# SimonsRoad/gf-pl-slam

Hardware: AMD Instinct MI355X
Metric: stereo frames/sec (2k ORB + 500 LBD, 10 GN iters) (higher is better)
Workload: dtype f64

## Files before the change

gf-pl-slam_amd/csrc/gfpl_abi.hip:

```cpp
#include <hip/hip_runtime.h>

#include <algorithm>
#include <atomic>
#include <cmath>
#include <mutex>
#include <cstdio>
#include <cstdlib>
#include <cstring>
#include <vector>

#include "../../include/gfpl.h"
#include "gfpl_kernels.hpp"

using namespace gfpl;

#define GFPL_NEV 10

struct gfpl_ctx {
    int device = 0;
    hipStream_t stream = nullptr;
    bool own_stream = false;
    gfpl_camera cam{};
    gfpl_config cfg{};
    bool has_cam = false, has_cfg = false;
    bool timing = false;
    hipEvent_t ev[GFPL_NEV]{};
    float stage_ms[7]{};
    std::vector<gfpl_seqbatch*> sbs;
    std::atomic<int> n_detectors{0};
    std::mutex host_mu;
    char* fuse_ws = nullptr;
    size_t fuse_ws_bytes = 0;
    int* fuse_host = nullptr;
    hipEvent_t fuse_ev[2][4]{};
    bool fuse_timed[2] = {false, false};
};

struct gfpl_seqbatch {
    gfpl_ctx* ctx = nullptr;
    int B = 0, kp_cap = 0, kl_cap = 0, mpt_cap = 0, mls_cap = 0;
    void* base = nullptr;
    int64_t bytes = 0;
    DevFrame slot[2];
    int prev_slot = 0;
    bool initialized = false;
    bool has_curr = false;
    DevTrack tr{};
    DevScratch scr{};
    void* stage[2] = {nullptr, nullptr};
    size_t stage_bytes[2] = {0, 0};
    gfpl_frames stage_view[2]{};
    hipStream_t copy = nullptr;
    hipEvent_t ev_ready[2]{}, ev_free[2]{};
    bool ready_pending[2] = {false, false}, free_recorded[2] = {false, false};
    hipEvent_t ev_ticket[16]{};
    int64_t n_tickets = 0;
    int32_t* last_n_pt = nullptr;
    int32_t* last_n_ls = nullptr;
    PyrBuild* pyrb = nullptr;
    int last_cut_mode = -1;
};

struct gfpl_event {
    int device = 0;
    hipEvent_t ev = nullptr;
    int64_t records = 0;
};

int gfpl_ctx_device(const gfpl_ctx* c) { return c->device; }
void* gfpl_ctx_stream(const gfpl_ctx* c) { return (void*)c->stream; }
const gfpl_camera* gfpl_ctx_camera(const gfpl_ctx* c) { return c->has_cam ? &c->cam : nullptr; }
const gfpl_config* gfpl_ctx_config(const gfpl_ctx* c) { return &c->cfg; }
int64_t gfpl_event_records(const gfpl_event* e) { return e->records; }
void gfpl_ctx_attach(gfpl_ctx* c) { c->n_detectors.fetch_add(1); }
void gfpl_ctx_detach(gfpl_ctx* c) { c->n_detectors.fetch_sub(1); }


namespace {

#define HIPCHK(x)                                                  \
    do {                                                            \
        hipError_t e_ = (x);                                        \
        if (e_ != hipSuccess) {                                     \
            std::fprintf(stderr, "gfpl: %s failed: %s\n", #x, hipGetErrorString(e_)); \
            return GFPL_E_HIP;                                      \
        }                                                           \
    } while (0)

int debug_fill_byte() { return env_int("GFPL_DEBUG_FILL", 0) & 0xFF; }

template <typename F, typename H, typename V>
void frame_fields(F& f, H& o, V& v) {
    v.pt(f.pt.pl, o.pt_pl, 2); v.pt(f.pt.pl_obs, o.pt_pl_obs, 2);
    v.pt(f.pt.disp, o.pt_disp, 1); v.pt(f.pt.P, o.pt_P, 3); v.pt(f.pt.sigma2, o.pt_sigma2, 1);
    v.pt(f.pt.idx, o.pt_idx, 1); v.pt(f.pt.level, o.pt_level, 1); v.pt(f.pt.inlier, o.pt_inlier, 1);
    v.pt(f.pt.desc, o.pdesc, 32); v.count(f.pt.n);
    v.ls(f.ls.spl, o.ls_spl, 2); v.ls(f.ls.epl, o.ls_epl, 2);
    v.ls(f.ls.spl_obs, o.ls_spl_obs, 2); v.ls(f.ls.epl_obs, o.ls_epl_obs, 2);
    v.ls(f.ls.sdisp, o.ls_sdisp, 1); v.ls(f.ls.edisp, o.ls_edisp, 1);
    v.ls(f.ls.sdisp_obs, o.ls_sdisp_obs, 1); v.ls(f.ls.edisp_obs, o.ls_edisp_obs, 1);
    v.ls(f.ls.angle, o.ls_angle, 1); v.ls(f.ls.sigma2, o.ls_sigma2, 1);
    v.ls(f.ls.sP, o.ls_sP, 3); v.ls(f.ls.eP, o.ls_eP, 3);
    v.ls(f.ls.le, o.ls_le, 3); v.ls(f.ls.le_obs, o.ls_le_obs, 3);
    v.ls(f.ls.covS, o.ls_covS, 9); v.ls(f.ls.covE, o.ls_covE, 9);
    v.ls(f.ls.cut, o.ls_cut, 2); v.ls(f.ls.invcov, o.ls_invcov, 36);
    v.ls(f.ls.idx, o.ls_idx, 1); v.ls(f.ls.level, o.ls_level, 1); v.ls(f.ls.inlier, o.ls_inlier, 1);
    v.ls(f.ls.desc, o.ldesc, 32); v.count(f.ls.n);
    v.seq(f.pose.Tfw, o.Tfw, 16); v.seq(f.pose.DT, o.DT, 16);
    v.seq(f.pose.DT_cov, o.DT_cov, 36); v.seq(f.pose.Tfw_cov, o.Tfw_cov, 36);
    v.seq(f.pose.DT_cov_eig, o.DT_cov_eig, 6);
    v.seq(f.pose.err_norm, &o.err_norm, 1); v.seq(f.pose.time_stamp, &o.time_stamp, 1);
}

struct SlotCarve {
    Carver& c;
    size_t B, P, L;
    template <typename T, typename U> void pt(T*& d, U, int w) { d = c.take<T>(P * w); }
    template <typename T, typename U> void ls(T*& d, U, int w) { d = c.take<T>(L * w); }
    template <typename T, typename U> void seq(T*& d, U, int w) { d = c.take<T>(B * w); }
    void count(int32_t*& d) { d = c.take<int32_t>(B); }
};

void carve(Carver& c, gfpl_seqbatch* sb) {
    const size_t B = sb->B, P = (size_t)B * sb->kp_cap, L = (size_t)B * sb->kl_cap;
    const gfpl_frame_host none{};
    SlotCarve v{c, B, P, L};
    for (int s = 0; s < 2; ++s) frame_fields(sb->slot[s], none, v);
    sb->tr.matched_pt = c.take<int32_t>(B * sb->mpt_cap);
    sb->tr.n_matched_pt = c.take<int32_t>(B);
    sb->tr.matched_ls = c.take<int32_t>(B * sb->mls_cap);
    sb->tr.n_matched_ls = c.take<int32_t>(B);
    sb->tr.n_inliers = c.take<int32_t>(B);
    sb->tr.n_inliers_pt = c.take<int32_t>(B);
    sb->tr.n_inliers_ls = c.take<int32_t>(B);
    sb->tr.num_frame_loss = c.take<int32_t>(B);
    sb->tr.kf_T = c.take<double>(B * 16);
    sb->tr.kf_cov = c.take<double>(B * 36);
    sb->tr.kf_entropy0 = c.take<double>(B);
    sb->tr.kf_ratio = c.take<double>(B);
    sb->tr.kf_prev_iskf = c.take<int32_t>(B);
    sb->tr.kf_nsince = c.take<int32_t>(B);
    sb->tr.kf_flag = c.take<int32_t>(B);
    sb->scr.cut_rec = c.take<double>(B * sb->mls_cap * CUT_REC);
    sb->scr.knn = c.take<int32_t>(B * 2 * (size_t)sb->kp_cap * 3);
    sb->scr.proj = reinterpret_cast<double*>(sb->scr.knn);
    sb->scr.bytes = c.take<int64_t>(B * STEP_REC);
    sb->scr.n_subpix = c.take<int32_t>(B);
    sb->scr.cut_sum = c.take<double>(B * CUT_SUM_REC);
    sb->scr.cut_dtinv = c.take<double>(B * 16);
    sb->scr.cut_vtab = c.take<double>(B * sb->mls_cap * 2 * CUT_KS);
    sb->scr.pose_DT = c.take<double>(B * 16);
    sb->scr.pose_H = c.take<double>(B * 36);
    sb->scr.pose_err = c.take<double>(B);
    sb->scr.pose_ok = c.take<int32_t>(B);
    sb->scr.pose_in = c.take<double>(B * (6 * (size_t)sb->mpt_cap + 10 * (size_t)sb->mls_cap));
    sb->scr.pose_act = c.take<double>(B * (6 * (size_t)sb->mpt_cap + 10 * (size_t)sb->mls_cap));
    sb->scr.pose_dtini = c.take<double>(B * 16);
    sb->scr.cross_tinv = c.take<double>(B * 16);
    sb->scr.dbg = c.take<int64_t>(B * DBG_REC);
    sb->scr.cut_prog = c.take<int32_t>((size_t)1 << 17);
    sb->scr.cut_path = c.take<uint8_t>(B * sb->mls_cap * CUT_PATH);
    sb->scr.cut_flag = c.take<int32_t>(B);
    sb->scr.cut_vmax = c.take<double>(B * sb->mls_cap * CUT_VMAX);
    sb->scr.cut_offl = c.take<int32_t>(1 + B * sb->mls_cap);
    sb->scr.cut_dtln = c.take<int32_t>(1 + CUT_DTL * B);
    sb->scr.cut_dtl = c.take<double>(CUT_DTL * B * CUT_DTL_REC);
    sb->scr.kf_mask = c.take<int32_t>(B);
    sb->last_n_pt = c.take<int32_t>(B);
    sb->last_n_ls = c.take<int32_t>(B);
}

DevCam devcam(const gfpl_camera& c) {
    DevCam d;
    d.fx = c.fx; d.fy = c.fy; d.cx = c.cx; d.cy = c.cy; d.b = c.b;
    d.width = c.width; d.height = c.height; d.n_levels = c.n_levels;
    for (int i = 0; i < GFPL_MAX_LEVELS; ++i) {
        d.scale[i] = c.scale[i]; d.inv_scale[i] = c.inv_scale[i];
        d.lvl_cols[i] = c.lvl_cols[i]; d.lvl_rows[i] = c.lvl_rows[i];
        d.lvl_offset[i] = c.lvl_offset[i];
        d.sigma2_pt[i] = c.sigma2_pt[i]; d.sigma2_ln[i] = c.sigma2_ln[i];
    }
    d.pyr_bytes = c.pyr_bytes;
    return d;
}

KParams params(gfpl_seqbatch* sb, const gfpl_frames* in) {
    KParams p;
    std::memset(&p, 0, sizeof p);
    p.cam = devcam(sb->ctx->cam);
    p.cfg = sb->ctx->cfg;
    p.prev = sb->slot[sb->prev_slot];
    p.curr = sb->slot[1 - sb->prev_slot];
    p.tr = sb->tr;
    p.scr = sb->scr;
    if (in) p.in = *in;
    p.B = sb->B; p.kp_cap = sb->kp_cap; p.kl_cap = sb->kl_cap;
    p.mpt_cap = sb->mpt_cap; p.mls_cap = sb->mls_cap;
    p.cfg.max_point_match_num = std::min(p.cfg.max_point_match_num, sb->mpt_cap);
    p.cfg.max_line_match_num = std::min(p.cfg.max_line_match_num, sb->mls_cap);
    p.sp_maxD = (float)p.cam.fx;
    p.sp_mbf = (float)(p.cam.fx * p.cam.b);
    p.cut_tq = 0.25 * p.cfg.cut_certify - 4.0 * 0x1p-53;
    {
        const double s = p.cfg.cut_step, lo = p.cfg.cut_rng[0], hi = p.cfg.cut_rng[1];
        auto same = [](double x, double y) { return std::memcmp(&x, &y, sizeof x) == 0; };
        int n = 0;
        for (double t = 0.0; n < CUT_KS && t <= hi && s > 0.0; t = t + s) p.cut_keys[n++] = t;
        const int ns = n;
        for (int i = 1; i < ns && n < CUT_KS; ++i) {
            const double e = p.cut_keys[i] - s;
            bool have = false;
            for (int k = 0; k < n; ++k) have = have || same(p.cut_keys[k], e);
            if (!have && e >= lo) p.cut_keys[n++] = e;
        }
        for (int i = 0; i < n; ++i) {
            int up = -1, dn = -1;
            for (int k = 0; k < n; ++k) {
                if (same(p.cut_keys[k], p.cut_keys[i] + s)) up = k;
                if (same(p.cut_keys[k], p.cut_keys[i] - s)) dn = k;
            }
            p.cut_knxt[i] = (int8_t)up;
            p.cut_kprv[i] = (int8_t)dn;
        }
        p.cut_nkeys = n;
    }
    return p;
}

int check_in(gfpl_seqbatch* sb, const gfpl_frames* in) {
    if (!in) return GFPL_E_INVALID;
    if (in->batch != sb->B || in->kp_cap != sb->kp_cap || in->kl_cap != sb->kl_cap) return GFPL_E_INVALID;
    if (!in->n_kp_l || !in->n_kp_r || !in->kp_l || !in->kp_r || !in->pdesc_l || !in->pdesc_r || !in->n_kl_l ||
        !in->n_kl_r || !in->kl_l || !in->kl_r || !in->ldesc_l || !in->ldesc_r || !in->pyr_r || !in->time_stamp)
        return GFPL_E_INVALID;
    if (((uintptr_t)in->pyr_r & 3) != 0) return GFPL_E_INVALID;
    if ((in->ready && in->ready->device != sb->ctx->device) || (in->consumed && in->consumed->device != sb->ctx->device))
        return GFPL_E_INVALID;
    return GFPL_OK;
}

int in_acquire(gfpl_seqbatch* sb, const gfpl_frames* in) {
    if (in->ready && hipStreamWaitEvent(sb->ctx->stream, in->ready->ev, 0) != hipSuccess) return -2;
    for (int s = 0; s < 2; ++s)
        if (sb->stage[s] && in->n_kp_l == sb->stage_view[s].n_kp_l) {
            if (sb->ready_pending[s] && hipStreamWaitEvent(sb->ctx->stream, sb->ev_ready[s], 0) != hipSuccess) return -2;
            return s;
        }
    return -1;
}
int in_release(gfpl_seqbatch* sb, const gfpl_frames* in, int slot) {
    if (in->consumed) {
        if (hipEventRecord(in->consumed->ev, sb->ctx->stream) != hipSuccess) return GFPL_E_HIP;
        ++in->consumed->records;
    }
    if (slot < 0) return GFPL_OK;
    if (hipEventRecord(sb->ev_free[slot], sb->ctx->stream) != hipSuccess) return GFPL_E_HIP;
    sb->free_recorded[slot] = true;
    return GFPL_OK;
}

static int cut_mode(const gfpl_config& c) { return c.cut_with_max_vol ? c.cut_proof : 0; }

int cfg_supported(const gfpl_config& c) {
    if (!c.best_lr_matches || !c.lr_in_parallel) return GFPL_E_UNSUPPORTED;
    if (c.max_point_match_num < 1 || c.max_point_match_num > GFPL_MAX_MATCHED_PT) return GFPL_E_INVALID;
    if (c.max_line_match_num < 1 || c.max_line_match_num > GFPL_MAX_MATCHED_LS) return GFPL_E_INVALID;
    if (!(c.cut_certify == 0.0 || (c.cut_certify >= 1e-10 && c.cut_certify < 1.0))) return GFPL_E_INVALID;
    if (c.cut_proof < 0 || c.cut_proof > 3) return GFPL_E_INVALID;
    if (!(std::isfinite(c.cut_step) && c.cut_step > 0.0)) return GFPL_E_INVALID;
    if (!(std::isfinite(c.cut_rng[0]) && std::isfinite(c.cut_rng[1]) && c.cut_rng[0] <= c.cut_rng[1]))
        return GFPL_E_INVALID;
    return GFPL_OK;
}

void tmark(gfpl_ctx* c, int i) {
    if (c->timing) (void)hipEventRecord(c->ev[i], c->stream);
}

}

extern "C" {

int gfpl_create(int device, void* stream, gfpl_ctx** out) {
    if (!out) return GFPL_E_INVALID;
    int n = 0;
    if (hipGetDeviceCount(&n) != hipSuccess || n == 0) return GFPL_E_NO_DEVICE;
    if (device < 0 || device >= n) return GFPL_E_INVALID;
    HIPCHK(hipSetDevice(device));
    gfpl_ctx* c = new gfpl_ctx();
    c->device = device;
    c->stream = (hipStream_t)stream;
    gfpl_config_default(&c->cfg);
    c->has_cfg = true;
    for (int i = 0; i < GFPL_NEV; ++i)
        if (hipEventCreate(&c->ev[i]) != hipSuccess) { delete c; return GFPL_E_HIP; }
    *out = c;
// ... 1017 lines not shown
}
}

extern "C" {

int gfpl_read_frame(gfpl_seqbatch* sb, int which, int seq, gfpl_frame_host* o) {
    if (!sb || !o || seq < 0 || seq >= sb->B || (which != GFPL_PREV && which != GFPL_CURR)) return GFPL_E_INVALID;
    hipStream_t s = sb->ctx->stream;
    const DevFrame& f = sb->slot[which == GFPL_PREV ? sb->prev_slot : 1 - sb->prev_slot];
    HIPCHK(hipStreamSynchronize(s));
    int np = 0, nl = 0;
    HIPCHK(hipMemcpy(&np, f.pt.n + seq, 4, hipMemcpyDeviceToHost));
    HIPCHK(hipMemcpy(&nl, f.ls.n + seq, 4, hipMemcpyDeviceToHost));
    o->n_pt = np; o->n_ls = nl;
    SlotCopy<true> v{s, (size_t)seq, (size_t)seq * sb->kp_cap, (size_t)seq * sb->kl_cap, (size_t)np, (size_t)nl};
    frame_fields(f, *o, v);
    HIPCHK(v.e);
    HIPCHK(hipStreamSynchronize(s));
    return GFPL_OK;
}

int gfpl_write_frame(gfpl_seqbatch* sb, int which, int seq, const gfpl_frame_host* o) {
    if (!sb || !o || seq < 0 || seq >= sb->B || (which != GFPL_PREV && which != GFPL_CURR)) return GFPL_E_INVALID;
    if (o->n_pt < 0 || o->n_pt > sb->kp_cap || o->n_ls < 0 || o->n_ls > sb->kl_cap) return GFPL_E_CAPACITY;
    hipStream_t s = sb->ctx->stream;
    const DevFrame& f = sb->slot[which == GFPL_PREV ? sb->prev_slot : 1 - sb->prev_slot];
    XFER(h2d, f.pt.n + seq, &o->n_pt, 1);
    XFER(h2d, f.ls.n + seq, &o->n_ls, 1);
    SlotCopy<false> v{s, (size_t)seq, (size_t)seq * sb->kp_cap, (size_t)seq * sb->kl_cap, (size_t)o->n_pt, (size_t)o->n_ls};
    frame_fields(f, *o, v);
    HIPCHK(v.e);
    HIPCHK(hipStreamSynchronize(s));
    sb->initialized = true;
    if (which == GFPL_CURR) sb->has_curr = true;
    return GFPL_OK;
}

int gfpl_read_track(gfpl_seqbatch* sb, int seq, gfpl_track_host* o) {
    return read_track(sb, seq, o, sb ? sb->tr.n_matched_pt : nullptr, sb ? sb->tr.n_matched_ls : nullptr);
}

int gfpl_read_last_track(gfpl_seqbatch* sb, int seq, gfpl_track_host* o) {
    return read_track(sb, seq, o, sb ? sb->last_n_pt : nullptr, sb ? sb->last_n_ls : nullptr);
}

int gfpl_write_track(gfpl_seqbatch* sb, int seq, const gfpl_track_host* o) {
    if (!sb || !o || seq < 0 || seq >= sb->B) return GFPL_E_INVALID;
    if (o->n_matched_pt < 0 || o->n_matched_pt > sb->mpt_cap || o->n_matched_ls < 0 || o->n_matched_ls > sb->mls_cap)
        return GFPL_E_CAPACITY;
    for (int i = 0; i < o->n_matched_pt; ++i)
        if (o->matched_pt[i] < 0 || o->matched_pt[i] >= sb->kp_cap) return GFPL_E_INVALID;
    for (int i = 0; i < o->n_matched_ls; ++i)
        if (o->matched_ls[i] < 0 || o->matched_ls[i] >= sb->kl_cap) return GFPL_E_INVALID;
    hipStream_t s = sb->ctx->stream;
    XFER(h2d, sb->tr.n_matched_pt + seq, &o->n_matched_pt, 1);
    XFER(h2d, sb->tr.n_matched_ls + seq, &o->n_matched_ls, 1);
    XFER(h2d, sb->tr.n_inliers + seq, &o->n_inliers, 1);
    XFER(h2d, sb->tr.n_inliers_pt + seq, &o->n_inliers_pt, 1);
    XFER(h2d, sb->tr.n_inliers_ls + seq, &o->n_inliers_ls, 1);
    XFER(h2d, sb->tr.num_frame_loss + seq, &o->num_frame_loss, 1);
    XFER(h2d, sb->tr.matched_pt + (size_t)seq * sb->mpt_cap, o->matched_pt, (size_t)o->n_matched_pt);
    XFER(h2d, sb->tr.matched_ls + (size_t)seq * sb->mls_cap, o->matched_ls, (size_t)o->n_matched_ls);
    HIPCHK(hipStreamSynchronize(s));
    return GFPL_OK;
}

int gfpl_set_timing(gfpl_ctx* c, int enable) {
    if (!c) return GFPL_E_INVALID;
    c->timing = enable != 0;
    return GFPL_OK;
}

int gfpl_get_stage_times(gfpl_ctx* c, float* ms7) {
    if (!c || !ms7) return GFPL_E_INVALID;
    if (!c->timing) return GFPL_E_STATE;
    HIPCHK(hipEventSynchronize(c->ev[6]));
    for (int i = 0; i < 6; ++i) HIPCHK(hipEventElapsedTime(&ms7[i], c->ev[i], c->ev[i + 1]));
    HIPCHK(hipEventElapsedTime(&ms7[6], c->ev[0], c->ev[6]));
    return GFPL_OK;
}

int gfpl_get_kernel_times(gfpl_ctx* c, float* ms4) {
    if (!c || !ms4) return GFPL_E_INVALID;
    if (!c->timing) return GFPL_E_STATE;
    if (!c->cfg.use_line_conf_cut) return GFPL_E_STATE;
    HIPCHK(hipEventSynchronize(c->ev[6]));
    HIPCHK(hipEventElapsedTime(&ms4[0], c->ev[4], c->ev[7]));
    HIPCHK(hipEventElapsedTime(&ms4[1], c->ev[7], c->ev[8]));
    HIPCHK(hipEventElapsedTime(&ms4[2], c->ev[8], c->ev[5]));
    HIPCHK(hipEventElapsedTime(&ms4[3], c->ev[5], c->ev[9]));
    return GFPL_OK;
}

}

namespace {
int step_rec_sums(gfpl_seqbatch* sb, int64_t* sums) {
    std::vector<int64_t> v((size_t)sb->B * STEP_REC);
    HIPCHK(hipStreamSynchronize(sb->ctx->stream));
    HIPCHK(hipMemcpy(v.data(), sb->scr.bytes, sizeof(int64_t) * v.size(), hipMemcpyDeviceToHost));
    for (int s = 0; s < STEP_REC; ++s) {
        int64_t t = 0;
        for (int b = 0; b < sb->B; ++b) t += v[(size_t)b * STEP_REC + s];
        sums[s] = t;
    }
    return GFPL_OK;
}
int step_rec_sums(gfpl_seqbatch* sb, int first, int n, int64_t* out, bool on = true) {
    if (!sb || !out) return GFPL_E_INVALID;
    int64_t v[STEP_REC];
    const int e = step_rec_sums(sb, v);
    if (e) return e;
    for (int s = 0; s < n; ++s) out[s] = on ? v[first + s] : 0;
    return GFPL_OK;
}
}

extern "C" {

int gfpl_last_step_kernel_bytes(gfpl_seqbatch* sb, int64_t* bytes4) {
    if (!sb || !bytes4) return GFPL_E_INVALID;
    int64_t v[STEP_REC];
    int e = step_rec_sums(sb, v);
    if (e) return e;
    const bool cut = sb->last_cut_mode >= 0;
    bytes4[0] = cut ? 212 * v[GFPL_STEP_M_L] + 44 * v[GFPL_STEP_M_P] + 552 * (int64_t)sb->B : 0;
    bytes4[1] = v[GFPL_STEP_B_CUT_SEARCH];
    bytes4[2] = cut ? 612 * v[GFPL_STEP_M_L] : 0;
    bytes4[3] = v[GFPL_STEP_B_POSE];
    return GFPL_OK;
}

int gfpl_last_step_stage_bytes(gfpl_seqbatch* sb, int64_t* bytes7) {
    return step_rec_sums(sb, GFPL_STEP_B_STEREO_POINTS, 7, bytes7);
}

int gfpl_last_step_counts(gfpl_seqbatch* sb, int64_t* counts8) {
    return step_rec_sums(sb, GFPL_STEP_N_O, 8, counts8);
}

int gfpl_last_step_track_counts(gfpl_seqbatch* sb, int64_t* counts4) {
    return step_rec_sums(sb, GFPL_STEP_CUT_STEPS, 4, counts4);
}

int gfpl_last_step_cut_proof(gfpl_seqbatch* sb, int64_t* counts4) {
    return step_rec_sums(sb, GFPL_STEP_PROOF_REDONE, 4, counts4,
                         sb && (sb->last_cut_mode == 1 || sb->last_cut_mode == 3));
}

int gfpl_debug_cut_records(gfpl_seqbatch* sb, int b, double* out, int n_lines) {
    if (!sb || !out || b < 0 || b >= sb->B || n_lines < 0 || n_lines > sb->mls_cap) return GFPL_E_INVALID;
    if (hipSetDevice(sb->ctx->device) != hipSuccess) return GFPL_E_HIP;
    if (hipStreamSynchronize(sb->ctx->stream) != hipSuccess) return GFPL_E_HIP;
    const size_t n = (size_t)n_lines * CUT_REC;
    return hipMemcpy(out, sb->scr.cut_rec + (size_t)b * sb->mls_cap * CUT_REC, n * sizeof(double),
                     hipMemcpyDeviceToHost) == hipSuccess ? GFPL_OK : GFPL_E_HIP;
}

int gfpl_debug_step_records(gfpl_seqbatch* sb, int64_t* out) {
    if (!sb || !out) return GFPL_E_INVALID;
    if (hipSetDevice(sb->ctx->device) != hipSuccess) return GFPL_E_HIP;
    if (hipStreamSynchronize(sb->ctx->stream) != hipSuccess) return GFPL_E_HIP;
    return hipMemcpy(out, sb->scr.bytes, (size_t)sb->B * STEP_REC * sizeof(int64_t), hipMemcpyDeviceToHost) == hipSuccess
               ? GFPL_OK : GFPL_E_HIP;
}

int gfpl_debug_clocks(gfpl_seqbatch* sb, int64_t* out) {
    if (!sb || !out) return GFPL_E_INVALID;
    if (hipSetDevice(sb->ctx->device) != hipSuccess) return GFPL_E_HIP;
    if (hipStreamSynchronize(sb->ctx->stream) != hipSuccess) return GFPL_E_HIP;
    return hipMemcpy(out, sb->scr.dbg, (size_t)sb->B * DBG_REC * sizeof(int64_t), hipMemcpyDeviceToHost) == hipSuccess
               ? GFPL_OK : GFPL_E_HIP;
}

int gfpl_last_step_bytes(gfpl_seqbatch* sb, int64_t* bytes) {
    if (!bytes) return GFPL_E_INVALID;
    return step_rec_sums(sb, GFPL_STEP_B_TOTAL, 1, bytes);
}

}
```

gf-pl-slam_amd/csrc/gfpl_kernels.hpp:

```cpp
#pragma once
#include "gfpl_layout.hpp"
#include "gfpl_state.hpp"

#include <atomic>
#include <cstdlib>

namespace gfpl {

inline int env_int(const char* name, int dflt) {
    const char* e = getenv(name);
    if (!e) return dflt;
    return (int)strtol(e, nullptr, (e[0] == '0' && (e[1] == 'x' || e[1] == 'X')) ? 16 : 10);
}

inline hipError_t ensure_dyn_lds(const void* fn, int bytes, std::atomic<unsigned long long>* done) {
    int dev = 0;
    hipError_t e = hipGetDevice(&dev);
    if (e != hipSuccess) return e;
    const unsigned long long bit = dev < 64 ? 1ull << dev : 0ull;
    if (bit && (done->load(std::memory_order_acquire) & bit)) return hipSuccess;
    e = hipFuncSetAttribute(fn, hipFuncAttributeMaxDynamicSharedMemorySize, bytes);
    if (e == hipSuccess && bit) done->fetch_or(bit, std::memory_order_acq_rel);
    return e;
}

constexpr int DYN_LDS_CEILING = 160 * 1024 - 1024;

int sp_wide_max_b();
hipError_t launch_stereo_points(const KParams& p, hipStream_t s);
hipError_t launch_stereo_lines(const KParams& p, hipStream_t s);
hipError_t launch_line_uncertainty(const KParams& p, hipStream_t s);
hipError_t launch_init(const KParams& p, hipStream_t s);
hipError_t launch_knn2(const uint8_t* q, int nq, const uint8_t* t, int nt, int cell, int32_t* idx, float* dist,
                       hipStream_t s);
hipError_t launch_knn2_batched(const uint8_t* q, const int* nq, const uint8_t* t, const int* nt, int cap, int B,
                               int cell, int32_t* packed, hipStream_t s);
hipError_t launch_knn2_counts(const uint8_t* q, const int* nq, const uint8_t* t, const int* nt, int cap, int cell,
                              int32_t* idx, float* dist, hipStream_t s);
hipError_t launch_radius_count(const uint8_t* q, int nq, const uint8_t* t, int nt, int cell, float radius,
                               int32_t* cnt, hipStream_t s);
hipError_t launch_radius_rows(const uint8_t* q, int nq, const uint8_t* t, int nt, int cell, float radius,
                              const int32_t* row_off, int32_t* idx, float* dist, hipStream_t s);
hipError_t launch_match_stats(int kind, const float* d0, const float* d1, int n, int max_num, double* out,
                              hipStream_t s);
hipError_t launch_cross_points(const KParams& p, hipStream_t s);
hipError_t launch_cross_lines(const KParams& p, hipStream_t s);
hipError_t launch_line_cut(const KParams& p, hipStream_t s, const hipEvent_t* marks );
hipError_t launch_pose(const KParams& p, hipStream_t s, hipEvent_t mark );
hipError_t launch_step_bytes(const KParams& p, hipStream_t s);
hipError_t launch_need_kf(const KParams& p, hipStream_t s);
hipError_t launch_curr_frame_is_kf(const KParams& p, const int32_t* mask , hipStream_t s);

struct KfGate {
    DevCam cam;
    double T0[16], T1[16];
    double max_ratio_12_p, desc_th_l;
    int lines, n0;
    int map;
    const int32_t* loc;
    int p_stride;
    double epip_p, epip_l;
    const double* le1;
    const int32_t* i12;
    const float* d12;
    const int32_t* i21;
    const double* P0;
    const double* eP0;
    const double* le0;
    const double* sigma2_0;
    const double* pl1;
    int32_t* pairs;
    int* count;
};
hipError_t launch_kf_gate(const KfGate& g, hipStream_t s);
hipError_t launch_kf_map_filter(const DevCam& cam, const double* T1, const double* P, int n, int lines,
                                int32_t* loc, uint8_t* desc_out, const uint8_t* desc_in, int* count, hipStream_t s);

struct FuseSelect {
    DevCam cam;
    int lines, n, n_kf;
    const double* X;
    const int32_t* kf;
    const double* T_kf;
    const uint8_t* desc_in;
    int32_t* loc;
    uint8_t* desc_out;
    int* count;
    int* bad_kf;
};
struct FuseGate {
    int lines, cap;
    const int* n_sel;
    const int32_t* loc;
    const int32_t* idx;
    const double* X;
    double max_pp, max_pl, max_dl;
    int32_t* pairs;
    int* count;
};
hipError_t launch_fuse_select(const FuseSelect& a, hipStream_t s);
hipError_t launch_fuse_gate(const FuseGate& g, hipStream_t s);

struct LoopPair {
    int n0_pt, n0_ls;
    const int32_t *pi12, *pi21;
    const int32_t *li12, *li21;
    const double* P0;
    const double* pl1;
    const double *sP0, *eP0;
    const double* le1;
};
struct LoopArgs {
    DevCam cam;
    double homog_th;
    int max_iters;
    gfpl_loop_params prm;
    const LoopPair* pairs;
    int pt_cap, ls_cap;
    int32_t* pt_pairs;
    uint8_t* pt_inlier;
    int32_t* ls_pairs;
    uint8_t* ls_inlier;
    gfpl_loop_result* out;
};
hipError_t launch_loop_closure(const LoopArgs& a, int n, hipStream_t s);

struct BowVocabDev {
    const uint8_t* desc;
    const BowNode* node;
    const int32_t* rank_word;
    const double* rank_weight;
    int weighting;
};
struct BowSet {
    const uint8_t* desc;
    int count, pad;
};
struct BowPair {
    const int32_t* ia; const double* va;
    const int32_t* ib; const double* vb;
    int na, nb;
};
hipError_t launch_bow_transform(const BowVocabDev& v, const BowSet* sets, int n, int max_count, int cap, int32_t* keys,
                                int32_t* word_ids, double* values, int32_t* n_words, hipStream_t s);
hipError_t launch_bow_score(const BowPair* pairs, int n, double* scores, hipStream_t s);

struct LbaProb {
    gfpl_lba_counts n;
    const double* x_kf;
    double* T_kf;
    const double* T_fix;
    double *pt, *ls;
    const double *pt_obs, *pt_sigma, *ls_obs, *ls_sigma;
    double* x_out;
    const int32_t *lm_start, *obs_lm, *obs_kf;
    LbaPtrs m;
};
struct LbaArgs {
    DevCam cam;
    double homog_th;
    gfpl_lba_params prm;
    const LbaProb* probs;
    gfpl_lba_result* out;
    int lds_kfs;
};
hipError_t launch_lba(const LbaArgs& a, int n, hipStream_t s);

struct GbaRules {
    int divisor_zero;
    int line_th_homog;
    int prepass_transposed;
    int any_sign_pivot;
};
constexpr GbaRules GBA_RULES_REFERENCE{1, 1, 1, 1};
struct GbaProb {
    gfpl_gba_counts n;
    const double* x_kf;
    double* T_kf;
    const double* T_fix;
    double *pt, *ls;
    const double *pt_obs, *pt_sigma, *ls_obs, *ls_sigma;
    double* x_out;
    const int32_t *lm_start, *obs_lm, *obs_kf, *obs_pair, *pair_start, *pair_kf, *kf_start, *kf_obs, *blk_start, *terms;
    GbaPtrs m;
};
struct GbaArgs {
    DevCam cam;
    double homog_th;
    gfpl_lba_params prm;
    GbaRules rules;
    GbaProb pr;
    gfpl_lba_result* out;
};
struct GbaGrid {
    int block = GBA_BLOCK;
    int ldlt_kfs = GBA_LDLT_KFS;
};
hipError_t enqueue_gba(const GbaArgs& a, const GbaGrid& grid, hipStream_t s);
int gba_max_lds_bytes(int n_kf);

// ... 161 lines not shown
```

gf-pl-slam_amd/csrc/gfpl_records.hpp:

```cpp
#pragma once
#include <stddef.h>
#include <stdint.h>

#include "../../include/gfpl.h"

namespace gfpl {

constexpr int STEP_REC = GFPL_STEP_REC;
constexpr int STEP_CUT_CLOCK_DURATION = GFPL_STEP_CUT_UNBOUNDED;

constexpr int64_t* step_rec(int64_t* bytes, int b) { return bytes + (size_t)STEP_REC * b; }

constexpr int DBG_REC = 8;
constexpr int64_t* dbg_row(int64_t* dbg, int b) { return dbg + DBG_REC * (size_t)b; }

enum DbgCutSearch { DBG_CUT_HW_ID = 6, DBG_CUT_XCC_ID = 7 };
enum DbgVerify {
    DBG_VFY_TS = 0, DBG_VFY_TK = 1, DBG_VFY_TA = 2, DBG_VFY_TV = 3,
    DBG_VFY_MASK = 4,
    DBG_VFY_WORST = 5,
    DBG_VFY_XCHK = 6,
    DBG_VFY_DLINES = 7
};
enum DbgCutEig { DBG_EIG_SWEEPS = 0, DBG_EIG_EVALS = 1 };
enum DbgCutClock { DBG_CCK_BEGIN = 0, DBG_CCK_END = 1, DBG_CCK_HW_ID = 2, DBG_CCK_XCC_ID = 3 };
enum DbgCutPhase { DBG_CPK_PHASES = 0 , DBG_CPK_TRANS = 4 , DBG_CPK_COUNTS = 7 };
enum DbgCutW { DBG_CWK_PHASES = 0 , DBG_CWK_ROUNDS = 5, DBG_CWK_TRANS = 6, DBG_CWK_STEPS = 7 };
enum DbgStereo { DBG_SP_PROBE_KEYS = 7 };
enum DbgPoseFinish { DBG_PFIN_INVERSE = 0, DBG_PFIN_EIG = 1, DBG_PFIN_REST = 2 };

#define CUT_PATH 64
#define CUT_P_STAY 8
#define CUT_P_EXACT 16
#define CUT_KS 22

#define CUT_FAST 56
#define CUT_REC 80
constexpr int CUT_INFO = 21;
constexpr int CUT_NX = CUT_FAST + CUT_INFO;
constexpr int CUT_NX_EB = 3;
#define PD_PS 0
#define PD_PE 18
#define PD_VS 36
#define PD_VE 41
#define PD_OK 46
#define PD_NEXT 47
#define PD_ERR 48
static_assert(PD_ERR + 7 <= CUT_FAST && CUT_FAST == 56, "per-line comparison data layout");
static_assert(CUT_REC * 8 == 640 && CUT_NX + CUT_NX_EB <= CUT_REC, "a record is 5 x 128 B: five 16-B loads per lane");

constexpr int CUT_SUM_REC = 24;

constexpr int CUT_VMAX_EB = 6;
constexpr int CUT_VMAX = CUT_VMAX_EB + 8;

#define CUT_DTL 4
constexpr int CUT_DTL_REC = 32;
enum CutDtl {
    DTL_S = 0,
    DTL_K0 = CUT_INFO, DTL_A1, DTL_B1, DTL_CS, DTL_CE, DTL_R0, DTL_RTS, DTL_RTE, DTL_OK, DTL_END
};
static_assert(DTL_END <= CUT_DTL_REC, "cut_dtl record");

}
```

gf-pl-slam_amd/csrc/gfpl_state.hpp:

```cpp
#pragma once
#include <stdint.h>

#include "../../include/gfpl.h"
#include "gfpl_device.hpp"
#include "gfpl_records.hpp"

namespace gfpl {

struct DevPoints {
    double* pl;
    double* pl_obs;
    double* disp;
    double* P;
    double* sigma2;
    int32_t* idx;
    int32_t* level;
    uint8_t* inlier;
    uint8_t* desc;
    int32_t* n;
};

struct DevLines {
    double *spl, *epl, *spl_obs, *epl_obs;
    double *sdisp, *edisp, *sdisp_obs, *edisp_obs;
    double *angle, *sigma2;
    double *sP, *eP, *le, *le_obs;
    double *covS, *covE;
    double *cut;
    double *invcov;
    int32_t *idx, *level;
    uint8_t *inlier;
    uint8_t *desc;
    int32_t* n;
};

struct DevPose {
    double *Tfw, *DT;
    double *DT_cov, *Tfw_cov;
    double *DT_cov_eig;
    double *err_norm, *time_stamp;
};

struct DevFrame {
    DevPoints pt;
    DevLines ls;
    DevPose pose;
};

struct DevTrack {
    int32_t* matched_pt;
    int32_t* n_matched_pt;
    int32_t* matched_ls;
    int32_t* n_matched_ls;
    int32_t* n_inliers;
    int32_t* n_inliers_pt;
    int32_t* n_inliers_ls;
    int32_t* num_frame_loss;
    double* kf_T;
    double* kf_cov;
    double* kf_entropy0;
    double* kf_ratio;
    int32_t* kf_prev_iskf;
    int32_t* kf_nsince;
    int32_t* kf_flag;
};

struct DevScratch {
    double* cut_rec;
    int32_t* knn;
    double* proj;
    int64_t* bytes;
    int32_t* n_subpix;
    double* cut_sum;
    double* cut_dtinv;
    double* cut_vtab;
    double* pose_DT;
    double* pose_H;
    double* pose_err;
    int32_t* pose_ok;
    double* pose_in;
    double* pose_act;
    double* pose_dtini;
    int32_t* kf_mask;
    double* cross_tinv;
    int64_t* dbg;
    int32_t* cut_prog;
    uint8_t* cut_path;
    int32_t* cut_flag;
    int32_t* cut_offl;
    int32_t* cut_dtln;
    double* cut_dtl;
    double* cut_vmax;
};

struct KParams {
    DevCam cam;
    gfpl_config cfg;
    DevFrame prev, curr;
    DevTrack tr;
    DevScratch scr;
    gfpl_frames in;
    int B, kp_cap, kl_cap, mpt_cap, mls_cap;
    const double* dt_ini;
    float sp_maxD, sp_mbf;
    double cut_tq;
    double cut_keys[CUT_KS];
    int cut_nkeys;
    int8_t cut_knxt[CUT_KS], cut_kprv[CUT_KS];
};

#define LINE_SLOT(p, b, m) ((size_t)(b) * (p).mls_cap + (m))

}
```

gf-pl-slam_amd/csrc/k_cut.hip:

```cpp
#include "gfpl_kernels.hpp"
#include "gfpl_wave.hpp"

namespace gfpl {

struct LineCutData {
    double sP[3], eP[3], covS[9], covE[9], Jl[2];
};

template <typename T, bool SD = false>
__device__ __forceinline__ T endpointVar_t(const DevCam& cam, const double* DT_inv, const T* Jl, const T* Pt,
                                           const T* cov, double zlo) {
    T Jdt[9];
#pragma unroll
    for (int i = 0; i < 3; ++i)
#pragma unroll
        for (int j = 0; j < 3; ++j) Jdt[i * 3 + j] = T(DT_inv[i * 4 + j]);
    T cur[3];
    se3_apply_t<T, double>(DT_inv, Pt, cur);
    rb_floor(cur[2], zlo);
    const T f = T(cam.fx), pz = cur[2], pz_2 = pz * pz;
    T Jp[9];
    Jp[0] = f / pz; Jp[3] = T(0.0); Jp[6] = T(0.0);
    Jp[1] = T(0.0); Jp[4] = f / pz; Jp[7] = T(0.0);
    if constexpr (SD) {
        const double n0 = (-f) * cur[0], n1 = (-f) * cur[1], n2 = (-f) * T(cam.b);
        const SharedDiv dz = div_prep(pz_2, n0);
        Jp[2] = div_by(dz, n0);
        Jp[5] = div_by(dz, n1);
        Jp[8] = div_by(dz, n2);
    } else {
        Jp[2] = ((-f) * cur[0]) / pz_2;
        Jp[5] = ((-f) * cur[1]) / pz_2;
        Jp[8] = ((-f) * T(cam.b)) / pz_2;
    }
    T T1[6], T2[6], T3[6], M[4];
#pragma unroll
    for (int i = 0; i < 2; ++i)
#pragma unroll
        for (int j = 0; j < 3; ++j)
            T1[i * 3 + j] = (Jp[i * 3 + 0] * Jdt[0 * 3 + j] + Jp[i * 3 + 1] * Jdt[1 * 3 + j]) + Jp[i * 3 + 2] * Jdt[2 * 3 + j];
#pragma unroll
    for (int i = 0; i < 2; ++i)
#pragma unroll
        for (int j = 0; j < 3; ++j)
            T2[i * 3 + j] = (T1[i * 3 + 0] * cov[0 * 3 + j] + T1[i * 3 + 1] * cov[1 * 3 + j]) + T1[i * 3 + 2] * cov[2 * 3 + j];
#pragma unroll
    for (int i = 0; i < 2; ++i)
#pragma unroll
        for (int j = 0; j < 3; ++j)
            T3[i * 3 + j] = (T2[i * 3 + 0] * Jdt[j * 3 + 0] + T2[i * 3 + 1] * Jdt[j * 3 + 1]) + T2[i * 3 + 2] * Jdt[j * 3 + 2];
#pragma unroll
    for (int i = 0; i < 2; ++i)
#pragma unroll
        for (int j = 0; j < 2; ++j)
            M[i * 2 + j] = (T3[i * 3 + 0] * Jp[j * 3 + 0] + T3[i * 3 + 1] * Jp[j * 3 + 1]) + T3[i * 3 + 2] * Jp[j * 3 + 2];
    const T r0 = Jl[0] * M[0] + Jl[1] * M[2];
    const T r1 = Jl[0] * M[1] + Jl[1] * M[3];
    return r0 * Jl[0] + r1 * Jl[1];
}

template <typename T, bool VAR = true>
__device__ __forceinline__ void cut_endpoint_t(const DevCam& cam, double homog, const double* DT_inv, const T* Jl,
                                               const T* P0, const T* P1, const T* C0, const T* C1, T c, T* out7,
                                               double zlo) {
    T Pt[3];
#pragma unroll
    for (int k = 0; k < 3; ++k) Pt[k] = (T(1.0) - c) * P0[k] + c * P1[k];
    if (VAR) {
        const T a = (T(1.0) - c) * (T(1.0) - c), q = c * c;
        T cov[9];
#pragma unroll
        for (int i = 0; i < 9; ++i) cov[i] = a * C0[i] + q * C1[i];
        out7[0] = endpointVar_t<T>(cam, DT_inv, Jl, Pt, cov, zlo);
    }
    T cur[3];
    se3_apply_t<T, double>(DT_inv, Pt, cur);
    rb_floor(cur[2], zlo);
    poseJac_t<T>(cam, homog, cur, Jl[0], Jl[1], out7 + 1);
}
__device__ __forceinline__ void cut_endpoint(const DevCam& cam, double homog, const double* DT_inv, const double* Jl,
                                             const double* P0, const double* P1, const double* C0, const double* C1,
                                             double c, double* out7) {
    cut_endpoint_t<double>(cam, homog, DT_inv, Jl, P0, P1, C0, C1, c, out7, 0.0);
}

template <bool FULL>
__device__ __forceinline__ void cut_assemble(const double* S7, const double* E7, double* info) {
    const double vs = S7[0], ve = E7[0];
    const double* Js = S7 + 1;
    const double* Je = E7 + 1;
    const double det = vs * ve - 0.0 * 0.0;
    const double invdet = 1.0 / det;
    const double i00 = ve * invdet, i10 = -0.0 * invdet, i01 = -0.0 * invdet, i11 = vs * invdet;
    double T0[6], T1[6];
#pragma unroll
    for (int i = 0; i < 6; ++i) {
        T0[i] = Js[i] * i00 + Je[i] * i10;
        T1[i] = Js[i] * i01 + Je[i] * i11;
    }
    if (FULL) {
#pragma unroll
        for (int i = 0; i < 6; ++i)
#pragma unroll
            for (int j = 0; j < 6; ++j) info[i * 6 + j] = T0[i] * Js[j] + T1[i] * Je[j];
    } else {
#pragma unroll
        for (int i = 0; i < 6; ++i)
#pragma unroll
            for (int j = 0; j <= i; ++j) info[tri(i, j)] = T0[i] * Js[j] + T1[i] * Je[j];
    }
}

template <bool FULL>
__device__ __forceinline__ void poseInfoOnLine(const DevCam& cam, double homog, const double* DT_inv,
                                               const LineCutData& L, double c0, double c1, double* info) {
    double S7[7], E7[7];
    cut_endpoint(cam, homog, DT_inv, L.Jl, L.sP, L.eP, L.covS, L.covE, c0, S7);
    cut_endpoint(cam, homog, DT_inv, L.Jl, L.eP, L.sP, L.covE, L.covS, c1, E7);
    cut_assemble<FULL>(S7, E7, info);
}

__device__ __forceinline__ void load_line(const DevLines& L, size_t q, LineCutData& d) {
#pragma unroll
    for (int k = 0; k < 3; ++k) { d.sP[k] = L.sP[3 * q + k]; d.eP[k] = L.eP[3 * q + k]; }
#pragma unroll
    for (int k = 0; k < 9; ++k) { d.covS[k] = L.covS[9 * q + k]; d.covE[k] = L.covE[9 * q + k]; }
    d.Jl[0] = L.le_obs[3 * q];
    d.Jl[1] = L.le_obs[3 * q + 1];
}


template <typename T>
__device__ __forceinline__ T sym3_t(const T* A, const T* x, const T* y) {
    const T ax = (A[0] * y[0] + A[1] * y[1]) + A[2] * y[2];
    const T ay = (A[1] * y[0] + A[3] * y[1]) + A[4] * y[2];
    const T az = (A[2] * y[0] + A[4] * y[1]) + A[5] * y[2];
    return (x[0] * ax + x[1] * ay) + x[2] * az;
}

template <typename T>
__device__ __forceinline__ void cut_poly_coeff_t(const T* g0, const T* g1, T lx, T ly, int k, T* Pk) {
    const T dx = g1[0] - g0[0], dy = g1[1] - g0[1], dz = g1[2] - g0[2];
    auto prod = [&](T a0, T a1, T b0, T b1) -> T {
        return k == 0 ? a0 * b0 : (k == 1 ? a0 * b1 + a1 * b0 : a1 * b1);
    };
    auto lin = [&](T a0, T a1) -> T { return k == 0 ? a0 : (k == 1 ? a1 : T(0.0)); };
    const T x0 = g0[0], y0 = g0[1], z0 = g0[2];
    Pk[0] = lx * lin(z0, dz);
    Pk[1] = ly * lin(z0, dz);
    Pk[2] = -(lx * lin(x0, dx) + ly * lin(y0, dy));
    Pk[3] = -((lx * prod(x0, dx, y0, dy) + ly * prod(y0, dy, y0, dy)) + ly * prod(z0, dz, z0, dz));
    Pk[4] = (lx * prod(x0, dx, x0, dx) + lx * prod(z0, dz, z0, dz)) + ly * prod(x0, dx, y0, dy);
    Pk[5] = ly * prod(x0, dx, z0, dz) - lx * prod(y0, dy, z0, dz);
}

template <typename T>
__device__ __forceinline__ void cut_poly_coef_t(const double* Dl, const T* sP, const T* eP, const T* covS,
                                                const T* covE, const T* Jl, T* P, T* V, T* g) {
    se3_apply_t<T, double>(Dl, sP, g);
    se3_apply_t<T, double>(Dl, eP, g + 3);
    T A[2][6];
    const T* Cs[2] = {covS, covE};
#pragma unroll
    for (int w = 0; w < 2; ++w) {
        T Tm[9];
#pragma unroll
        for (int i = 0; i < 3; ++i)
#pragma unroll
            for (int k = 0; k < 3; ++k)
                Tm[i * 3 + k] = (T(Dl[i * 4 + 0]) * Cs[w][0 * 3 + k] + T(Dl[i * 4 + 1]) * Cs[w][1 * 3 + k]) +
                                T(Dl[i * 4 + 2]) * Cs[w][2 * 3 + k];
        const int ii[6] = {0, 0, 0, 1, 1, 2}, jj[6] = {0, 1, 2, 1, 2, 2};
#pragma unroll
        for (int e = 0; e < 6; ++e)
            A[w][e] = (Tm[ii[e] * 3 + 0] * T(Dl[jj[e] * 4 + 0]) + Tm[ii[e] * 3 + 1] * T(Dl[jj[e] * 4 + 1])) +
                      Tm[ii[e] * 3 + 2] * T(Dl[jj[e] * 4 + 2]);
    }
#pragma unroll
    for (int side = 0; side < 2; ++side) {
        T* Ps = P + 18 * side;
#pragma unroll
        for (int k = 0; k < 3; ++k) cut_poly_coeff_t<T>(g + 3 * side, g + 3 * (1 - side), Jl[0], Jl[1], k, Ps + 6 * k);
        const T* p0 = Ps;
        const T* p1 = Ps + 6;
        const T a0 = sym3_t<T>(A[side], p0, p0), a1 = sym3_t<T>(A[side], p0, p1), a2 = sym3_t<T>(A[side], p1, p1);
        const T b0 = sym3_t<T>(A[1 - side], p0, p0), b1 = sym3_t<T>(A[1 - side], p0, p1), b2 = sym3_t<T>(A[1 - side], p1, p1);
        T* v = V + 5 * side;
        v[0] = a0;
        v[1] = T(2.0) * (a1 - a0);
        v[2] = ((a2 - T(4.0) * a1) + a0) + b0;
        v[3] = T(2.0) * ((a1 - a2) + b1);
        v[4] = a2 + b2;
    }
}

__device__ __forceinline__ void cut_poly_data(const double* Dl, const LineCutData& d, double homog, double* fd) {
    double P[36], V[10], g[6];
    cut_poly_coef_t<double>(Dl, d.sP, d.eP, d.covS, d.covE, d.Jl, P, V, g);
#pragma unroll
    for (int i = 0; i < 18; ++i) { fd[PD_PS + i] = P[i]; fd[PD_PE + i] = P[18 + i]; }
#pragma unroll
    for (int i = 0; i < 5; ++i) { fd[PD_VS + i] = V[i]; fd[PD_VE + i] = V[5 + i]; }
    const double z0 = g[2], z1 = g[5];
    fd[PD_OK] = (((z0 > 0.0 && z1 > 0.0) || (z0 < 0.0 && z1 < 0.0)) && z0 * z0 > 2.0 * homog && z1 * z1 > 2.0 * homog)
                    ? 1.0 : 0.0;
}

template <int W>
__global__ void __launch_bounds__(64 * W) k_cut_prep(KParams p) {
    extern __shared__ double prep_lds[];
    const int b = blockIdx.x;
    const int lane = threadIdx.x & 63, wv = W > 1 ? (int)(threadIdx.x >> 6) : 0;
    const int nls = p.tr.n_matched_ls[b];
    const int npt = p.tr.n_matched_pt[b];
    if (nls == 0) return;
    double (*chunk)[65] = reinterpret_cast<double (*)[65]>(prep_lds + (size_t)wv * 21 * 65);
    const DevCam& cam = p.cam;
    const double homog = p.cfg.homog_th;
    DevLines& L = p.prev.ls;
    const DevPoints& P = p.prev.pt;
    const size_t lb = (size_t)b * p.kl_cap, pbase = (size_t)b * p.kp_cap;
    const int32_t* mls = p.tr.matched_ls + (size_t)b * p.mls_cap;
    const int32_t* mpt = p.tr.matched_pt + (size_t)b * p.mpt_cap;
    double* rec_l = p.scr.cut_rec + LINE_SLOT(p, b, 0) * CUT_REC;
    double Dl[16];
    {
        double Tc[16], Tp[16], Ti[16];
#pragma unroll
        for (int i = 0; i < 16; ++i) { Tc[i] = p.curr.pose.Tfw[16 * b + i]; Tp[i] = p.prev.pose.Tfw[16 * b + i]; }
        mat4_inv(Tc, Ti);
        mat4_mul(Ti, Tp, Dl);
    }
    if (wv == 0 && lane < 16) p.scr.cut_dtinv[16 * b + lane] = Dl[lane];
    double s = 0.0;
    const int nl_ch = (nls + 63) >> 6, np_ch = (npt + 63) >> 6;
    auto chunk_cnt = [&](int c) {
        const bool lines = c < nl_ch;
        return min(64, (lines ? nls : npt) - (((lines ? c : c - nl_ch)) << 6));
    };
    for (int c0 = 0; c0 < nl_ch + np_ch; c0 += W) {
        const int c = c0 + wv;
        if (c < nl_ch + np_ch) {
            const bool lines = c < nl_ch;
            const int m = ((lines ? c : c - nl_ch) << 6) + lane;
            const int cnt = chunk_cnt(c);
            double info[21];
            double fd[CUT_FAST];
            if (lane < cnt) {
                if (lines) {
                    LineCutData d;
                    load_line(L, lb + mls[m], d);
                    poseInfoOnLine<false>(cam, homog, Dl, d, 0.0, 0.0, info);
#pragma unroll
                    for (int i = PD_ERR; i < CUT_FAST; ++i) fd[i] = 0.0;
                    cut_poly_data(Dl, d, homog, fd);
                    fd[PD_NEXT] = (double)mls[min(m + 1, nls - 1)];
                } else {
                    const size_t q = pbase + mpt[m];
                    double Pp[3] = {P.P[3 * q], P.P[3 * q + 1], P.P[3 * q + 2]};
                    double cur[3], uv[2];
                    se3_apply(Dl, Pp, cur);
                    projection(cam, cur, uv);
                    const double dx = uv[0] - P.pl_obs[2 * q], dy = uv[1] - P.pl_obs[2 * q + 1];
                    double J[6];
                    poseJac(cam, homog, cur, dx, dy, J);
#pragma unroll
                    for (int i = 0; i < 6; ++i)
#pragma unroll
                        for (int j = 0; j <= i; ++j) info[tri(i, j)] = J[i] * J[j];
                }
            }
            if (lines) {
                double* stg = &chunk[0][0];
                const int pl = lane >> 3, pp = lane & 7;
                double* rc = rec_l + (size_t)(c << 6) * CUT_REC;
#pragma unroll
                for (int sl = 0; sl < CUT_REC / 16; ++sl) {
                    if (lane < cnt) {
#pragma unroll
                        for (int k = 0; k < 16; ++k) {
                            const int x = 16 * sl + k;
                            stg[lane * 17 + k] = x < CUT_FAST ? fd[x] : (x < CUT_FAST + 21 ? info[x - CUT_FAST] : 0.0);
                        }
                    }
                    wave_lds_sync();
#pragma unroll
                    for (int g8 = 0; g8 < 8; ++g8) {
                        const int ln = 8 * g8 + pl;
                        if (ln < cnt)
                            reinterpret_cast<double2*>(rc + (size_t)ln * CUT_REC + 16 * sl)[pp] =
                                make_double2(stg[ln * 17 + 2 * pp], stg[ln * 17 + 2 * pp + 1]);
                    }
                    wave_lds_sync();
                }
            }
            if (lane < cnt) {
#pragma unroll
                for (int i = 0; i < 21; ++i) chunk[i][lane] = info[i];
            }
        }
        __syncthreads();
        if (wv == 0 && lane < 21) {
            const double (*all)[21][65] = reinterpret_cast<const double (*)[21][65]>(prep_lds);
            for (int k = 0; k < W && c0 + k < nl_ch + np_ch; ++k) {
                const int cnt = chunk_cnt(c0 + k);
                for (int e = 0; e < cnt; ++e) s = s + all[k][lane][e];
            }
        }
        __syncthreads();
    }
    if (wv == 0 && lane < 21) p.scr.cut_sum[CUT_SUM_REC * b + lane] = s;
}
constexpr size_t cut_prep_lds(int w) { return (size_t)w * 21 * 65 * sizeof(double); }

__device__ __forceinline__ float ceil_f32(double x) {
    if (!(x >= 0.0)) return __builtin_inff();
    float f = (float)x;
    if ((double)f < x) f = __uint_as_float(__float_as_uint(f) + 1u);
    return f;
}
template <bool SD>
__device__ __forceinline__ double ref_vprime_at(const DevCam& cam, double homog, const double* Dl, const double* P0,
                                                const double* P1, const double* C0, const double* C1, const double* Jl,
                                                double c) {
    double Pt[3];
#pragma unroll
    for (int k = 0; k < 3; ++k) Pt[k] = (1.0 - c) * P0[k] + c * P1[k];
    const double a = (1.0 - c) * (1.0 - c), qq = c * c;
    double cov[9];
#pragma unroll
    for (int i = 0; i < 9; ++i) cov[i] = a * C0[i] + qq * C1[i];
    const double v = endpointVar_t<double, SD>(cam, Dl, Jl, Pt, cov, 0.0);
    double cur[3];
    se3_apply(Dl, Pt, cur);
    const double f = cam.fx / ref_max(homog, cur[2] * cur[2]);
    return v / (f * f);
}
__device__ __forceinline__ double ref_vprime(const DevCam& cam, double homog, const double* Dl, const DevLines& L,
                                             size_t q, int side, double c) {
    const double* P0 = side ? L.eP + 3 * q : L.sP + 3 * q;
    const double* P1 = side ? L.sP + 3 * q : L.eP + 3 * q;
    const double* C0 = side ? L.covE + 9 * q : L.covS + 9 * q;
    const double* C1 = side ? L.covS + 9 * q : L.covE + 9 * q;
    const double Jl[2] = {L.le_obs[3 * q], L.le_obs[3 * q + 1]};
    return ref_vprime_at<false>(cam, homog, Dl, P0, P1, C0, C1, Jl, c);
}

__global__ void __launch_bounds__(256) k_cut_vtab(KParams p) {
    const int b = blockIdx.x;
    const int nls = p.tr.n_matched_ls[b];
    const int nk = p.cut_nkeys;
    if (nls == 0 || nk == 0 || (p.cfg.cut_proof != 2 && p.scr.cut_flag[b] == 0)) return;
    const DevLines& L = p.prev.ls;
    const double* Dl = p.scr.cut_dtinv + 16 * (size_t)b;
    const int per = 2 * nk;
    for (int idx = threadIdx.x; idx < nls * per; idx += 256) {
        const int m = idx / per, r = idx - m * per;
        const int side = r >= nk ? 1 : 0, slot = r - side * nk;
        const size_t q = (size_t)b * p.kl_cap + p.tr.matched_ls[LINE_SLOT(p, b, m)];
        p.scr.cut_vtab[LINE_SLOT(p, b, m) * (2 * CUT_KS) + side * CUT_KS + slot] =
            ref_vprime(p.cam, p.cfg.homog_th, Dl, L, q, side, p.cut_keys[slot]);
    }
}

__device__ __forceinline__ void cut_line_bounds(const KParams& p, size_t q, bool pd_ok, const double* Dl, float* eb) {
    const DevLines& L = p.prev.ls;
    const double rlo = p.cfg.cut_rng[0], rhi = p.cfg.cut_rng[1];
    const double C = fmax(rhi, 0.0), T = fmax(fabs(rlo), fabs(rhi));
#pragma unroll
    for (int i = 0; i < 14; ++i) eb[i] = __builtin_inff();
    bool ok = rlo >= 0.0 && rhi <= 1.0 && pd_ok && p.cam.fx > 0.0;
    RB sP[3], eP[3], cS[9], cE[9], Jl[2];
#pragma unroll
    for (int k = 0; k < 3; ++k) { sP[k] = RB(L.sP[3 * q + k]); eP[k] = RB(L.eP[3 * q + k]); }
#pragma unroll
    for (int k = 0; k < 9; ++k) { cS[k] = RB(L.covS[9 * q + k]); cE[k] = RB(L.covE[9 * q + k]); }
    Jl[0] = RB(L.le_obs[3 * q]);
    Jl[1] = RB(L.le_obs[3 * q + 1]);
    double eo[2][7];
    double zlo = 0.0, zmax = 0.0;
    if (ok) {
        RB P[36], V[10], g[6];
        cut_poly_coef_t<RB>(Dl, sP, eP, cS, cE, Jl, P, V, g);
        double gd[6];
        {
            const double s3[3] = {L.sP[3 * q], L.sP[3 * q + 1], L.sP[3 * q + 2]};
            const double e3[3] = {L.eP[3 * q], L.eP[3 * q + 1], L.eP[3 * q + 2]};
            se3_apply(Dl, s3, gd);
            se3_apply(Dl, e3, gd + 3);
        }
        zlo = fmin(fabs(gd[2]) - g[2].e, fabs(gd[5]) - g[5].e);
        zmax = fmax(fabs(gd[2]) + g[2].e, fabs(gd[5]) + g[5].e);
        ok = zlo > 0.0;
#pragma unroll
        for (int side = 0; side < 2; ++side) {
#pragma unroll
            for (int i = 0; i < 6; ++i)
                eo[side][i] = (P[18 * side + i].e + T * (P[18 * side + 6 + i].e + T * P[18 * side + 12 + i].e));
            const RB* v = V + 5 * side;
            eo[side][6] = v[0].e + T * (v[1].e + T * (v[2].e + T * (v[3].e + T * v[4].e)));
        }
    }
    if (ok) {
        const double cam_fx = p.cam.fx;
        const double s1 = zmax * zmax / cam_fx;
#pragma unroll
        for (int side = 0; side < 2; ++side) {
            RB o7[7];
            cut_endpoint_t<RB, false>(p.cam, p.cfg.homog_th, Dl, Jl, side ? eP : sP, side ? sP : eP, side ? cE : cS,
                                      side ? cS : cE, RB(C, 0.0, 0.0), o7, zlo);
#pragma unroll
            for (int i = 0; i < 6; ++i) eb[7 * side + i] = ceil_f32(1.01 * (eo[side][i] + o7[1 + i].e * s1));
            {
                const RB c(C, 0.0, 0.0);
                const RB* Q0 = side ? eP : sP;
                const RB* Q1 = side ? sP : eP;
                RB Pt[3], cur[3];
#pragma unroll
                for (int k = 0; k < 3; ++k) Pt[k] = (RB(1.0) - c) * Q0[k] + c * Q1[k];
                se3_apply_t<RB, double>(Dl, Pt, cur);
                rb_floor(cur[2], zlo);
                eb[7 * side + 6] = cur[2].lo > 0.0 ? ceil_f32(1.01 * cur[2].e / cur[2].lo) : __builtin_inff();
            }
        }
    }
}

__device__ __forceinline__ void cut_line_bounds_p(const KParams& p, size_t q, bool pd_ok, const double* Dl, float* eb) {
    const DevLines& L = p.prev.ls;
    const double rlo = p.cfg.cut_rng[0], rhi = p.cfg.cut_rng[1];
    const double C = fmax(rhi, 0.0), T = fmax(fabs(rlo), fabs(rhi));
#pragma unroll
    for (int i = 0; i < 14; ++i) eb[i] = __builtin_inff();
    if (!(rlo >= 0.0 && rhi <= 1.0 && pd_ok && p.cam.fx > 0.0)) return;
    RB sP[3], eP[3], Jl[2];
#pragma unroll
    for (int k = 0; k < 3; ++k) { sP[k] = RB(L.sP[3 * q + k]); eP[k] = RB(L.eP[3 * q + k]); }
    Jl[0] = RB(L.le_obs[3 * q]);
    Jl[1] = RB(L.le_obs[3 * q + 1]);
    RB g[6];
    se3_apply_t<RB, double>(Dl, sP, g);
    se3_apply_t<RB, double>(Dl, eP, g + 3);
    double gd[6];
    {
        const double s3[3] = {L.sP[3 * q], L.sP[3 * q + 1], L.sP[3 * q + 2]};
        const double e3[3] = {L.eP[3 * q], L.eP[3 * q + 1], L.eP[3 * q + 2]};
        se3_apply(Dl, s3, gd);
        se3_apply(Dl, e3, gd + 3);
    }
    const double zlo = fmin(fabs(gd[2]) - g[2].e, fabs(gd[5]) - g[5].e);
    const double zmax = fmax(fabs(gd[2]) + g[2].e, fabs(gd[5]) + g[5].e);
    if (!(zlo > 0.0)) return;
    const double s1 = zmax * zmax / p.cam.fx;
#pragma unroll
    for (int side = 0; side < 2; ++side) {
        double eo[6] = {0, 0, 0, 0, 0, 0};
        double tk = 1.0;
#pragma unroll
        for (int k = 0; k < 3; ++k) {
            RB Pk[6];
            cut_poly_coeff_t<RB>(g + 3 * side, g + 3 * (1 - side), Jl[0], Jl[1], k, Pk);
#pragma unroll
            for (int i = 0; i < 6; ++i) eo[i] = eo[i] + tk * Pk[i].e;
            tk = tk * T;
        }
        RB o7[7];
        cut_endpoint_t<RB, false>(p.cam, p.cfg.homog_th, Dl, Jl, side ? eP : sP, side ? sP : eP, nullptr, nullptr,
                                  RB(C, 0.0, 0.0), o7, zlo);
#pragma unroll
        for (int i = 0; i < 6; ++i) eb[7 * side + i] = ceil_f32(1.01 * (eo[i] + o7[1 + i].e * s1));
        const RB c(C, 0.0, 0.0);
        const RB* Q0 = side ? eP : sP;
        const RB* Q1 = side ? sP : eP;
        RB Pt[3], cur[3];
#pragma unroll
        for (int k = 0; k < 3; ++k) Pt[k] = (RB(1.0) - c) * Q0[k] + c * Q1[k];
        se3_apply_t<RB, double>(Dl, Pt, cur);
        rb_floor(cur[2], zlo);
        eb[7 * side + 6] = cur[2].lo > 0.0 ? ceil_f32(1.01 * cur[2].e / cur[2].lo) : __builtin_inff();
    }
}

__global__ void __launch_bounds__(64) k_cut_bounds(KParams p) {
    const int b = blockIdx.y;
    const int m = blockIdx.x * 64 + threadIdx.x;
    const int nls = p.tr.n_matched_ls[b];
    if (m >= nls || (p.cfg.cut_proof != 2 && p.scr.cut_flag[b] == 0)) return;
    const size_t q = (size_t)b * p.kl_cap + p.tr.matched_ls[LINE_SLOT(p, b, m)];
    double* rec = p.scr.cut_rec + LINE_SLOT(p, b, m) * CUT_REC;
    double Dl[16];
#pragma unroll
    for (int i = 0; i < 16; ++i) Dl[i] = p.scr.cut_dtinv[16 * b + i];
    float eb[14];
    cut_line_bounds(p, q, rec[PD_OK] != 0.0, Dl, eb);
    float* out = reinterpret_cast<float*>(rec + PD_ERR);
#pragma unroll
    for (int i = 0; i < 14; ++i) out[i] = eb[i];
}

#define CUT_G 8
#ifndef CUT_BATCH
#define CUT_BATCH 8
#endif
#ifndef CUT_WAIT
#define CUT_WAIT 16
#endif
#define CUT_SL 7
#define CUT_EP 43

__device__ __forceinline__ void exact_endpoint(const DevCam& cam, double homog, const double* Dl, const DevLines& L,
                                               size_t q, int side, double t, double* o7) {
    const double* sP = L.sP + 3 * q;
    const double* eP = L.eP + 3 * q;
    const double* cS = L.covS + 9 * q;
    const double* cE = L.covE + 9 * q;
    const double Jl[2] = {L.le_obs[3 * q], L.le_obs[3 * q + 1]};
    cut_endpoint(cam, homog, Dl, Jl, side ? eP : sP, side ? sP : eP, side ? cE : cS, side ? cS : cE, t, o7);
}

__device__ __forceinline__ int nb_off(int j, int side) {
    const unsigned pl = side == 0 ? 0x31u : 0x54u, mi = side == 0 ? 0xC2u : 0xA8u;
    return (int)((pl >> j) & 1u) - (int)((mi >> j) & 1u);
}
__device__ __forceinline__ double nb_step(int j, int side, double st) {
    return (double)nb_off(j, side) * st;
}
__device__ __forceinline__ int nb_slot(int j, int side) {
    return 1 + nb_off(j, side);
}

constexpr double CUT_MIN_PIVOT = 1e-2;
__device__ __forceinline__ void chol_s(const double* a, double* out) {
    double L[21];
#pragma unroll
    for (int i = 0; i < 21; ++i) L[i] = a[i];
    bool ok = true;
#pragma unroll
    for (int k = 0; k < 6; ++k) {
        const double akk = L[tri(k, k)];
        double x = akk;
#pragma unroll
        for (int j = 0; j < k; ++j) x = x - L[tri(k, j)] * L[tri(k, j)];
        if (!(x > CUT_MIN_PIVOT * akk && akk < 1e300)) { ok = false; x = 1.0; }
        double r = __builtin_amdgcn_rsq(x);
        r = r * (1.5 - (0.5 * x) * (r * r));
        r = r * (1.5 - (0.5 * x) * (r * r));
        L[tri(k, k)] = 0.0;
        out[21 + k] = r;
#pragma unroll
        for (int i = k + 1; i < 6; ++i) {
            double v = L[tri(i, k)];
#pragma unroll
            for (int j = 0; j < k; ++j) v = v - L[tri(i, j)] * L[tri(k, j)];
            L[tri(i, k)] = v * r;
        }
    }
#pragma unroll
    for (int i = 0; i < 21; ++i) out[i] = L[i];
    out[27] = ok ? 1.0 : 0.0;
}

__device__ __forceinline__ double rcp_fast(double x) {
    double r = __builtin_amdgcn_rcp(x);
    r = __builtin_fma(__builtin_fma(-x, r, 1.0), r, r);
    r = __builtin_fma(__builtin_fma(-x, r, 1.0), r, r);
    return r;
}

__device__ __forceinline__ double h4(const double* c, double t) {
    return __builtin_fma(t, __builtin_fma(t, __builtin_fma(t, __builtin_fma(t, c[4], c[3]), c[2]), c[1]), c[0]);
}
__device__ __forceinline__ double h4abs(const double* c, double t) {
    return __builtin_fma(t, __builtin_fma(t, __builtin_fma(t, __builtin_fma(t, fabs(c[4]), fabs(c[3])), fabs(c[2])),
                                          fabs(c[1])), fabs(c[0]));
}
__device__ __forceinline__ double h2(double c0, double c1, double c2, double t) {
    return __builtin_fma(t, __builtin_fma(t, c2, c1), c0);
}

__device__ __forceinline__ double cut_ours_P(const double* fd, int side, int i, double t) {
    const int o = side ? PD_PE : PD_PS;
    return h2(fd[o + i], fd[o + 6 + i], fd[o + 12 + i], t);
}
__device__ __forceinline__ double cut_ours_V(const double* fd, int side, double t) {
    const int o = side ? PD_VE : PD_VS;
    return __builtin_fma(t, __builtin_fma(t, __builtin_fma(t, __builtin_fma(t, fd[o + 4], fd[o + 3]), fd[o + 2]),
                                          fd[o + 1]), fd[o]);
}
__device__ __forceinline__ double cut_ours_info(const double* xs, double is, double ie, int ra, int cb) {
    return __builtin_fma(xs[1 + ra] * is, xs[1 + cb], (xs[8 + ra] * ie) * xs[8 + cb]);
}

struct __attribute__((aligned(16))) CutCmp {
    double ns[5], ne[5];
    double vs[5], ve[5];
    double cc[9];
    double bnd[3];
    double bs[3], be[3];
    float eb[6];
};
static_assert(sizeof(CutCmp) == 336, "CutCmp: 84 dwords (bank spread of the 8 groups' rows)");
enum { CC_NS = 0, CC_NE = 5, CC_VS = 10, CC_VE = 15, CC_CC = 20, CC_BND = 29, CC_BS = 32, CC_BE = 35, CC_END = 38 };
static_assert(offsetof(CutCmp, ns) == 8 * CC_NS && offsetof(CutCmp, ne) == 8 * CC_NE && offsetof(CutCmp, vs) == 8 * CC_VS &&
              offsetof(CutCmp, ve) == 8 * CC_VE && offsetof(CutCmp, cc) == 8 * CC_CC && offsetof(CutCmp, bnd) == 8 * CC_BND &&
              offsetof(CutCmp, bs) == 8 * CC_BS && offsetof(CutCmp, be) == 8 * CC_BE && offsetof(CutCmp, eb) == 8 * CC_END,
              "CutCmp's fields as double offsets");
struct CutReg {
    double ns[5], ne[5], vs[5], ve[5], cc[9], bnd[3];
    float eb[6];
};
__device__ __forceinline__ void cut_reg_load(const CutCmp& c, CutReg& r) {
#pragma unroll
    for (int i = 0; i < 5; ++i) { r.ns[i] = c.ns[i]; r.ne[i] = c.ne[i]; r.vs[i] = c.vs[i]; r.ve[i] = c.ve[i]; }
#pragma unroll
    for (int i = 0; i < 9; ++i) r.cc[i] = c.cc[i];
#pragma unroll
    for (int i = 0; i < 3; ++i) r.bnd[i] = c.bnd[i];
#pragma unroll
    for (int i = 0; i < 6; ++i) r.eb[i] = c.eb[i];
}

template <bool PROOF>
__device__ __forceinline__ double cut_dcore_p1(double Ns, double Vs, double Ne, double Ve, double C, double P1,
                                              double VsA, double VeA, const float* eb, double tq, int& bound_ok) {
    const double D = __builtin_fma(Vs + Ns, Ve + Ne, -(C * C));
    const double den = Vs * Ve;
    const double r = rcp_fast(den);
    const double d = D * r;
    const double P2 = __builtin_fma(VsA, Ve, VeA * Vs);
    constexpr double u = 0x1p-53;
    const double Dd = D * den;
    const bool healthy = (Vs > 0.0) & (Ve > 0.0) & (D > 0.0) & (d < 1e300) & (Dd < 1e300);
    const float iVs = (float)(Ve * r), iVe = (float)(Vs * r);
    const float E = __builtin_fmaf(iVs, __builtin_fmaf(eb[2], iVs, eb[1]), iVe * __builtin_fmaf(eb[4], iVe, eb[3]));
    bool agree = true;
    if (PROOF) agree = (E * 1.0001f <= eb[0]) & (eb[5] * (iVs + iVe) <= 0.25f);
    (void)E;
    const bool fwd = __builtin_fma((40.0 * u) * P1, den, ((16.0 * u) * P2) * D) <= tq * Dd;
    bound_ok = healthy & agree & fwd;
    return healthy ? d : __longlong_as_double(0x7ff8000000000000ll);
}
template <bool PROOF>
__device__ __forceinline__ double cut_dval(const CutReg& c, double t0, double t1, double tq, int& bound_ok,
                                           double vs_t = 0.0, double ve_t = 0.0) {
    const double Ns = h4(c.ns, t0), Ne = h4(c.ne, t1);
    const double Vs = PROOF ? vs_t : h4(c.vs, t0), Ve = PROOF ? ve_t : h4(c.ve, t1);
    const double C = __builtin_fma(t1, __builtin_fma(t1, h2(c.cc[2], c.cc[5], c.cc[8], t0), h2(c.cc[1], c.cc[4], c.cc[7], t0)),
                                   h2(c.cc[0], c.cc[3], c.cc[6], t0));
    return cut_dcore_p1<PROOF>(Ns, Vs, Ne, Ve, C, c.bnd[0], c.bnd[1], c.bnd[2], c.eb, tq, bound_ok);
}

__device__ __attribute__((noinline)) double cut_exact_step(const double* sj, const double* ej, const double* s1,
                                                           const double* e4, const double* S, const double* Sb,
                                                           int first, double* mc) {
    double tot[21], tmp[21];
    cut_assemble<false>(sj, ej, tmp);
#pragma unroll
    for (int i = 0; i < 21; ++i) tot[i] = tmp[i] + S[i];
    const double vj = logdet6_lower(tot);
    if (first) {
#pragma unroll
        for (int i = 0; i < 21; ++i) tot[i] = Sb[i];
    } else {
        cut_assemble<false>(s1, e4, tmp);
#pragma unroll
        for (int i = 0; i < 21; ++i) tot[i] = tmp[i] + S[i];
    }
    *mc = logdet6_lower(tot);
    return vj;
}


__device__ __forceinline__ int group_first_max(double v, int valid, int j, double mc, double& top) {
    const double x = (valid && v == v) ? v : -__builtin_inf();
    double mx = fmax(x, dpp_mov_f64<DPP_XOR1>(x));
    mx = fmax(mx, dpp_mov_f64<DPP_XOR2>(mx));
    mx = fmax(mx, dpp_mov_f64<DPP_HALF_MIRROR>(mx));
    top = mx;
    const unsigned long long at = __ballot((x == mx) & (mx > -__builtin_inf()));
    const unsigned gb = (unsigned)(at >> (threadIdx.x & ~7u)) & 0xFFu;
    const int k = gb ? __builtin_ctz(gb) : 8;
    (void)j;
    return (k < 8 && mx > mc) ? k : -1;
}


struct CutX {
    int best;
    int m_sync;
};
template <typename T>
__device__ __forceinline__ T* rl_ptr(T* p, int l) {
    const unsigned long long v = reinterpret_cast<unsigned long long>(p);
    const unsigned lo = (unsigned)__builtin_amdgcn_readlane((int)(unsigned)v, l);
    const unsigned hi = (unsigned)__builtin_amdgcn_readlane((int)(unsigned)(v >> 32), l);
    return reinterpret_cast<T*>(((unsigned long long)hi << 32) | lo);
}
__device__ __attribute__((noinline)) CutX cut_exact_round(bool exact, int valid, int first, int m, int m_sync, double r0,
                                                          double r1, size_t q_cur, size_t lb, int best,
                                                          const int32_t* mls, const double* rec_l, double* sP, double* eP,
                                                          double* covS, double* covE, double* le_obs, double* cut,
                                                          double* sumE, double* tmp, double* tmpw, const double* Dl,
                                                          double fx, double cb, double homog, double st) {
    const int j = threadIdx.x & 7;
    const int lane = threadIdx.x & 63;
    DevCam cam{};
    cam.fx = fx;
    cam.b = cb;
    DevLines L{};
    L.sP = sP;
    L.eP = eP;
    L.covS = covS;
    L.covE = covE;
    L.le_obs = le_obs;
    L.cut = cut;
    __builtin_amdgcn_fence(__ATOMIC_SEQ_CST, "workgroup");
    {
        unsigned long long need = __ballot(j == 0 && exact && m_sync < m);
        while (need) {
            const int gl = __ffsll((long long)need) - 1;
            need &= need - 1;
            const int ms = __builtin_amdgcn_readlane(m_sync, gl), me = __builtin_amdgcn_readlane(m, gl);
            const size_t lbG = (size_t)(unsigned)__builtin_amdgcn_readlane((int)(unsigned)lb, gl) |
                               ((size_t)(unsigned)__builtin_amdgcn_readlane((int)(unsigned)(lb >> 32), gl) << 32);
            const int32_t* mlsG = rl_ptr(mls, gl);
            const double* recG = rl_ptr(rec_l, gl);
            const double* DlG = rl_ptr(Dl, gl);
            double* sumEG = rl_ptr(sumE, gl);
            const bool mine = (lane >> 3) == (gl >> 3);
            for (int s0 = ms; s0 < me; s0 += 64) {
                const int nl = min(64, me - s0);
                double info[21];
                if (lane < nl) {
                    const size_t qf = lbG + mlsG[s0 + lane];
                    const double c0 = __hip_atomic_load(&L.cut[2 * qf], __ATOMIC_RELAXED, __HIP_MEMORY_SCOPE_WORKGROUP);
                    const double c1 = __hip_atomic_load(&L.cut[2 * qf + 1], __ATOMIC_RELAXED, __HIP_MEMORY_SCOPE_WORKGROUP);
                    double s7[7], e7[7];
                    exact_endpoint(cam, homog, DlG, L, qf, 0, c0, s7);
                    exact_endpoint(cam, homog, DlG, L, qf, 1, c1, e7);
                    cut_assemble<false>(s7, e7, info);
                }
#pragma unroll
                for (int c = 0; c < 6; ++c) {
                    if (lane < nl) {
#pragma unroll
                        for (int i = 0; i < 4; ++i) {
                            const int e = 4 * c + i;
                            if (e < 21) {
                                tmpw[4 * lane + i] = info[e];
                                tmpw[256 + 4 * lane + i] = recG[(size_t)(s0 + lane) * CUT_REC + CUT_FAST + e];
                            }
                        }
                    }
                    wave_lds_sync();
                    if (mine && j < 4 && 4 * c + j < 21) {
                        const int e = 4 * c + j;
                        double Se = sumEG[e];
                        for (int l = 0; l < nl; ++l) Se = (Se - tmpw[256 + 4 * l + j]) + tmpw[4 * l + j];
                        sumEG[e] = Se;
                    }
                    wave_lds_sync();
                }
            }
            if (mine) m_sync = me;
        }
    }
    double* const epf = tmp;
    double* const xs = tmp + CUT_EP;
    if (exact) {
        if (j < 6) {
            const int eside = j < 3 ? 0 : 1;
            const double eoff = (j % 3) == 0 ? -st : ((j % 3) == 2 ? st : 0.0);
            const double t = (eside == 0 ? r0 : r1) + eoff;
            double o7[7];
            exact_endpoint(cam, homog, Dl, L, q_cur, eside, t, o7);
#pragma unroll
            for (int i = 0; i < 7; ++i) epf[CUT_SL * j + i] = o7[i];
        }
#pragma unroll
        for (int e = 0; e < 21; ++e) xs[e] = sumE[e] - rec_l[(size_t)m * CUT_REC + CUT_FAST + e];
    }
    wave_lds_sync();
    if (exact) {
        const int cs = nb_slot(j, 0), ce = 3 + nb_slot(j, 1);
        double mc, top;
        const double vj = cut_exact_step(&epf[CUT_SL * cs], &epf[CUT_SL * ce], &epf[CUT_SL * 1], &epf[CUT_SL * 4], xs,
                                         sumE, first, &mc);
        best = group_first_max(vj, valid, j, mc, top);
    }
    wave_lds_sync();
    return CutX{best, m_sync};
}

constexpr unsigned long long tri_pack(int want_row) {
    unsigned long long v = 0;
    int e = 0;
    for (int i = 0; i < 6; ++i)
        for (int k = 0; k <= i; ++k, ++e) v |= (unsigned long long)(want_row ? i : k) << (3 * e);
    return v;
}

__device__ __attribute__((noinline)) void cut_bound_row(int j, double T, const double* fs, const double* sA,
                                                        const double* tg, double* wg) {
    const float* ef = reinterpret_cast<const float*>(fs + PD_ERR);
    const double sg = 1.002 * tg[57 + j];
    const double Sii = sA[tri(j, j)];
    const double es = ef[j], ee = ef[7 + j];
    const double ps = fabs(fs[PD_PS + j]) + T * (fabs(fs[PD_PS + 6 + j]) + T * fabs(fs[PD_PS + 12 + j])) + es;
    const double pe = fabs(fs[PD_PE + j]) + T * (fabs(fs[PD_PE + 6 + j]) + T * fabs(fs[PD_PE + 12 + j])) + ee;
    const double rs = sqrt(sg);
    double row = 0.0;
    const double kc = Sii * sg;
    const int ex = __builtin_amdgcn_frexp_exp(Sii);
    wg[j] = kc;
    wg[6 + j] = sqrt(kc);
    wg[12 + j] = sg * ps * ps;
    wg[18 + j] = sg * pe * pe;
    wg[24 + j] = es * rs;
    wg[30 + j] = ee * rs;
    wg[36 + j] = (Sii > 0.0 && Sii < 1e300) ? 0.6931471805599453 * (double)(abs(ex) + 1) : __builtin_inf();
    wg[42 + j] = row * rs;
}
__device__ __attribute__((noinline)) void cut_bound_line(double T, double tau, const double* cl, const double* fs,
                                                         const double* wg, float* eb) {
    const float* ef = reinterpret_cast<const float*>(fs + PD_ERR);
    const double Bs = h2(cl[CC_BS], cl[CC_BS + 1], cl[CC_BS + 2], T), Be = h2(cl[CC_BE], cl[CC_BE + 1], cl[CC_BE + 2], T);
    double sum[8];
    for (int q = 0; q < 8; ++q) {
        double a = wg[6 * q];
        for (int i = 1; i < 6; ++i) a = a + wg[6 * q + i];
        sum[q] = a;
    }
    constexpr double u = 0x1p-53;
    const double Kc = sum[0], xi = sum[1], Qs = sum[2], Qe = sum[3], Lam = sum[6];
    const double epsS = sum[7] + (7.01 * u) * xi * xi;
    const double hs = sum[4] + (6.01 * u) * Bs * xi, he = sum[5] + (6.01 * u) * Be * xi;
    const double rvs = 4.1 * (double)ef[6] + 12.0 * u, rve = 4.1 * (double)ef[13] + 12.0 * u;
    const double ck = 110.0 * u;
    const double K0 = 1.002 * epsS + ck * Kc + (7.1 * u) * Lam;
    const double bs = Bs + hs, be = Be + he;
    const double A1 = 1.03 * (2.0 * ck * Qs + 4.0 * hs * bs + 4.0 * rvs * bs * bs), A2 = 0.0;
    const double B1 = 1.03 * (2.0 * ck * Qe + 4.0 * he * be + 4.0 * rve * be * be), B2 = 0.0;
    double R0 = fmin(0.125 * tau, 1e-3) - 1.01 * K0;
    if (!(epsS <= 1e-3 && Kc <= 1e8 && R0 > 0.0)) R0 = -1.0;
    float r0f = (float)R0;
    if ((double)r0f > R0) r0f = R0 > 0.0 ? __uint_as_float(__float_as_uint(r0f) - 1u) : -1.0f;
    eb[0] = r0f;
    eb[1] = ceil_f32(A1);
    eb[2] = ceil_f32(A2);
    eb[3] = ceil_f32(B1);
    eb[4] = ceil_f32(B2);
    eb[5] = (rvs <= 0.25 && rve <= 0.25) ? 0.0f : __builtin_inff();
}

__device__ __forceinline__ int wave_sum8(int v) {
    v += __shfl_xor(v, 8);
    v += __shfl_xor(v, 16);
    v += __shfl_xor(v, 32);
    return __builtin_amdgcn_readfirstlane(v);
}
struct CutProg { int* own; int* partner; };
__device__ __forceinline__ CutProg cut_prog_slots(int* base) {
    const unsigned hw = __builtin_amdgcn_s_getreg((4 << 0) | (0 << 6) | (31 << 11));
    const unsigned xcc = __builtin_amdgcn_s_getreg((20 << 0) | (0 << 6) | (31 << 11));
    const unsigned simd = ((((xcc & 7u) * 8u + ((hw >> 13) & 7u)) * 2u + ((hw >> 12) & 1u)) * 16u + ((hw >> 8) & 15u)) * 4u +
                          ((hw >> 4) & 3u);
    const unsigned slot = hw & 15u;
    return CutProg{base + simd * 16u + slot, base + simd * 16u + (slot ^ 1u)};
}
#ifndef GFPL_CUT_WPE
#define GFPL_CUT_WPE 2
#endif
#ifndef GFPL_CUT_NOPF
#define GFPL_CUT_NOPF 0
#endif
#define CUT_SSTR (GFPL_CUT_NOPF ? 21 : 25)
template <bool PROOF, bool REC = false>
__global__ void __launch_bounds__(64) __attribute__((amdgpu_waves_per_eu(GFPL_CUT_WPE, GFPL_CUT_WPE))) k_cut_search(KParams p) {
    __shared__ double sumA[CUT_G][CUT_SSTR];
    __shared__ double sumE[CUT_G][CUT_SSTR];
    __shared__ double fst[CUT_G][CUT_FAST + 1];
    constexpr bool PF = !PROOF && !GFPL_CUT_NOPF;
    __shared__ __attribute__((aligned(16))) double nxl[PF ? 5 : 1][PF ? 128 : 2];
    __shared__ double tmp[CUT_G][CUT_EP + 25 + 1];
    static_assert(CUT_G * (CUT_EP + 25 + 1) >= 512, "the exact-sum flush stages 64 x (4 + 4) doubles in tmp");
    __shared__ CutCmp cmpl[CUT_G];
    __shared__ double vtab[PROOF ? CUT_G : 1][PROOF ? 2 * CUT_KS : 1];
    __shared__ int cnxt[PROOF ? CUT_KS : 1], cprv[PROOF ? CUT_KS : 1];
    const int lane = threadIdx.x;
    constexpr bool CLOCK = GFPL_DIAG(GFPL_CUT_CLOCK);
    const uint64_t t_beg = CLOCK ? wall_clock64() : 0;
    const int g = lane >> 3, j = lane & 7;
    const int b = blockIdx.x * CUT_G + g;
    if (!PROOF && p.cfg.cut_proof == 0 && j == 0 && b < p.B) {
        dbg_row(p.scr.dbg, b)[DBG_CUT_HW_ID] = (int64_t)__builtin_amdgcn_s_getreg((4 << 0) | (0 << 6) | (31 << 11));
        dbg_row(p.scr.dbg, b)[DBG_CUT_XCC_ID] = (int64_t)__builtin_amdgcn_s_getreg((20 << 0) | (0 << 6) | (31 << 11));
    }
    const bool live = b < p.B && (!PROOF || p.cfg.cut_proof == 2 || p.scr.cut_flag[b] != 0);
    const int nls = live ? p.tr.n_matched_ls[b] : 0;
    constexpr bool rec = !PROOF && REC;
    uint8_t* const path = p.scr.cut_path + LINE_SLOT(p, live ? b : 0, 0) * CUT_PATH;
    int lstep = 0;
    __shared__ __attribute__((aligned(8))) uint8_t pth[REC ? CUT_G : 1][REC ? CUT_PATH : 8];
    const DevCam& cam = p.cam;
    const double homog = p.cfg.homog_th;
    const double tau = p.cfg.cut_certify;
    const double tq = p.cut_tq;
    DevLines& L = p.prev.ls;
    const size_t lb = (size_t)(live ? b : 0) * p.kl_cap;
    const int32_t* mls = p.tr.matched_ls + (size_t)(live ? b : 0) * p.mls_cap;
    const double* rec_l = p.scr.cut_rec + LINE_SLOT(p, live ? b : 0, 0) * CUT_REC;
    const double* Dl = p.scr.cut_dtinv + 16 * (size_t)(live ? b : 0);
    const double st = p.cfg.cut_step;
    const double rlo = p.cfg.cut_rng[0], rhi = p.cfg.cut_rng[1];
    double* const xs = &tmp[g][CUT_EP];
    double* const wg = &tmp[g][0];
    double* const gm = &tmp[g][36];
    const double nb0 = nb_step(j, 0, st), nb1 = nb_step(j, 1, st);
    constexpr unsigned long long TRI_ROW = tri_pack(1), TRI_COL = tri_pack(0);
    if (PROOF) {
        if (lane < CUT_KS) {
            cnxt[lane] = p.cut_knxt[lane];
            cprv[lane] = p.cut_kprv[lane];
        }
        __syncthreads();
    }
    int m = 0;
    int m_sync = 0;
    int first = 1;
    double r0 = 0.0, r1 = 0.0;
    int line_ok = 0;
    int pend = 0;
    int wait = 0;
    double dc = 0.0;
    int c_ok = 0;
    int n_unb = 0;
    int i0 = 0, i1 = 0, n0s = -1, p0s = -1, n1s = -1, p1s = -1;
    size_t q_cur = 0, q_nx = 0;
    auto open_line = [&]() {
        if (PROOF) {
            const double* vt = p.scr.cut_vtab + LINE_SLOT(p, live ? b : 0, m) * (2 * CUT_KS);
            for (int idx = j; idx < 2 * CUT_KS; idx += 8) vtab[g][idx] = vt[idx];
            i0 = 0;
            i1 = 0;
            n0s = n1s = cnxt[0];
            p0s = p1s = cprv[0];
        }
        double o[28];
        {
            double S[21];
#pragma unroll
            for (int e = 0; e < 21; ++e) S[e] = sumA[g][e];
            chol_s(S, o);
        }
        line_ok = (o[27] != 0.0) && (fst[g][PD_OK] != 0.0);
        if (j < 6) {
            double w[6];
#pragma unroll
            for (int i = 0; i < 6; ++i) {
                double u = fst[g][6 * j + i];
#pragma unroll
                for (int k = 0; k < i; ++k) u = __builtin_fma(-o[tri(i, k)], w[k], u);
                w[i] = u * o[21 + i];
            }
#pragma unroll
            for (int i = 0; i < 6; ++i) wg[6 * j + i] = w[i];
            double x[6], sg = 0.0;
            if (PROOF) {
#pragma unroll
            for (int i = 0; i < 6; ++i) {
                double uu = i == j ? 1.0 : 0.0;
#pragma unroll
                for (int k = 0; k < i; ++k) uu = __builtin_fma(-o[tri(i, k)], x[k], uu);
                x[i] = uu * o[21 + i];
                sg = __builtin_fma(x[i], x[i], sg);
            }
            tmp[g][57 + j] = sg;
            }
        }
        wave_lds_sync();
#pragma unroll
        for (int kk = 0; kk < 3; ++kk) {
            const int e = j + 8 * kk;
            if (e < 21) {
                const int ra = (int)((TRI_ROW >> (3 * e)) & 7), cb = (int)((TRI_COL >> (3 * e)) & 7);
                double s = wg[6 * ra] * wg[6 * cb];
#pragma unroll
                for (int i = 1; i < 6; ++i) s = __builtin_fma(wg[6 * ra + i], wg[6 * cb + i], s);
                gm[e] = s;
            }
        }
        wave_lds_sync();
        double* cl = reinterpret_cast<double*>(&cmpl[g]);
        if (j < 2) {
            const int a = 3 * j, b2 = a + 1, c2 = a + 2;
            double* o = cl + CC_NS + 5 * j;
            o[0] = gm[tri(a, a)];
            o[1] = 2.0 * gm[tri(b2, a)];
            o[2] = __builtin_fma(2.0, gm[tri(c2, a)], gm[tri(b2, b2)]);
            o[3] = 2.0 * gm[tri(c2, b2)];
            o[4] = gm[tri(c2, c2)];
        } else if (j < 4) {
#pragma unroll
            for (int i = 0; i < 5; ++i) cl[CC_VS + 5 * (j - 2) + i] = fst[g][PD_VS + 5 * (j - 2) + i];
        } else if (j < 7) {
            const int i = j - 4;
#pragma unroll
            for (int k = 0; k < 3; ++k) cl[CC_CC + 3 * i + k] = gm[tri(3 + k, i)];
            const double gs = fmax(gm[tri(i, i)], 0.0), ge = fmax(gm[tri(3 + i, 3 + i)], 0.0);
            cl[CC_BS + i] = gs > 0.0 ? 1.01 * gs * __builtin_amdgcn_rsq(gs) : 0.0;
            cl[CC_BE + i] = ge > 0.0 ? 1.01 * ge * __builtin_amdgcn_rsq(ge) : 0.0;
        }
        wave_lds_sync();
        const double T = fmax(fabs(rlo), fabs(rhi));
        if (j == 7) {
            const double Bs = h2(cl[CC_BS], cl[CC_BS + 1], cl[CC_BS + 2], T);
            const double Be = h2(cl[CC_BE], cl[CC_BE + 1], cl[CC_BE + 2], T);
            const double VsA = h4abs(cl + CC_VS, T), VeA = h4abs(cl + CC_VE, T);
            const double Bs2 = Bs * Bs, Be2 = Be * Be;
            cl[CC_BND] = __builtin_fma(Bs2 + VsA, Be2 + VeA, Bs2 * Be2);
            cl[CC_BND + 1] = VsA;
            cl[CC_BND + 2] = VeA;
        } else if (PROOF && j < 6) {
            cut_bound_row(j, T, fst[g], sumA[g], tmp[g], wg);
        }
        wave_lds_sync();
        if (PROOF && j == 7) cut_bound_line(T, tau, cl, fst[g], wg, cmpl[g].eb);
        wave_lds_sync();
        if (PROOF) {
            const float* e6 = cmpl[g].eb;
            bool usable = e6[0] > 0.0f;
#pragma unroll
            for (int i = 1; i < 6; ++i) usable = usable && e6[i] < __builtin_inff();
            n_unb += usable ? 0 : 1;
            if (j < 6 && live) reinterpret_cast<float*>(const_cast<double*>(rec_l) + (size_t)m * CUT_REC + CUT_NX)[j] = e6[j];
        }
        const double vs0 = PROOF ? vtab[g][0] : cl[CC_VS], ve0 = PROOF ? vtab[g][CUT_KS] : cl[CC_VE];
        dc = cut_dcore_p1<PROOF>(cl[CC_NS], vs0, cl[CC_NE], ve0, cl[CC_CC], cl[CC_BND], cl[CC_BND + 1], cl[CC_BND + 2],
                                 cmpl[g].eb, tq, c_ok);
    };
    auto pf_issue = [&](int mm) {
        if (!PF) return;
        const char* src = reinterpret_cast<const char*>(rec_l + (size_t)mm * CUT_REC) + 16 * j;
#pragma unroll
        for (int k = 0; k < (PF ? 5 : 0); ++k) {
            const uint32_t dst = (uint32_t)(uintptr_t)&nxl[k][0];
            asm volatile("s_mov_b32 m0, %1\n\tglobal_load_lds_dwordx4 %0, off" ::"v"(src + 128 * k), "s"(dst)
                         : "memory", "m0");
        }
    };
    if (m < nls) {
        q_cur = lb + mls[0];
        if (nls > 1) q_nx = lb + mls[1];
        for (int e = j; e < CUT_FAST; e += 8) fst[g][e] = rec_l[e];
#pragma unroll
        for (int e = j; e < 21; e += 8) {
            const double s0 = p.scr.cut_sum[CUT_SUM_REC * b + e];
            sumA[g][e] = s0 - rec_l[CUT_FAST + e];
            sumE[g][e] = s0;
        }
        wave_lds_sync();
        open_line();
        if (nls > 1) pf_issue(1);
    }
    __syncthreads();
    int n_steps = 0, n_exact = 0;
    const CutProg prog = cut_prog_slots(p.scr.cut_prog);
    if (lane == 0) __hip_atomic_store(prog.own, 0, __ATOMIC_RELAXED, __HIP_MEMORY_SCOPE_AGENT);
    int partner_done = 0;
    __shared__ int pslot[1];
    if (!PROOF && lane == 0) pslot[0] = 0;
    __builtin_amdgcn_s_setprio(2);
    constexpr bool PCLOCK = GFPL_DIAG(GFPL_CUT_PCLOCK);
    PhaseClock<PCLOCK, 4> pk;
    PhaseClock<PCLOCK, 3> tk;
    pk.reset();
    tk.reset();
    while (__any(m < nls)) {
        const bool act = m < nls && !pend;
        const double t0 = r0 + nb0, t1 = r1 + nb1;
        int valid = act ? 1 : 0;
        if (t0 + t1 > 1.0) valid = 0;
        if (t0 < rlo || t0 > rhi) valid = 0;
        if (t1 < rlo || t1 > rhi) valid = 0;
        int bok;
        double dj;
        CutReg cr;
        cut_reg_load(cmpl[g], cr);
        double vst = 0.0, vet = 0.0;
        if (PROOF) {
            const int s0 = nb0 > 0.0 ? n0s : (nb0 < 0.0 ? p0s : i0);
            const int s1 = nb1 > 0.0 ? n1s : (nb1 < 0.0 ? p1s : i1);
            vst = s0 >= 0 ? vtab[g][s0] : __longlong_as_double(0x7ff8000000000000ll);
            vet = s1 >= 0 ? vtab[g][CUT_KS + s1] : __longlong_as_double(0x7ff8000000000000ll);
        }
        dj = cut_dval<PROOF>(cr, t0, t1, tq, bok, vst, vet);
        double top;
        int best = group_first_max(dj, valid, j, dc, top);
        const bool has = best >= 0, vl = valid != 0;
        const bool f1 = vl & !bok;
        const bool f2 = has & vl & (j != best) & !(top - dj > tau * top);
        const bool f3 = has & !(top - dc > tau * top);
        const bool f4 = !has & vl & !(dc - dj > tau * dc);
        const bool f5 = !((tau > 0.0) & (line_ok != 0) & (c_ok != 0) & (dc == dc));
        const int ok = (f1 | f2 | f3 | f4 | f5) ? 0 : 1;
        const bool exact = act && ((__ballot(!ok) >> (8 * g)) & 0xFFull) != 0;
        n_steps += act ? 1 : 0;
        n_exact += exact ? 1 : 0;
        double dnext = top;
        int cnext = 1;
        PHASE_TICK(pk, 0);
        if (__any(exact)) {
            const CutX xr = cut_exact_round(exact, valid, first, m, m_sync, r0, r1, q_cur, lb, best, mls, rec_l, L.sP, L.eP,
                                            L.covS, L.covE, L.le_obs, L.cut, sumE[g], tmp[g], &tmp[0][0], Dl, cam.fx, cam.b,
                                            homog, st);
            best = xr.best;
            m_sync = xr.m_sync;
            const int src = (lane & ~7) + (best >= 0 ? best : 0);
            const double sd = __shfl(dj, src);
            const int sb = __shfl(bok, src);
            if (exact) { dnext = sd; cnext = sb; }
        }
        PHASE_TICK(pk, 1);
        int finalize = 0;
        if (rec && act) {
            if (j == 0 && lstep < CUT_PATH)
                pth[g][lstep] = (uint8_t)((best >= 0 ? best : CUT_P_STAY) | (exact ? CUT_P_EXACT : 0));
            ++lstep;
        }
        if (act) {
            first = 0;
            if (best >= 0) {
                if (PROOF) {
                    const double a0 = nb_step(best, 0, st), a1 = nb_step(best, 1, st);
                    i0 = i0 < 0 ? -1 : (a0 > 0.0 ? n0s : (a0 < 0.0 ? p0s : i0));
                    i1 = i1 < 0 ? -1 : (a1 > 0.0 ? n1s : (a1 < 0.0 ? p1s : i1));
                    n0s = i0 >= 0 ? cnxt[i0] : -1;
                    p0s = i0 >= 0 ? cprv[i0] : -1;
                    n1s = i1 >= 0 ? cnxt[i1] : -1;
                    p1s = i1 >= 0 ? cprv[i1] : -1;
                }
                r0 = r0 + nb_step(best, 0, st);
                r1 = r1 + nb_step(best, 1, st);
                dc = dnext;
                c_ok = cnext;
                if (!(r0 + r1 <= 1.0)) finalize = 1;
            } else {
                finalize = 1;
            }
        }
        if (rec && act && finalize && m + 1 >= nls) {
            __builtin_amdgcn_wave_barrier();
            if (8 * j < lstep)
                *reinterpret_cast<unsigned long long*>(path + (size_t)m * CUT_PATH + 8 * j) =
                    *reinterpret_cast<const unsigned long long*>(&pth[g][8 * j]);
        }
        if (act && finalize) {
            if (j == 0 && (PROOF || m + 1 >= nls)) {
                L.cut[2 * q_cur] = r0;
                L.cut[2 * q_cur + 1] = r1;
            }
            ++m;
            pend = m < nls;
            wait = 0;
        }
        PHASE_TICK(pk, 2);
        const int npend = __popcll(__ballot(pend)) >> 3;
        if (npend > 0 && (npend >= CUT_BATCH || __any(pend && wait >= CUT_WAIT) || __ballot(m < nls && !pend) == 0)) {
            PHASE_START(tk);
            double info[3];
            if (pend) {
                if (!PROOF && fst[g][PD_OK] != 0.0) {
                    if (j < 6) {
                        xs[1 + j] = cut_ours_P(fst[g], 0, j, r0);
                        xs[8 + j] = cut_ours_P(fst[g], 1, j, r1);
                    } else {
                        xs[7 * (j - 6)] = cut_ours_V(fst[g], j - 6, j == 6 ? r0 : r1);
                    }
                } else if (j < 2) {
                    double o7[7];
                    exact_endpoint(cam, homog, Dl, L, q_cur, j, j ? r1 : r0, o7);
#pragma unroll
                    for (int i = 0; i < 7; ++i) xs[7 * j + i] = o7[i];
                }
            }
            wave_lds_sync();
            if (pend) {
                const double is = rcp_fast(xs[0]), ie = rcp_fast(xs[7]);
                const double invdet = 1.0 / (xs[0] * xs[7] - 0.0 * 0.0);
                const double i00 = xs[7] * invdet, i10 = -0.0 * invdet, i01 = -0.0 * invdet, i11 = xs[0] * invdet;
#pragma unroll
                for (int kk = 0; kk < 3; ++kk) {
                    const int e = min(j + 8 * kk, 20);
                    const int ra = (int)((TRI_ROW >> (3 * e)) & 7), cb = (int)((TRI_COL >> (3 * e)) & 7);
                    if (PROOF) {
                        const double T0 = xs[1 + ra] * i00 + xs[8 + ra] * i10, T1 = xs[1 + ra] * i01 + xs[8 + ra] * i11;
                        info[kk] = T0 * xs[1 + cb] + T1 * xs[8 + cb];
                    } else {
                        info[kk] = cut_ours_info(xs, is, ie, ra, cb);
                    }
                }
                if (!PF) {
#pragma unroll
                    for (int k = 0; k < CUT_FAST / 8; ++k) fst[g][j + 8 * k] = rec_l[(size_t)m * CUT_REC + j + 8 * k];
                }
                if (!PROOF) {
                    if (PF) asm volatile("s_waitcnt vmcnt(0)" ::: "memory");
                    if (j == 0) {
                        L.cut[2 * q_cur] = r0;
                        L.cut[2 * q_cur + 1] = r1;
                    }
                    if (rec && 8 * j < lstep)
                        *reinterpret_cast<unsigned long long*>(path + (size_t)(m - 1) * CUT_PATH + 8 * j) =
                            *reinterpret_cast<const unsigned long long*>(&pth[g][8 * j]);
#pragma unroll
                    for (int k = 0; k < (PF ? CUT_FAST / 8 : 0); ++k) {
                        const int e = j + 8 * k;
                        fst[g][e] = nxl[e >> 4][16 * g + (e & 15)];
                    }
                }
            }
            wave_lds_sync();
            if (pend) {
                q_cur = q_nx;
                q_nx = lb + (size_t)(int)fst[g][PD_NEXT];
                if (PROOF) m_sync = m;
                first = 1;
                lstep = 0;
                r0 = 0.0;
                r1 = 0.0;
#pragma unroll
                for (int kk = 0; kk < 3; ++kk) {
                    const int e = j + 8 * kk;
                    const int x = CUT_FAST + e;
                    if (e < 21) {
                        const double mid = sumA[g][e] + info[kk];
                        const double nw = mid - (PF ? nxl[x >> 4][16 * g + (x & 15)] : rec_l[(size_t)m * CUT_REC + x]);
                        sumA[g][e] = nw;
                        if (PROOF) sumE[g][e] = mid;
                    }
                }
            }
            wave_lds_sync();
            PHASE_TICK(tk, 0);
            if (pend) {
                open_line();
                if (m + 1 < nls) pf_issue(m + 1);
                pend = 0;
            }
            PHASE_TICK(tk, 1);
            {
                if (!PROOF) partner_done = pslot[0];
                const int done = wave_sum8(j == 0 ? m : 0);
                if (done > __builtin_amdgcn_readfirstlane(partner_done)) __builtin_amdgcn_s_setprio(0);
                else __builtin_amdgcn_s_setprio(2);
                if (lane == 0) __hip_atomic_store(prog.own, done, __ATOMIC_RELAXED, __HIP_MEMORY_SCOPE_AGENT);
                if (PROOF) {
                    partner_done = __hip_atomic_load(prog.partner, __ATOMIC_RELAXED, __HIP_MEMORY_SCOPE_AGENT);
                } else if (lane == 0) {
                    const uint32_t dst = (uint32_t)(uintptr_t)&pslot[0];
                    asm volatile("s_mov_b32 m0, %1\n\tglobal_load_lds_dword %0, off sc1" ::"v"(prog.partner), "s"(dst)
                                 : "memory", "m0");
                }
            }
            PHASE_TICK(tk, 2);
        } else if (pend) {
            ++wait;
        }
        PHASE_TICK(pk, 3);
    }
    if (PCLOCK && live && j == 0) {
        int64_t* d = dbg_row(p.scr.dbg, b);
        pk.store(d + DBG_CPK_PHASES);
        tk.store(d + DBG_CPK_TRANS);
        d[DBG_CPK_COUNTS] = (pk.ticks(2) << 32) | tk.ticks(2);
    }
    if (live && j == 0) {
        step_rec(p.scr.bytes, b)[GFPL_STEP_CUT_STEPS] = n_steps;
        step_rec(p.scr.bytes, b)[GFPL_STEP_CUT_EXACT] = n_exact;
        step_rec(p.scr.bytes, b)[GFPL_STEP_CUT_UNBOUNDED] = n_unb;
        if (CLOCK) {
            const uint64_t t_end = wall_clock64();
            int64_t* d = dbg_row(p.scr.dbg, b);
            step_rec(p.scr.bytes, b)[STEP_CUT_CLOCK_DURATION] = (int64_t)(t_end - t_beg);
            d[DBG_CCK_BEGIN] = (int64_t)t_beg;
            d[DBG_CCK_END] = (int64_t)t_end;
            d[DBG_CCK_HW_ID] = (int64_t)__builtin_amdgcn_s_getreg((4 << 0) | (0 << 6) | (31 << 11));
            d[DBG_CCK_XCC_ID] = (int64_t)__builtin_amdgcn_s_getreg((20 << 0) | (0 << 6) | (31 << 11));
        }
    }
}

#ifndef CUT_WAVE_MAX_B
#define CUT_WAVE_MAX_B 2048
#endif

__global__ void __launch_bounds__(64) __attribute__((amdgpu_waves_per_eu(2, 2))) k_cut_search_w(KParams p) {
    __shared__ double sumA[25];
    __shared__ double sumE[25];
    __shared__ double fst[CUT_FAST + 1];
    __shared__ double tmp[CUT_G][CUT_EP + 25 + 1];
    __shared__ double wgs[64];
    __shared__ double xsl[16];
    __shared__ CutCmp cmpl;
    __shared__ double dgx[100];
    __shared__ int dgf[100];
    const int lane = threadIdx.x;
    const int b = blockIdx.x;
    const int nls = p.tr.n_matched_ls[b];
    const DevCam& cam = p.cam;
    const double homog = p.cfg.homog_th;
    const double tau = p.cfg.cut_certify;
    const double tq = p.cut_tq;
    DevLines& L = p.prev.ls;
    const size_t lb = (size_t)b * p.kl_cap;
    const int32_t* mls = p.tr.matched_ls + (size_t)b * p.mls_cap;
    const double* rec_l = p.scr.cut_rec + LINE_SLOT(p, b, 0) * CUT_REC;
    const double* Dl = p.scr.cut_dtinv + 16 * (size_t)b;
    const double st = p.cfg.cut_step;
    const double rlo = p.cfg.cut_rng[0], rhi = p.cfg.cut_rng[1];
    const bool rec = p.cfg.cut_proof != 0;
    uint8_t* const path = p.scr.cut_path + LINE_SLOT(p, b, 0) * CUT_PATH;
    constexpr unsigned long long TRI_ROW = tri_pack(1), TRI_COL = tri_pack(0);
    int m = 0, m_sync = 0, first = 1, line_ok = 0, c_ok = 0, lstep = 0;
    double r0 = 0.0, r1 = 0.0, dc = 0.0;
    size_t q_cur = 0;
    int n_steps = 0, n_exact = 0;
    constexpr bool TCLOCK = GFPL_DIAG(GFPL_CUTW_TCLOCK);
    PhaseClock<TCLOCK, 7> tk;
    tk.reset();
    auto open_line = [&]() {
        double o[28];
        {
            double S[21];
#pragma unroll
            for (int e = 0; e < 21; ++e) S[e] = sumA[e];
            chol_s(S, o);
        }
        PHASE_TICK(tk, 2);
        line_ok = (o[27] != 0.0) && (fst[PD_OK] != 0.0);
        if (lane < 6) {
            double w[6];
#pragma unroll
            for (int i = 0; i < 6; ++i) {
                double u = fst[6 * lane + i];
#pragma unroll
                for (int k = 0; k < i; ++k) u = __builtin_fma(-o[tri(i, k)], w[k], u);
                w[i] = u * o[21 + i];
            }
#pragma unroll
            for (int i = 0; i < 6; ++i) wgs[6 * lane + i] = w[i];
        }
        wave_lds_sync();
        PHASE_TICK(tk, 3);
        if (lane < 21) {
            const int ra = (int)((TRI_ROW >> (3 * lane)) & 7), cb = (int)((TRI_COL >> (3 * lane)) & 7);
            double s = wgs[6 * ra] * wgs[6 * cb];
#pragma unroll
            for (int i = 1; i < 6; ++i) s = __builtin_fma(wgs[6 * ra + i], wgs[6 * cb + i], s);
            wgs[36 + lane] = s;
        }
        wave_lds_sync();
        PHASE_TICK(tk, 4);
        const double* gm = wgs + 36;
        double* cl = reinterpret_cast<double*>(&cmpl);
        double G[21], cv[CC_END];
#pragma unroll
        for (int e = 0; e < 21; ++e) G[e] = gm[e];
#pragma unroll
        for (int i = 0; i < 10; ++i) cv[CC_VS + i] = fst[PD_VS + i];
#pragma unroll
        for (int sd = 0; sd < 2; ++sd) {
            const int a0 = 3 * sd, b2 = a0 + 1, c2 = a0 + 2;
            cv[CC_NS + 5 * sd + 0] = G[tri(a0, a0)];
            cv[CC_NS + 5 * sd + 1] = 2.0 * G[tri(b2, a0)];
            cv[CC_NS + 5 * sd + 2] = __builtin_fma(2.0, G[tri(c2, a0)], G[tri(b2, b2)]);
            cv[CC_NS + 5 * sd + 3] = 2.0 * G[tri(c2, b2)];
            cv[CC_NS + 5 * sd + 4] = G[tri(c2, c2)];
        }
#pragma unroll
        for (int i = 0; i < 3; ++i) {
#pragma unroll
            for (int k = 0; k < 3; ++k) cv[CC_CC + 3 * i + k] = G[tri(3 + k, i)];
            const double gs = fmax(G[tri(i, i)], 0.0), ge = fmax(G[tri(3 + i, 3 + i)], 0.0);
            cv[CC_BS + i] = gs > 0.0 ? 1.01 * gs * __builtin_amdgcn_rsq(gs) : 0.0;
            cv[CC_BE + i] = ge > 0.0 ? 1.01 * ge * __builtin_amdgcn_rsq(ge) : 0.0;
        }
        {
            const double T = fmax(fabs(rlo), fabs(rhi));
            const double Bs = h2(cv[CC_BS], cv[CC_BS + 1], cv[CC_BS + 2], T);
            const double Be = h2(cv[CC_BE], cv[CC_BE + 1], cv[CC_BE + 2], T);
            const double VsA = h4abs(cv + CC_VS, T), VeA = h4abs(cv + CC_VE, T);
            const double Bs2 = Bs * Bs, Be2 = Be * Be;
            cv[CC_BND] = __builtin_fma(Bs2 + VsA, Be2 + VeA, Bs2 * Be2);
            cv[CC_BND + 1] = VsA;
            cv[CC_BND + 2] = VeA;
        }
        if (lane == 0) {
#pragma unroll
            for (int i = 0; i < CC_END; ++i) cl[i] = cv[i];
        }
        wave_lds_sync();
        PHASE_TICK(tk, 5);
        dc = cut_dcore_p1<false>(cv[CC_NS], cv[CC_VS], cv[CC_NE], cv[CC_VE], cv[CC_CC], cv[CC_BND], cv[CC_BND + 1],
                                 cv[CC_BND + 2], cmpl.eb, tq, c_ok);
        PHASE_TICK(tk, 6);
    };
    if (nls > 0) {
        q_cur = lb + mls[0];
        for (int e = lane; e < CUT_FAST; e += 64) fst[e] = rec_l[e];
        if (lane < 21) {
            const double s0 = p.scr.cut_sum[CUT_SUM_REC * b + lane];
            sumA[lane] = s0 - rec_l[CUT_FAST + lane];
            sumE[lane] = s0;
        }
        wave_lds_sync();
        open_line();
    }
    double pf_f0 = 0.0, pf_i0 = 0.0;
    int pf_q = 0;
    auto prefetch = [&](int mn) {
        if (mn < nls) {
            int iv = mn;
            asm volatile("" : "+v"(iv));
            const double* rn = rec_l + (size_t)iv * CUT_REC;
            pf_i0 = lane < 21 ? rn[CUT_FAST + lane] : 0.0;
            pf_f0 = rn[lane < CUT_FAST ? lane : 0];
            pf_q = mls[iv];
        }
    };
    prefetch(1);
    constexpr bool WCLOCK = GFPL_DIAG(GFPL_CUTW_CLOCK);
    enum { CK_EVAL, CK_DEC, CK_WALK, CK_EXACT, CK_TRANS };
    PhaseClock<WCLOCK, 5> ck;
    ck.reset();
    while (m < nls) {
        double g0[8], g1[8];
        g0[1] = r0;
        g1[1] = r1;
        g0[0] = r0 + (-st);
        g1[0] = r1 + (-st);
#pragma unroll
        for (int k = 2; k < 8; ++k) { g0[k] = g0[k - 1] + st; g1[k] = g1[k - 1] + st; }
        int inc0 = 0, inc1 = 0;
#pragma unroll
        for (int k = 2; k <= 6; ++k) {
            inc0 |= (__double_as_longlong(g0[k] + (-st)) != __double_as_longlong(g0[k - 1])) ? (1 << k) : 0;
            inc1 |= (__double_as_longlong(g1[k] + (-st)) != __double_as_longlong(g1[k - 1])) ? (1 << k) : 0;
        }
        const int k0 = inc0 ? __builtin_ctz(inc0) : -1, k1 = inc1 ? __builtin_ctz(inc1) : -1;
        int dj_valid = 0, bok = 0;
        double dj = 0.0;
        double t0 = g0[0], t1 = g1[0];
        CutReg cr;
        cut_reg_load(cmpl, cr);
        {
            const int a = lane >> 3, c = lane & 7;
#pragma unroll
            for (int k = 1; k < 8; ++k) { t0 = a == k ? g0[k] : t0; t1 = c == k ? g1[k] : t1; }
            int valid = 1;
            if (t0 + t1 > 1.0) valid = 0;
            if (t0 < rlo || t0 > rhi) valid = 0;
            if (t1 < rlo || t1 > rhi) valid = 0;
            dj_valid = valid;
            dj = cut_dval<false>(cr, t0, t1, tq, bok);
        }
        if (inc0 | inc1) {
            const int a = lane >> 3, c = lane & 7;
            const int k0s = __builtin_amdgcn_readfirstlane(k0), k1s = __builtin_amdgcn_readfirstlane(k1);
            const double h0 = readlane_f64(t0, k0s > 0 ? 8 * k0s : 0) + (-st);
            const double h1 = readlane_f64(t1, k1s > 0 ? k1s : 0) + (-st);
            const bool row = lane < 8, col = lane == 8 || (c == 7 && a >= 1), cor = lane == 16;
            const double u0 = (row || cor) ? h0 : (lane == 8 ? g0[0] : t0);
            const double u1 = row ? t1 : h1;
            int valid = (row && k0s >= 0) || (col && k1s >= 0) || (cor && k0s >= 0 && k1s >= 0);
            if (u0 + u1 > 1.0) valid = 0;
            if (u0 < rlo || u0 > rhi) valid = 0;
            if (u1 < rlo || u1 > rhi) valid = 0;
            int abok = 0;
            const double da = cut_dval<false>(cr, u0, u1, tq, abok);
            if (row | col | cor) {
                const int slot = row ? 82 + lane : (cor ? 98 : 90 + (lane == 8 ? 0 : a));
                dgx[slot] = (valid && da == da) ? da : -__builtin_inf();
                dgf[slot] = abok | (valid << 1) | ((valid && !(da == da)) ? 4 : 0);
            }
        }
        PHASE_TICK(ck, CK_EVAL);
        constexpr int WAVE_EXACT = 16, WAVE_STOP = 32;
        int dec = WAVE_STOP;
        {
            const int a = lane >> 3, c = lane & 7;
            const int bad0 = inc0 & ~(k0 >= 0 ? 1 << k0 : 0), bad1 = inc1 & ~(k1 >= 0 ? 1 << k1 : 0);
            const bool cons = a >= 1 && a <= 6 && c >= 1 && c <= 6 && !((bad0 >> a) & 1) && !((bad1 >> c) & 1);
            const bool ia = a == k0, ic = c == k1;
            const double xo = (dj_valid && dj == dj) ? dj : -__builtin_inf();
            dgx[9 + lane] = xo;
            dgf[9 + lane] = bok | (dj_valid << 1) | ((dj_valid && !(dj == dj)) ? 4 : 0);
            wave_lds_sync();
            double vjn[8];
            int fl[8];
            if (inc0 | inc1) {
#pragma unroll
                for (int jn = 0; jn < 8; ++jn) {
                    const int da = nb_off(jn, 0), dc = nb_off(jn, 1);
                    const bool xa = ia && da < 0, xc = ic && dc < 0;
                    const int l = (xa && xc) ? 82 + 16 : (xa ? 82 + c + dc : (xc ? 90 + a + da : 9 + lane + 8 * da + dc));
                    vjn[jn] = dgx[l];
                    fl[jn] = dgf[l];
                }
            } else {
#pragma unroll
                for (int jn = 0; jn < 8; ++jn) {
                    const int l = 9 + lane + 8 * nb_off(jn, 0) + nb_off(jn, 1);
                    vjn[jn] = dgx[l];
                    fl[jn] = dgf[l];
                }
            }
            const double dcl = dj;
            const int cok = bok;
            const double m01 = fmax(vjn[0], vjn[1]), m23 = fmax(vjn[2], vjn[3]);
            const double m45 = fmax(vjn[4], vjn[5]), m67 = fmax(vjn[6], vjn[7]);
            const double mx = fmax(fmax(m01, m23), fmax(m45, m67));
            int atm = 0;
#pragma unroll
            for (int jn = 0; jn < 8; ++jn) atm |= (vjn[jn] == mx) ? (1 << jn) : 0;
            const int kf = (mx > -__builtin_inf()) ? __builtin_ctz(atm | 256) : 8;
            const int best = (kf < 8 && mx > dcl) ? kf : -1;
            const double top = mx;
            const bool has = best >= 0;
            const double ttop = tau * top, tdc = tau * dcl;
            int fail = (int)(has & !(top - dcl > ttop)) | (int)!((tau > 0.0) & (line_ok != 0) & (cok != 0) & (dcl == dcl));
#pragma unroll
            for (int jn = 0; jn < 8; ++jn) {
                const double v = vjn[jn];
                const int f = fl[jn];
                const int vl = (f >> 1) & 1;
                const int f1 = vl & ~f & 1;
                const int f2 = (int)has & vl & (int)(jn != best) & (int)!(top - v > ttop);
                const int f4 = (int)!has & vl & (int)!(dcl - v > tdc);
                const int f3 = (f >> 2) & 1;
                fail |= f1 | f2 | f3 | f4;
            }
            const bool ok = fail == 0;
            const bool off = has && ((ia && nb_off(best, 0) < 0) || (ic && nb_off(best, 1) < 0));
            dec = !cons ? WAVE_STOP : (!ok ? ((ia || ic) ? WAVE_STOP : WAVE_EXACT) : (off ? WAVE_STOP : (has ? best : CUT_P_STAY)));
            const int mv = has ? best : 0;
            const double n0 = t0 + nb_step(mv, 0, st), n1 = t1 + nb_step(mv, 1, st);
            const int fin = (has && !(n0 + n1 <= 1.0)) ? 64 : 0;
            dec |= fin | ((lane + 8 * nb_off(mv, 0) + nb_off(mv, 1)) & 63) << 8;
        }
        PHASE_TICK(ck, CK_DEC);
        int pos = 9;
        int exact = 0, finalize = 0;
        double vj[8];
        int bj[8], valj[8];
        int pathv = 0, ns = 0;
        if (!rec) {
            const int dpos = dec & 63;
            const bool cont = dpos < CUT_P_STAY && !(dec & 64);
            int jump = cont ? (dec >> 8) & 63 : lane;
            int acc = cont ? 1 : 0;
#pragma unroll
            for (int r = 0; r < 6; ++r) {
                const int jj = __shfl(jump, jump);
                const int aa = __shfl(acc, jump);
                acc += aa;
                jump = jj;
            }
            const int T = __builtin_amdgcn_readlane(jump, 9);
            ns = __builtin_amdgcn_readlane(acc, 9);
            const int wT = __builtin_amdgcn_readlane(dec, T);
            const int dT = wT & 63;
            pos = T;
            if (dT >= WAVE_EXACT) {
                exact = dT == WAVE_EXACT;
            } else {
                ++ns;
                finalize = 1;
                if (dT != CUT_P_STAY) pos = wT >> 8;
            }
        } else {
            for (int sstep = 0; sstep < 64; ++sstep) {
                const int w = __builtin_amdgcn_readlane(dec, pos);
                const int dpos = w & 63;
                if (dpos >= WAVE_EXACT) {
                    exact = dpos == WAVE_EXACT;
                    break;
                }
                pathv = lane == ns ? dpos : pathv;
                ++ns;
                if (dpos == CUT_P_STAY) { finalize = 1; break; }
                pos = w >> 8;
                if (w & 64) { finalize = 1; break; }
            }
        }
        if (ns) {
            if (rec && lane < ns && lstep + lane < CUT_PATH) path[(size_t)m * CUT_PATH + lstep + lane] = (uint8_t)pathv;
            n_steps += ns;
            lstep += ns;
            first = 0;
        }
        if (exact) {
            const int pa = pos >> 3, pc = pos & 7;
#pragma unroll
            for (int jn = 0; jn < 8; ++jn) {
                const int l = (pa + nb_off(jn, 0)) * 8 + (pc + nb_off(jn, 1));
                vj[jn] = readlane_f64(dj, l);
                bj[jn] = __builtin_amdgcn_readlane(bok, l);
                valj[jn] = __builtin_amdgcn_readlane(dj_valid, l);
            }
        }
        r0 = readlane_f64(t0, pos);
        r1 = readlane_f64(t1, pos);
        PHASE_TICK(ck, CK_WALK);
        if (exact) {
            int myv = 0;
#pragma unroll
            for (int jn = 0; jn < 8; ++jn) myv = lane == jn ? valj[jn] : myv;
            const CutX xr = cut_exact_round(lane < 8, myv, first, m, m_sync, r0, r1, q_cur, lb, -1, mls, rec_l, L.sP,
                                            L.eP, L.covS, L.covE, L.le_obs, L.cut, sumE, tmp[0], &tmp[0][0], Dl,
                                            cam.fx, cam.b, homog, st);
            const int best = __builtin_amdgcn_readfirstlane(xr.best);
            m_sync = __builtin_amdgcn_readfirstlane(xr.m_sync);
            ++n_steps;
            ++n_exact;
            if (rec && lane == 0) {
                if (lstep < CUT_PATH)
                    path[(size_t)m * CUT_PATH + lstep] = (uint8_t)((best >= 0 ? best : CUT_P_STAY) | CUT_P_EXACT);
            }
            ++lstep;
            first = 0;
            if (best < 0) {
                finalize = 1;
            } else {
                double vb = vj[0];
                int bb = bj[0];
#pragma unroll
                for (int jn = 1; jn < 8; ++jn) { vb = best == jn ? vj[jn] : vb; bb = best == jn ? bj[jn] : bb; }
                dc = vb;
                c_ok = bb;
                r0 = r0 + nb_step(best, 0, st);
                r1 = r1 + nb_step(best, 1, st);
                if (!(r0 + r1 <= 1.0)) finalize = 1;
            }
        }
        PHASE_TICK(ck, CK_EXACT);
        if (finalize) {
            PHASE_START(tk);
            if (lane == 0) {
                L.cut[2 * q_cur] = r0;
                L.cut[2 * q_cur + 1] = r1;
            }
            double info = 0.0;
            {
                const int ra = (int)((TRI_ROW >> (3 * lane)) & 7), cb = (int)((TRI_COL >> (3 * lane)) & 7);
                if (fst[PD_OK] != 0.0) {
                    if (lane < 21) {
                        const double is = rcp_fast(cut_ours_V(fst, 0, r0)), ie = rcp_fast(cut_ours_V(fst, 1, r1));
                        const double psr = cut_ours_P(fst, 0, ra, r0), psc = cut_ours_P(fst, 0, cb, r0);
                        const double per = cut_ours_P(fst, 1, ra, r1), pec = cut_ours_P(fst, 1, cb, r1);
                        info = __builtin_fma(psr * is, psc, (per * ie) * pec);
                    }
                } else {
                    if (lane < 2) {
                        double o7[7];
                        exact_endpoint(cam, homog, Dl, L, q_cur, lane, lane ? r1 : r0, o7);
#pragma unroll
                        for (int i = 0; i < 7; ++i) xsl[7 * lane + i] = o7[i];
                    }
                    wave_lds_sync();
                    if (lane < 21) info = cut_ours_info(xsl, rcp_fast(xsl[0]), rcp_fast(xsl[7]), ra, cb);
                }
            }
            ++m;
            PHASE_TICK(tk, 0);
            if (m < nls) {
                wave_lds_sync();
                if (lane < CUT_FAST) fst[lane] = pf_f0;
                if (lane < 21) sumA[lane] = (sumA[lane] + info) - pf_i0;
                q_cur = lb + __builtin_amdgcn_readfirstlane(pf_q);
                first = 1;
                lstep = 0;
                r0 = 0.0;
                r1 = 0.0;
                wave_lds_sync();
                PHASE_TICK(tk, 1);
                open_line();
                prefetch(m + 1);
            }
        }
        PHASE_TICK(ck, CK_TRANS);
    }
    if (lane == 0) {
        step_rec(p.scr.bytes, b)[GFPL_STEP_CUT_STEPS] = n_steps;
        step_rec(p.scr.bytes, b)[GFPL_STEP_CUT_EXACT] = n_exact;
        step_rec(p.scr.bytes, b)[GFPL_STEP_CUT_UNBOUNDED] = 0;
        if (WCLOCK) {
            int64_t* d = dbg_row(p.scr.dbg, b);
            ck.store(d + DBG_CWK_PHASES);
            d[DBG_CWK_ROUNDS] = ck.ticks(CK_WALK);
            d[DBG_CWK_TRANS] = m;
            d[DBG_CWK_STEPS] = n_steps;
        }
        if (TCLOCK) tk.store(dbg_row(p.scr.dbg, b));
    }
}

#define CUTE_LN 27
__global__ void __launch_bounds__(64) __attribute__((amdgpu_waves_per_eu(2, 2))) k_cut_search_eig(KParams p) {
    __shared__ double lnd[CUT_G][CUTE_LN];
    __shared__ double dti[CUT_G][17];
    __shared__ double smat[CUT_G][21];
    __shared__ double ninf[CUT_G][8 * 21 + 1];
    const int lane = threadIdx.x;
    const int g = lane >> 3, j = lane & 7;
    const int b = blockIdx.x * CUT_G + g;
    const bool seq = b < p.B;
    const int nls = seq ? p.tr.n_matched_ls[b] : 0;
    const DevCam& cam = p.cam;
    const double homog = p.cfg.homog_th;
    DevLines& L = p.prev.ls;
    const size_t lb = (size_t)(seq ? b : 0) * p.kl_cap;
    const int32_t* mls = p.tr.matched_ls + (size_t)(seq ? b : 0) * p.mls_cap;
    const double* rec_l = p.scr.cut_rec + LINE_SLOT(p, seq ? b : 0, 0) * CUT_REC;
    const double st = p.cfg.cut_step;
    const double rlo = p.cfg.cut_rng[0], rhi = p.cfg.cut_rng[1];
    const double nb0 = nb_step(j, 0, st), nb1 = nb_step(j, 1, st);
    int m = 0;
    int open = 1;
    double r0 = 0.0, r1 = 0.0;
    double mc = 0.0;
    size_t q_cur = 0;
    double se[3] = {0.0, 0.0, 0.0}, ss[3] = {0.0, 0.0, 0.0}, ci[3] = {0.0, 0.0, 0.0};
    int n_steps = 0, n_eval = 0, n_sweeps = 0;
    auto open_line = [&]() {
        q_cur = lb + mls[m];
        for (int i = j; i < 26; i += 8) {
            double v;
            if (i < 3) v = L.sP[3 * q_cur + i];
            else if (i < 6) v = L.eP[3 * q_cur + i - 3];
            else if (i < 15) v = L.covS[9 * q_cur + i - 6];
            else if (i < 24) v = L.covE[9 * q_cur + i - 15];
            else v = L.le_obs[3 * q_cur + i - 24];
            lnd[g][i] = v;
        }
#pragma unroll
        for (int kk = 0; kk < 3; ++kk) {
            const int e = j + 8 * kk;
            if (e < 21) {
                ci[kk] = rec_l[(size_t)m * CUT_REC + CUT_FAST + e];
                ss[kk] = se[kk] - ci[kk];
                smat[g][e] = se[kk];
            }
        }
        r0 = 0.0;
        r1 = 0.0;
        open = 1;
    };
    if (nls > 0) {
        for (int i = j; i < 16; i += 8) dti[g][i] = p.scr.cut_dtinv[16 * (size_t)b + i];
#pragma unroll
        for (int kk = 0; kk < 3; ++kk) {
            const int e = j + 8 * kk;
            if (e < 21) se[kk] = p.scr.cut_sum[CUT_SUM_REC * (size_t)b + e];
        }
        open_line();
    }
    while (__any(m < nls)) {
        wave_lds_sync();
        const bool live = m < nls;
        const double t0 = r0 + nb0, t1 = r1 + nb1;
        int valid = (live && !open) ? 1 : 0;
        if (t0 + t1 > 1.0) valid = 0;
        if (t0 < rlo || t0 > rhi) valid = 0;
        if (t1 < rlo || t1 > rhi) valid = 0;
        double v = 0.0;
        if (live && (open || valid)) {
            double tot[21];
            if (open) {
#pragma unroll
                for (int e = 0; e < 21; ++e) tot[e] = smat[g][e];
            } else {
                double S7[7], E7[7], info[21];
                const double* d = lnd[g];
                cut_endpoint(cam, homog, dti[g], d + 24, d, d + 3, d + 6, d + 15, t0, S7);
                cut_endpoint(cam, homog, dti[g], d + 24, d + 3, d, d + 15, d + 6, t1, E7);
                cut_assemble<false>(S7, E7, info);
#pragma unroll
                for (int e = 0; e < 21; ++e) {
                    ninf[g][21 * j + e] = info[e];
                    tot[e] = info[e] + smat[g][e];
                }
            }
            double A[36], w[6];
#pragma unroll
            for (int i = 0; i < 6; ++i)
#pragma unroll
                for (int k = 0; k <= i; ++k) {
                    A[i * 6 + k] = tot[tri(i, k)];
                    A[k * 6 + i] = tot[tri(i, k)];
                }
            int sw = 0;
            eig_sym<6, true>(A, w, &sw);
            v = w[0];
            if (!open || j == 0) {
                n_sweeps += sw;
                ++n_eval;
            }
        }
        wave_lds_sync();
        double top;
        const int best = group_first_max(v, valid, j, mc, top);
        if (live && open) {
            mc = v;
            open = 0;
#pragma unroll
            for (int kk = 0; kk < 3; ++kk) {
                const int e = j + 8 * kk;
                if (e < 21) smat[g][e] = ss[kk];
            }
        } else if (live) {
            ++n_steps;
            bool fin = true;
            if (best >= 0) {
#pragma unroll
                for (int kk = 0; kk < 3; ++kk) {
                    const int e = j + 8 * kk;
                    if (e < 21) ci[kk] = ninf[g][21 * best + e];
                }
                r0 = r0 + nb_step(best, 0, st);
                r1 = r1 + nb_step(best, 1, st);
                mc = top;
                fin = !(r0 + r1 <= 1.0);
            }
            if (fin) {
                if (j == 0) {
                    L.cut[2 * q_cur] = r0;
                    L.cut[2 * q_cur + 1] = r1;
                }
#pragma unroll
                for (int kk = 0; kk < 3; ++kk) se[kk] = ss[kk] + ci[kk];
                ++m;
                if (m < nls) open_line();
            }
        }
    }
    n_sweeps += __shfl_xor(n_sweeps, 1); n_sweeps += __shfl_xor(n_sweeps, 2); n_sweeps += __shfl_xor(n_sweeps, 4);
    n_eval += __shfl_xor(n_eval, 1); n_eval += __shfl_xor(n_eval, 2); n_eval += __shfl_xor(n_eval, 4);
    if (seq && j == 0) {
        step_rec(p.scr.bytes, b)[GFPL_STEP_CUT_STEPS] = n_steps;
        step_rec(p.scr.bytes, b)[GFPL_STEP_CUT_EXACT] = n_steps;
        step_rec(p.scr.bytes, b)[GFPL_STEP_CUT_UNBOUNDED] = 0;
        dbg_row(p.scr.dbg, b)[DBG_EIG_SWEEPS] = n_sweeps;
        dbg_row(p.scr.dbg, b)[DBG_EIG_EVALS] = n_eval;
    }
}

#ifndef GFPL_FIN_WAVES
#define GFPL_FIN_WAVES 4
#endif
__global__ void __launch_bounds__(64, GFPL_FIN_WAVES) k_cut_finish(KParams p) {
    const int b = blockIdx.x;
    const int nls = p.tr.n_matched_ls[b];
    if (nls == 0) return;
    const bool ends_only = p.cfg.cut_with_max_vol && (p.cfg.cut_proof == 1 || p.cfg.cut_proof == 3) &&
                           p.scr.cut_flag[b] == 0;
    const DevCam& cam = p.cam;
    DevLines& L = p.prev.ls;
    const size_t lb = (size_t)b * p.kl_cap;
    const int32_t* mls = p.tr.matched_ls + (size_t)b * p.mls_cap;
    double Dl[16];
#pragma unroll
    for (int i = 0; i < 16; ++i) Dl[i] = p.scr.cut_dtinv[16 * b + i];
    for (int m0 = 0; m0 < nls; m0 += 64) {
        const int m = m0 + (int)threadIdx.x;
        const bool live = m < nls;
        const size_t q = lb + (live ? mls[m] : 0);
        LineCutData d;
        double r0 = 0.0, r1 = 0.0;
        double info[36];
        if (live && ends_only) {
            load_line(L, q, d);
            r0 = L.cut[2 * q];
            r1 = L.cut[2 * q + 1];
        } else if (live) {
            load_line(L, q, d);
            r0 = L.cut[2 * q];
            r1 = L.cut[2 * q + 1];
            poseInfoOnLine<true>(cam, p.cfg.homog_th, Dl, d, r0, r1, info);
            double2* iv = reinterpret_cast<double2*>(L.invcov + 36 * q);
#pragma unroll
            for (int i = 0; i < 18; ++i) iv[i] = make_double2(info[2 * i], info[2 * i + 1]);
        }
        if (live && !(fabs(r0) < 0.0001 && fabs(r1) < 0.0001)) {
            double sP[3] = {d.sP[0], d.sP[1], d.sP[2]}, eP[3] = {d.eP[0], d.eP[1], d.eP[2]};
            if (fabs(r0) > 0.0001) {
                double s[3];
                for (int k = 0; k < 3; ++k) s[k] = (1 - r0) * sP[k] + r0 * eP[k];
                for (int k = 0; k < 3; ++k) { sP[k] = s[k]; L.sP[3 * q + k] = s[k]; }
                double uv[2];
                projection(cam, sP, uv);
                L.spl[2 * q] = uv[0]; L.spl[2 * q + 1] = uv[1];
                L.sdisp[q] = (cam.fx * cam.b) / sP[2];
            }
            if (fabs(r1) > 0.0001) {
                double e[3];
                for (int k = 0; k < 3; ++k) e[k] = (1 - r1) * eP[k] + r1 * sP[k];
                for (int k = 0; k < 3; ++k) { eP[k] = e[k]; L.eP[3 * q + k] = e[k]; }
                double uv[2];
                projection(cam, eP, uv);
                L.epl[2 * q] = uv[0]; L.epl[2 * q + 1] = uv[1];
                L.edisp[q] = (cam.fx * cam.b) / eP[2];
            }
        }
    }
}

__device__ __forceinline__ void vref_replay(const KParams& p, int b, int m) {
    const double* fd = p.scr.cut_rec + LINE_SLOT(p, b, m) * CUT_REC;
    double* out = p.scr.cut_vmax + LINE_SLOT(p, b, m) * CUT_VMAX;
    const uint8_t* path = p.scr.cut_path + LINE_SLOT(p, b, m) * CUT_PATH;
    const DevLines& L = p.prev.ls;
    const size_t q = (size_t)b * p.kl_cap + p.tr.matched_ls[LINE_SLOT(p, b, m)];
    const double* Dl = p.scr.cut_dtinv + 16 * (size_t)b;
    const double st = p.cfg.cut_step, rlo = p.cfg.cut_rng[0], rhi = p.cfg.cut_rng[1];
    double sP[3], eP[3], cS[9], cE[9], Jl[2], qs[5], qe[5];
#pragma unroll
    for (int k = 0; k < 3; ++k) { sP[k] = L.sP[3 * q + k]; eP[k] = L.eP[3 * q + k]; }
#pragma unroll
    for (int k = 0; k < 9; ++k) { cS[k] = L.covS[9 * q + k]; cE[k] = L.covE[9 * q + k]; }
    Jl[0] = L.le_obs[3 * q];
    Jl[1] = L.le_obs[3 * q + 1];
#pragma unroll
    for (int k = 0; k < 5; ++k) { qs[k] = fd[PD_VS + k]; qe[k] = fd[PD_VE + k]; }
    double r0 = 0.0, r1 = 0.0;
    bool done = false;
    long long ct0[4] = {-1, -1, -1, -1}, ct1[4] = {-1, -1, -1, -1};
    double cv0[4] = {0, 0, 0, 0}, cv1[4] = {0, 0, 0, 0};
    int slot0 = 0, slot1 = 0;
    double ivm[2] = {0.0, 0.0}, rim[2] = {0.0, 0.0};
    int marg = 0, nbad = 0, nev = 0;
    for (int k = 0; k < CUT_PATH && !done; ++k) {
        const int by = path[k];
        if (!(by & CUT_P_EXACT)) {
            ++marg;
            for (int w = 0; w < 6; ++w) {
                const int side = w >= 3 ? 1 : 0, o = w - 3 * side;
                const double rc = side ? r1 : r0;
                const double t = o == 0 ? rc + (-st) : (o == 2 ? rc + st : rc);
                if (!(t >= rlo && t <= rhi)) continue;
                const long long tb = __double_as_longlong(t);
                double vr = 0.0;
                bool hit = false;
#pragma unroll
                for (int z = 0; z < 4; ++z) {
                    const bool h = side ? ct1[z] == tb : ct0[z] == tb;
                    vr = h ? (side ? cv1[z] : cv0[z]) : vr;
                    hit = hit || h;
                }
                if (!hit) {
                    vr = side ? ref_vprime_at<true>(p.cam, p.cfg.homog_th, Dl, eP, sP, cE, cS, Jl, t)
                              : ref_vprime_at<true>(p.cam, p.cfg.homog_th, Dl, sP, eP, cS, cE, Jl, t);
                    ++nev;
#pragma unroll
                    for (int z = 0; z < 4; ++z) {
                        if (side && slot1 == z) { ct1[z] = tb; cv1[z] = vr; }
                        if (!side && slot0 == z) { ct0[z] = tb; cv0[z] = vr; }
                    }
                    if (side) slot1 = (slot1 + 1) & 3; else slot0 = (slot0 + 1) & 3;
                }
                const double* qc = side ? qe : qs;
                const double vo = __builtin_fma(t, __builtin_fma(t, __builtin_fma(t, __builtin_fma(t, qc[4], qc[3]), qc[2]),
                                                                 qc[1]), qc[0]);
                const double lo = fmin(vr, vo);
                const double rv = fabs(vo - vr) / vr;
                if (!(lo > 0.0 && rv < 0.01)) { ++nbad; continue; }
                const double iv = 1.01 / lo;
                ivm[side] = fmax(ivm[side], iv);
                rim[side] = fmax(rim[side], rv * iv);
            }
        }
        if (by & CUT_P_STAY) {
            done = true;
        } else {
            const int jj = by & 7;
            r0 = r0 + nb_step(jj, 0, st);
            r1 = r1 + nb_step(jj, 1, st);
            if (!(r0 + r1 <= 1.0)) done = true;
        }
    }
    if (!done || __double_as_longlong(r0) != __double_as_longlong(L.cut[2 * q]) ||
        __double_as_longlong(r1) != __double_as_longlong(L.cut[2 * q + 1]))
        nbad += 1 << 20;
    out[0] = ivm[0];
    out[1] = rim[0];
    out[2] = ivm[1];
    out[3] = rim[1];
    out[4] = (double)marg + 1024.0 * (double)nev;
    out[5] = (double)nbad;
}


__global__ void __launch_bounds__(64) k_cut_vref(KParams p) {
    __shared__ double keys[CUT_KS];
    __shared__ int8_t knx[CUT_KS], kpv[CUT_KS];
    __shared__ uint16_t items[64 * 2 * CUT_KS];
    __shared__ unsigned long long red[4][64];
    __shared__ int nbl[64];
    __shared__ int qln[64];
    const int b = blockIdx.y;
    const int lane = threadIdx.x;
    const int m = blockIdx.x * 64 + lane;
    const int nls = p.tr.n_matched_ls[b];
    if (blockIdx.x * 64 >= nls) return;
    const int nk = p.cut_nkeys;
    if (lane < CUT_KS) {
        keys[lane] = p.cut_keys[lane];
        knx[lane] = p.cut_knxt[lane];
        kpv[lane] = p.cut_kprv[lane];
    }
#pragma unroll
    for (int i = 0; i < 4; ++i) red[i][lane] = 0ull;
    nbl[lane] = 0;
    wave_lds_sync();
    const bool on = m < nls;
    const double st = p.cfg.cut_step, rlo = p.cfg.cut_rng[0], rhi = p.cfg.cut_rng[1];
    uint32_t mk[2] = {0u, 0u};
    int marg = 0, nbad = 0;
    bool off = nk == 0;
    if (on && !off) {
        const uint4* pv = reinterpret_cast<const uint4*>(p.scr.cut_path + LINE_SLOT(p, b, m) * CUT_PATH);
        uint32_t pw[CUT_PATH / 4];
#pragma unroll
        for (int i = 0; i < CUT_PATH / 16; ++i) {
            const uint4 v = pv[i];
            pw[4 * i] = v.x; pw[4 * i + 1] = v.y; pw[4 * i + 2] = v.z; pw[4 * i + 3] = v.w;
        }
        double r[2] = {0.0, 0.0};
        int kc[2] = {0, 0};
        bool done = false;
        for (int k = 0; k < CUT_PATH && !done && !off; ++k) {
            uint32_t wd = pw[0];
#pragma unroll
            for (int i = 1; i < CUT_PATH / 4; ++i) wd = (k >> 2) == i ? pw[i] : wd;
            const int by = (int)((wd >> (8 * (k & 3))) & 255u);
            if (!(by & CUT_P_EXACT)) {
                ++marg;
#pragma unroll
                for (int side = 0; side < 2; ++side) {
#pragma unroll
                    for (int o = 0; o < 3; ++o) {
                        const double t = o == 0 ? r[side] + (-st) : (o == 2 ? r[side] + st : r[side]);
                        if (!(t >= rlo && t <= rhi)) continue;
                        const int kk = kc[side] < 0 ? -1 : (o == 0 ? kpv[kc[side]] : (o == 2 ? knx[kc[side]] : kc[side]));
                        if (kk < 0 || __double_as_longlong(keys[kk]) != __double_as_longlong(t)) { off = true; continue; }
                        mk[side] |= 1u << kk;
                    }
                }
            }
            if (by & CUT_P_STAY) {
                done = true;
            } else {
                const int jj = by & 7;
#pragma unroll
                for (int side = 0; side < 2; ++side) {
                    const double sv = nb_step(jj, side, st);
                    r[side] = r[side] + sv;
                    if (kc[side] >= 0) kc[side] = sv > 0.0 ? knx[kc[side]] : (sv < 0.0 ? kpv[kc[side]] : kc[side]);
                }
                if (!(r[0] + r[1] <= 1.0)) done = true;
            }
        }
        const int qi = p.tr.matched_ls[LINE_SLOT(p, b, m)];
        qln[lane] = qi;
        const size_t q = (size_t)b * p.kl_cap + qi;
        if (!done || __double_as_longlong(r[0]) != __double_as_longlong(p.prev.ls.cut[2 * q]) ||
            __double_as_longlong(r[1]) != __double_as_longlong(p.prev.ls.cut[2 * q + 1]))
            nbad += 1 << 20;
    }
    if (off) mk[0] = mk[1] = 0u;
    const int cnt = __popc(mk[0]) + __popc(mk[1]);
    int inc = cnt;
#pragma unroll
    for (int o = 1; o < 64; o <<= 1) {
        const int v = __shfl_up(inc, o);
        if (lane >= o) inc += v;
    }
    const int total = __shfl(inc, 63);
    {
        int w = inc - cnt;
#pragma unroll
        for (int side = 0; side < 2; ++side) {
            uint32_t x = mk[side];
            while (x) {
                const int kk = __ffs(x) - 1;
                x &= x - 1u;
                items[w++] = (uint16_t)((lane << 6) | (side << 5) | kk);
            }
        }
    }
    wave_lds_sync();
    const DevLines& L = p.prev.ls;
    const double* Dl = p.scr.cut_dtinv + 16 * (size_t)b;
    for (int i0 = 0; i0 < total; i0 += 64) {
        const int i = i0 + lane;
        if (i < total) {
            const int it = items[i];
            const int ln = it >> 6, side = (it >> 5) & 1, kk = it & 31;
            const int mm = blockIdx.x * 64 + ln;
            const size_t q = (size_t)b * p.kl_cap + qln[ln];
            const double* fd = p.scr.cut_rec + LINE_SLOT(p, b, mm) * CUT_REC;
            double P0[3], P1[3], C0[9], C1[9], Jl[2], qc[5];
            const double* A3 = side ? L.eP : L.sP;
            const double* B3 = side ? L.sP : L.eP;
            const double* A9 = side ? L.covE : L.covS;
            const double* B9 = side ? L.covS : L.covE;
#pragma unroll
            for (int k = 0; k < 3; ++k) { P0[k] = A3[3 * q + k]; P1[k] = B3[3 * q + k]; }
#pragma unroll
            for (int k = 0; k < 9; ++k) { C0[k] = A9[9 * q + k]; C1[k] = B9[9 * q + k]; }
            Jl[0] = L.le_obs[3 * q];
            Jl[1] = L.le_obs[3 * q + 1];
#pragma unroll
            for (int k = 0; k < 5; ++k) qc[k] = fd[(side ? PD_VE : PD_VS) + k];
            const double t = keys[kk];
            const double vr = ref_vprime_at<true>(p.cam, p.cfg.homog_th, Dl, P0, P1, C0, C1, Jl, t);
            const double vo = __builtin_fma(t, __builtin_fma(t, __builtin_fma(t, __builtin_fma(t, qc[4], qc[3]), qc[2]),
                                                             qc[1]), qc[0]);
            const double lo = fmin(vr, vo);
            const double rv = fabs(vo - vr) / vr;
            if (!(lo > 0.0 && rv < 0.01)) {
                atomicAdd(&nbl[ln], 1);
            } else {
                const double iv = 1.01 / lo;
                atomicMax(&red[2 * side][ln], (unsigned long long)__double_as_longlong(iv));
                atomicMax(&red[2 * side + 1][ln], (unsigned long long)__double_as_longlong(rv * iv));
            }
        }
    }
    wave_lds_sync();
    if (!on) return;
    double* out = p.scr.cut_vmax + LINE_SLOT(p, b, m) * CUT_VMAX;
    if (off) {
        const int slot = atomicAdd(p.scr.cut_offl, 1);
        p.scr.cut_offl[1 + slot] = b * p.mls_cap + m;
        return;
    }
#pragma unroll
    for (int i = 0; i < 4; ++i) out[i] = __longlong_as_double((long long)red[i][lane]);
    out[4] = (double)marg + 1024.0 * (double)cnt;
    out[5] = (double)(nbad + nbl[lane]);
}

__global__ void __launch_bounds__(64) k_cut_vref_off(KParams p) {
    const int n = p.scr.cut_offl[0];
    for (int i = blockIdx.x * 64 + threadIdx.x; i < n; i += gridDim.x * 64) {
        const int e = p.scr.cut_offl[1 + i];
        vref_replay(p, e / p.mls_cap, e % p.mls_cap);
    }
}

__global__ void __launch_bounds__(64) k_cut_ebound(KParams p) {
    const int b = blockIdx.y;
    const int m = blockIdx.x * 64 + threadIdx.x;
    if (m >= p.tr.n_matched_ls[b]) return;
    const double* fd = p.scr.cut_rec + LINE_SLOT(p, b, m) * CUT_REC;
    if (fd[PD_OK] == 0.0) return;
    const size_t q = (size_t)b * p.kl_cap + p.tr.matched_ls[LINE_SLOT(p, b, m)];
    double Dl[16];
#pragma unroll
    for (int i = 0; i < 16; ++i) Dl[i] = p.scr.cut_dtinv[16 * b + i];
    float eb[14];
    cut_line_bounds_p(p, q, true, Dl, eb);
    float* o = reinterpret_cast<float*>(p.scr.cut_vmax + LINE_SLOT(p, b, m) * CUT_VMAX + CUT_VMAX_EB);
#pragma unroll
    for (int i = 0; i < 14; ++i) o[i] = eb[i];
}

__device__ __attribute__((noinline)) int verify_exact_step(const KParams& p, const double* Dl, size_t q, double r0,
                                                           double r1, int first, const double* Sref, const double* Sfull,
                                                           int recorded) {
    const double st = p.cfg.cut_step, rlo = p.cfg.cut_rng[0], rhi = p.cfg.cut_rng[1];
    double ep[6][7];
#pragma unroll
    for (int j = 0; j < 6; ++j) {
        const int side = j < 3 ? 0 : 1;
        const double eoff = (j % 3) == 0 ? -st : ((j % 3) == 2 ? st : 0.0);
        exact_endpoint(p.cam, p.cfg.homog_th, Dl, p.prev.ls, q, side, (side == 0 ? r0 : r1) + eoff, ep[j]);
    }
    double tot[21], tmp[21];
    double mc;
    if (first) {
#pragma unroll
        for (int i = 0; i < 21; ++i) tot[i] = Sfull[i];
    } else {
        cut_assemble<false>(ep[1], ep[4], tmp);
#pragma unroll
        for (int i = 0; i < 21; ++i) tot[i] = tmp[i] + Sref[i];
    }
    mc = logdet6_lower(tot);
    double mx = -__builtin_inf();
    int best = -1;
    for (int jn = 0; jn < 8; ++jn) {
        const double t0 = r0 + nb_step(jn, 0, st), t1 = r1 + nb_step(jn, 1, st);
        if (t0 + t1 > 1.0 || t0 < rlo || t0 > rhi || t1 < rlo || t1 > rhi) continue;
        cut_assemble<false>(ep[nb_slot(jn, 0)], ep[3 + nb_slot(jn, 1)], tmp);
#pragma unroll
        for (int i = 0; i < 21; ++i) tot[i] = tmp[i] + Sref[i];
        const double v = logdet6_lower(tot);
        if (v == v && v > mx) { mx = v; best = jn; }
    }
    const int ref = (best >= 0 && mx > mc) ? best : CUT_P_STAY;
    return ref == recorded ? 1 : 0;
}

__device__ __attribute__((noinline)) int verify_line_detail(const KParams& p, const double* Dl, size_t q,
                                                            const uint8_t* path_m, const double* fd, double r0f,
                                                            double r1f, double K0, double A1, double B1, double cs,
                                                            double ce, double R0, double rts, double rte, bool line_ok,
                                                            const double* Scol, int sstride, int& n_xchk) {
    const double st = p.cfg.cut_step, rlo = p.cfg.cut_rng[0], rhi = p.cfg.cut_rng[1];
    const bool pdok = fd[PD_OK] != 0.0;
    int bad = 0;
    {
            double r0 = 0.0, r1 = 0.0;
            bool done = false;
            int first = 1;
            double ct[2][4], cv[2][4];
            int cn[2] = {0, 0};
            for (int k = 0; k < CUT_PATH && !done; ++k) {
                const int by = path_m[k];
                if (!(by & CUT_P_EXACT)) {
                    double ivm[2] = {0.0, 0.0}, rim[2] = {0.0, 0.0};
                    bool vok = pdok;
                    for (int w = 0; w < 6 && vok; ++w) {
                        const int side = w / 3, o = w % 3;
                        const double rc = side ? r1 : r0;
                        const double t = o == 0 ? rc + (-st) : (o == 2 ? rc + st : rc);
                        if (!(t >= rlo && t <= rhi)) continue;
                        double vr = 0.0;
                        bool hit = false;
                        for (int z = 0; z < cn[side]; ++z)
                            if (__double_as_longlong(ct[side][z]) == __double_as_longlong(t)) { vr = cv[side][z]; hit = true; }
                        if (!hit) {
                            vr = ref_vprime(p.cam, p.cfg.homog_th, Dl, p.prev.ls, q, side, t);
                            const int z = cn[side] < 4 ? cn[side]++ : (k & 3);
                            ct[side][z] = t;
                            cv[side][z] = vr;
                        }
                        const double vo = cut_ours_V(fd, side, t);
                        const double lo = fmin(vr, vo);
                        const double rv = fabs(vo - vr) / vr;
                        if (!(lo > 0.0 && rv < 0.01)) { vok = false; continue; }
                        const double iv = 1.01 / lo;
                        ivm[side] = fmax(ivm[side], iv);
                        rim[side] = fmax(rim[side], (1.01 * rv + (side ? rte : rts)) * iv);
                    }
                    const double E = K0 + A1 * ivm[0] + cs * rim[0] + B1 * ivm[1] + ce * rim[1];
                    if (!(vok && line_ok && E * 1.0001 <= R0)) {
                        double Sref[21], Sfull[21];
#pragma unroll
                        for (int e = 0; e < 21; ++e) { Sfull[e] = Scol[sstride * e]; Sref[e] = Sfull[e] - fd[CUT_FAST + e]; }
                        ++n_xchk;
                        if (!verify_exact_step(p, Dl, q, r0, r1, first, Sref, Sfull, (by & CUT_P_STAY) ? CUT_P_STAY : (by & 7)))
                            bad |= 512;
                    }
                }
                first = 0;
                if (by & CUT_P_STAY) {
                    done = true;
                } else {
                    const int jj = by & 7;
                    r0 = r0 + nb_step(jj, 0, st);
                    r1 = r1 + nb_step(jj, 1, st);
                    if (!(r0 + r1 <= 1.0)) done = true;
                }
            }
            if (!done || __double_as_longlong(r0) != __double_as_longlong(r0f) ||
                __double_as_longlong(r1) != __double_as_longlong(r1f))
                bad |= 1;
        }
    return bad;
}

struct LineBound {
    double K0, A1, B1, cs, ce, R0, rts, rte, epsS, kt;
    int ok;
};
__device__ __forceinline__ LineBound verify_line_bound(const KParams& p, size_t q, const double* fd, const double* vmx,
                                                      const double* Dl, const double* So, const double* Sf) {
    const double rlo = p.cfg.cut_rng[0], rhi = p.cfg.cut_rng[1];
    const double T = fmax(fabs(rlo), fabs(rhi));
    const double tau = p.cfg.cut_certify;
    constexpr double u = 0x1p-53;
    LineBound lbd;
    double K0, A1, B1, cs, ce, R0, rts, rte, epsS_l, kt_l;
    bool line_ok;
        float eb[14];
        {
            const float* ebg = reinterpret_cast<const float*>(vmx + 6);
#pragma unroll
            for (int i = 0; i < 14; ++i) eb[i] = ebg[i];
        }
        double o28[28];
        {
            double S[21];
#pragma unroll
            for (int e = 0; e < 21; ++e) S[e] = So[65 * e];
            chol_s(S, o28);
        }
        double sg[6];
#pragma unroll
        for (int j = 0; j < 6; ++j) {
            double x[6], a = 0.0;
#pragma unroll
            for (int i = 0; i < 6; ++i) {
                double uu = i == j ? 1.0 : 0.0;
#pragma unroll
                for (int k = 0; k < i; ++k) uu = uu - o28[tri(i, k)] * x[k];
                x[i] = uu * o28[21 + i];
                a = a + x[i] * x[i];
            }
            sg[j] = 1.002 * a;
        }
        double Bn[2] = {0.0, 0.0};
#pragma unroll
        for (int side = 0; side < 2; ++side) {
            double tk = 1.0;
#pragma unroll
            for (int kk = 0; kk < 3; ++kk) {
                double w[6], a = 0.0;
#pragma unroll
                for (int i = 0; i < 6; ++i) {
                    double uu = fd[(side ? PD_PE : PD_PS) + 6 * kk + i];
#pragma unroll
                    for (int k = 0; k < i; ++k) uu = uu - o28[tri(i, k)] * w[k];
                    w[i] = uu * o28[21 + i];
                    a = a + w[i] * w[i];
                }
                Bn[side] = Bn[side] + 1.01 * sqrt(a) * tk;
                tk = tk * T;
            }
        }
        double Kc = 0.0, xi = 0.0, Qs = 0.0, Qe = 0.0, hs0 = 0.0, he0 = 0.0, Lam = 0.0, dSn = 0.0;
#pragma unroll
        for (int i = 0; i < 6; ++i) {
            const double Sii = So[65 * tri(i, i)];
            const double es = eb[i], ee = eb[7 + i];
            const double ps = fabs(fd[PD_PS + i]) + T * (fabs(fd[PD_PS + 6 + i]) + T * fabs(fd[PD_PS + 12 + i])) + es;
            const double pe = fabs(fd[PD_PE + i]) + T * (fabs(fd[PD_PE + 6 + i]) + T * fabs(fd[PD_PE + 12 + i])) + ee;
            const double kc = Sii * sg[i];
            Kc = Kc + kc;
            xi = xi + sqrt(kc);
            Qs = Qs + sg[i] * ps * ps;
            Qe = Qe + sg[i] * pe * pe;
            hs0 = hs0 + es * sqrt(sg[i]);
            he0 = he0 + ee * sqrt(sg[i]);
            Lam = Lam + ((Sii > 0.0 && Sii < 1e300) ? 0.6931471805599453 * (double)(abs(__builtin_amdgcn_frexp_exp(Sii)) + 1)
                                                     : __builtin_inf());
#pragma unroll
            for (int k = 0; k < 6; ++k) {
                const int e = tri(i > k ? i : k, i > k ? k : i);
                const double sref = Sf[65 * e] - fd[CUT_FAST + e];
                const double dd = 1.0000000000000004 * fabs(So[65 * e] - sref);
                dSn = dSn + dd * sqrt(sg[i] * sg[k]);
            }
        }
        const double epsS = 1.01 * dSn + (7.01 * u) * xi * xi;
        const double hs = hs0 + (6.01 * u) * Bn[0] * xi, he = he0 + (6.01 * u) * Bn[1] * xi;
        const double ck = 110.0 * u;
        K0 = 1.002 * epsS + ck * Kc + (7.1 * u) * Lam;
        const double bs = Bn[0] + hs, be = Bn[1] + he;
        rts = 4.1 * (double)eb[6] + 16.0 * u;
        rte = 4.1 * (double)eb[13] + 16.0 * u;
        A1 = 1.03 * (2.0 * ck * Qs + 4.0 * hs * bs);
        B1 = 1.03 * (2.0 * ck * Qe + 4.0 * he * be);
        cs = 4.12 * bs * bs;
        ce = 4.12 * be * be;
        R0 = fmin(0.125 * tau, 1e-3) - 1.01 * K0;
        line_ok = o28[27] != 0.0 && epsS <= 1e-3 && Kc <= 1e8 && R0 > 0.0 && rlo >= 0.0 && rhi <= 1.0 &&
                  tau > 0.0 && rts + rte <= 0.01;
        epsS_l = 1.002 * epsS;
        kt_l = ck * Kc + (7.1 * u) * Lam;

    lbd.K0 = K0; lbd.A1 = A1; lbd.B1 = B1; lbd.cs = cs; lbd.ce = ce; lbd.R0 = R0; lbd.rts = rts; lbd.rte = rte;
    lbd.epsS = epsS_l; lbd.kt = kt_l; lbd.ok = line_ok ? 1 : 0;
    return lbd;
}

__global__ void __launch_bounds__(64) __attribute__((amdgpu_waves_per_eu(2, 2))) k_cut_verify(KParams p) {
    __shared__ double fo[21][65];
    __shared__ double fr[21][65];
    const int b = blockIdx.x;
    const int lane = threadIdx.x;
    const int nls = p.tr.n_matched_ls[b];
    const DevCam& cam = p.cam;
    const double homog = p.cfg.homog_th;
    DevLines& L = p.prev.ls;
    const size_t lb = (size_t)b * p.kl_cap;
    const int32_t* mls = p.tr.matched_ls + (size_t)b * p.mls_cap;
    const double* rec_l = p.scr.cut_rec + LINE_SLOT(p, b, 0) * CUT_REC;
    double Dl[16];
#pragma unroll
    for (int i = 0; i < 16; ++i) Dl[i] = p.scr.cut_dtinv[16 * b + i];
    int bad = p.cfg.cut_proof == 3 ? 256 : 0;
    double worst = 0.0;
    double tS = 0.0, tK = 0.0, tA = 0.0, tV = 0.0;
    int64_t n_marg = 0, n_eval = 0, n_mline = 0, n_xchk = 0, n_dline = 0;
    double sA = 0.0, sE = 0.0;
    if (nls > 0 && lane < 21) {
        const double s0 = p.scr.cut_sum[CUT_SUM_REC * b + lane];
        sA = s0 - rec_l[CUT_FAST + lane];
        sE = s0;
    }
    constexpr bool VCLOCK = GFPL_DIAG(GFPL_VERIFY_CLOCK);
    PhaseClock<VCLOCK, 5> vk;
    vk.reset();
    for (int c0 = 0; c0 < nls; c0 += 64) {
        const int m = c0 + lane;
        const bool on = m < nls;
        const size_t q = lb + (on ? mls[m] : mls[0]);
        const double* fd = rec_l + (size_t)(on ? m : 0) * CUT_REC;
        const double r0f = L.cut[2 * q], r1f = L.cut[2 * q + 1];
        {
            LineCutData d;
            load_line(L, q, d);
            double info[36];
            poseInfoOnLine<true>(cam, homog, Dl, d, r0f, r1f, info);
            if (on) {
                double2* iv = reinterpret_cast<double2*>(L.invcov + 36 * q);
#pragma unroll
                for (int i = 0; i < 18; ++i) iv[i] = make_double2(info[2 * i], info[2 * i + 1]);
#pragma unroll
                for (int i = 0; i < 6; ++i)
#pragma unroll
                    for (int k = 0; k <= i; ++k) fr[tri(i, k)][lane] = info[i * 6 + k];
            }
        }
        PHASE_TICK(vk, 0);
        const bool pdok = fd[PD_OK] != 0.0;
        {
            double xs[14];
            if (pdok) {
                xs[0] = cut_ours_V(fd, 0, r0f);
                xs[7] = cut_ours_V(fd, 1, r1f);
#pragma unroll
                for (int i = 0; i < 6; ++i) { xs[1 + i] = cut_ours_P(fd, 0, i, r0f); xs[8 + i] = cut_ours_P(fd, 1, i, r1f); }
            } else {
                exact_endpoint(cam, homog, Dl, L, q, 0, r0f, xs);
                exact_endpoint(cam, homog, Dl, L, q, 1, r1f, xs + 7);
            }
            const double is = rcp_fast(xs[0]), ie = rcp_fast(xs[7]);
            if (on) {
#pragma unroll
                for (int i = 0; i < 6; ++i)
#pragma unroll
                    for (int k = 0; k <= i; ++k) fo[tri(i, k)][lane] = cut_ours_info(xs, is, ie, i, k);
            }
        }
        wave_lds_sync();
        PHASE_TICK(vk, 1);
        const int cnt = min(64, nls - c0);
        if (lane < 21) {
            auto fetch = [&](int l0, double* v) {
#pragma unroll
                for (int k = 0; k < 17; ++k) {
                    const int mm = c0 + l0 + k;
                    v[k] = (l0 + k <= cnt && mm < nls) ? rec_l[(size_t)mm * CUT_REC + CUT_FAST + lane] : 0.0;
                }
            };
            double iv[17];
            for (int l0 = 0; l0 < cnt; l0 += 16) {
                fetch(l0, iv);
#pragma unroll
                for (int k = 0; k < 16; ++k) {
                    const int l = l0 + k;
                    if (l < cnt) {
                        const double sref = sE - iv[k];
                        const double f_o = fo[lane][l], f_r = fr[lane][l];
                        fo[lane][l] = sA;
                        fr[lane][l] = sE;
                        sE = sref + f_r;
                        sA = (sA + f_o) - iv[k + 1];
                    }
                }
            }
        }
        wave_lds_sync();
        PHASE_TICK(vk, 2);
        double K0 = 0.0, A1 = 0.0, B1 = 0.0, cs = 0.0, ce = 0.0, R0 = -1.0, rts = 0.0, rte = 0.0;
        double epsS_l = 0.0, kt_l = 0.0;
        bool line_ok = false;
        if (on && pdok) {
            const LineBound lbd = verify_line_bound(p, q, fd, p.scr.cut_vmax + LINE_SLOT(p, b, m) * CUT_VMAX, Dl,
                                                    &fo[0][0] + lane, &fr[0][0] + lane);
            K0 = lbd.K0; A1 = lbd.A1; B1 = lbd.B1; cs = lbd.cs; ce = lbd.ce; R0 = lbd.R0; rts = lbd.rts; rte = lbd.rte;
            epsS_l = lbd.epsS; kt_l = lbd.kt; line_ok = lbd.ok != 0;
        }
        PHASE_TICK(vk, 3);
        int marg = 0;
        bool detail = false;
        if (on) {
            const double* vm = p.scr.cut_vmax + LINE_SLOT(p, b, m) * CUT_VMAX;
            const double mv = vm[4];
            marg = (int)fmod(mv, 1024.0);
            n_eval += (int64_t)(mv / 1024.0);
            if (marg) {
                const double E = K0 + A1 * vm[0] + cs * (1.01 * vm[1] + rts * vm[0]) + B1 * vm[2] +
                                 ce * (1.01 * vm[3] + rte * vm[2]);
                detail = !(vm[5] == 0.0 && line_ok && E * 1.0001 <= R0);
                if (!detail && E / R0 > worst) {
                    worst = E / R0;
                    tS = epsS_l / R0;
                    tK = kt_l / R0;
                    tA = (A1 * vm[0] + B1 * vm[2]) / R0;
                    tV = (cs * (1.01 * vm[1] + rts * vm[0]) + ce * (1.01 * vm[3] + rte * vm[2])) / R0;
                }
            }
            n_marg += marg;
            n_mline += marg ? 1 : 0;
            n_dline += detail ? 1 : 0;
        }
        PHASE_TICK(vk, 4);
        if (detail) {
            const int slot = atomicAdd(p.scr.cut_dtln, 1);
            if (slot < CUT_DTL * p.B) {
                double* e = p.scr.cut_dtl + (size_t)slot * CUT_DTL_REC;
#pragma unroll
                for (int i = 0; i < CUT_INFO; ++i) e[DTL_S + i] = fr[i][lane];
                e[DTL_K0] = K0; e[DTL_A1] = A1; e[DTL_B1] = B1; e[DTL_CS] = cs; e[DTL_CE] = ce; e[DTL_R0] = R0;
                e[DTL_RTS] = rts; e[DTL_RTE] = rte;
                e[DTL_OK] = line_ok ? 1.0 : 0.0;
                p.scr.cut_dtln[1 + slot] = b * p.mls_cap + m;
            } else {
                bad |= 1024;
            }
        }
        wave_lds_sync();
    }
    int mask = bad;
    int wl = lane;
#pragma unroll
    for (int o = 32; o > 0; o >>= 1) {
        mask |= __shfl_xor(mask, o);
        const double ow = __shfl_xor(worst, o);
        const int ol = __shfl_xor(wl, o);
        if (ow > worst || (ow == worst && ol < wl)) { worst = ow; wl = ol; }
    }
    tS = __shfl(tS, wl); tK = __shfl(tK, wl); tA = __shfl(tA, wl); tV = __shfl(tV, wl);
    bad = mask != 0 ? 1 : 0;
#pragma unroll
    for (int o = 32; o > 0; o >>= 1) {
        n_marg += __shfl_xor(n_marg, o);
        n_eval += __shfl_xor(n_eval, o);
        n_mline += __shfl_xor(n_mline, o);
        n_xchk += __shfl_xor(n_xchk, o);
        n_dline += __shfl_xor(n_dline, o);
    }
    if (lane == 0) {
        p.scr.cut_flag[b] = bad;
        step_rec(p.scr.bytes, b)[GFPL_STEP_PROOF_REDONE] = bad;
        step_rec(p.scr.bytes, b)[GFPL_STEP_PROOF_STEPS] = n_marg;
        step_rec(p.scr.bytes, b)[GFPL_STEP_PROOF_VREF] = n_eval;
        step_rec(p.scr.bytes, b)[GFPL_STEP_PROOF_LINES] = n_mline;
        dbg_row(p.scr.dbg, b)[DBG_VFY_MASK] = mask;
        dbg_row(p.scr.dbg, b)[DBG_VFY_WORST] = __double_as_longlong(worst);
        dbg_row(p.scr.dbg, b)[DBG_VFY_XCHK] = n_xchk;
        dbg_row(p.scr.dbg, b)[DBG_VFY_DLINES] = n_dline;
        dbg_row(p.scr.dbg, b)[DBG_VFY_TS] = __double_as_longlong(tS);
        dbg_row(p.scr.dbg, b)[DBG_VFY_TK] = __double_as_longlong(tK);
        dbg_row(p.scr.dbg, b)[DBG_VFY_TA] = __double_as_longlong(tA);
        dbg_row(p.scr.dbg, b)[DBG_VFY_TV] = __double_as_longlong(tV);
        if (VCLOCK) vk.store(dbg_row(p.scr.dbg, b));
    }
}

__global__ void __launch_bounds__(64) k_cut_verify_detail(KParams p) {
    const int n = min(p.scr.cut_dtln[0], CUT_DTL * p.B);
    for (int i = blockIdx.x * 64 + threadIdx.x; i < n; i += gridDim.x * 64) {
        const int e = p.scr.cut_dtln[1 + i];
        const int b = e / p.mls_cap, m = e % p.mls_cap;
        const double* pl = p.scr.cut_dtl + (size_t)i * CUT_DTL_REC;
        const size_t q = (size_t)b * p.kl_cap + p.tr.matched_ls[LINE_SLOT(p, b, m)];
        const double* fd = p.scr.cut_rec + LINE_SLOT(p, b, m) * CUT_REC;
        const uint8_t* path = p.scr.cut_path + LINE_SLOT(p, b, m) * CUT_PATH;
        double Dl[16];
#pragma unroll
        for (int k = 0; k < 16; ++k) Dl[k] = p.scr.cut_dtinv[16 * b + k];
        int nx = 0;
        const int bad = verify_line_detail(p, Dl, q, path, fd, p.prev.ls.cut[2 * q], p.prev.ls.cut[2 * q + 1], pl[DTL_K0],
                                           pl[DTL_A1], pl[DTL_B1], pl[DTL_CS], pl[DTL_CE], pl[DTL_R0], pl[DTL_RTS],
                                           pl[DTL_RTE], pl[DTL_OK] != 0.0, pl + DTL_S, 1, nx);
        if (bad) {
            atomicOr(&p.scr.cut_flag[b], 1);
            atomicOr(reinterpret_cast<unsigned long long*>(&step_rec(p.scr.bytes, b)[GFPL_STEP_PROOF_REDONE]), 1ull);
        }
        if (nx)
            atomicAdd(reinterpret_cast<unsigned long long*>(&dbg_row(p.scr.dbg, b)[DBG_VFY_XCHK]), (unsigned long long)nx);
    }
}

static int cut_wave_max_b() { return env_int("GFPL_CUT_WAVE_MAX_B", CUT_WAVE_MAX_B); }

static int cut_prep_w8_max_b() { return env_int("GFPL_CUT_PREP_W8_MAX_B", 256); }

hipError_t launch_line_cut(const KParams& p, hipStream_t s, const hipEvent_t* marks) {
    const int mode = p.cfg.cut_proof;
    const dim3 gsearch((p.B + CUT_G - 1) / CUT_G);
    if (p.B <= cut_prep_w8_max_b()) {
        static std::atomic<unsigned long long> attr{0};
        const hipError_t e = ensure_dyn_lds(reinterpret_cast<const void*>(k_cut_prep<8>), (int)cut_prep_lds(8), &attr);
        if (e != hipSuccess) return e;
        hipLaunchKernelGGL(k_cut_prep<8>, dim3(p.B), dim3(512), cut_prep_lds(8), s, p);
    } else {
        hipLaunchKernelGGL(k_cut_prep<1>, dim3(p.B), dim3(64), cut_prep_lds(1), s, p);
    }
    if (!p.cfg.cut_with_max_vol) {
        if (marks) (void)hipEventRecord(marks[0], s);
        hipLaunchKernelGGL(k_cut_search_eig, gsearch, dim3(64), 0, s, p);
        if (marks) (void)hipEventRecord(marks[1], s);
        hipLaunchKernelGGL(k_cut_finish, dim3(p.B), dim3(64), 0, s, p);
        return hipGetLastError();
    }
    if (mode == 2) {
        hipLaunchKernelGGL(k_cut_bounds, dim3((p.mls_cap + 63) / 64, p.B), dim3(64), 0, s, p);
        hipLaunchKernelGGL(k_cut_vtab, dim3(p.B), dim3(256), 0, s, p);
    }
    if (marks) (void)hipEventRecord(marks[0], s);
    if (mode == 2)
        hipLaunchKernelGGL(k_cut_search<true>, gsearch, dim3(64), 0, s, p);
    else if (p.B <= cut_wave_max_b())
        hipLaunchKernelGGL(k_cut_search_w, dim3(p.B), dim3(64), 0, s, p);
    else if (mode == 1 || mode == 3)
        hipLaunchKernelGGL(HIP_KERNEL_NAME(k_cut_search<false, true>), gsearch, dim3(64), 0, s, p);
    else
        hipLaunchKernelGGL(k_cut_search<false>, gsearch, dim3(64), 0, s, p);
    if (marks) (void)hipEventRecord(marks[1], s);
    if (mode == 1 || mode == 3) {
        if (hipMemsetAsync(p.scr.cut_offl, 0, sizeof(int32_t), s) != hipSuccess) return hipGetLastError();
        hipLaunchKernelGGL(k_cut_vref, dim3((p.mls_cap + 63) / 64, p.B), dim3(64), 0, s, p);
        hipLaunchKernelGGL(k_cut_vref_off, dim3(256), dim3(64), 0, s, p);
        hipLaunchKernelGGL(k_cut_ebound, dim3((p.mls_cap + 63) / 64, p.B), dim3(64), 0, s, p);
        if (hipMemsetAsync(p.scr.cut_dtln, 0, sizeof(int32_t), s) != hipSuccess) return hipGetLastError();
        hipLaunchKernelGGL(k_cut_verify, dim3(p.B), dim3(64), 0, s, p);
        hipLaunchKernelGGL(k_cut_verify_detail, dim3(256), dim3(64), 0, s, p);
        hipLaunchKernelGGL(k_cut_bounds, dim3((p.mls_cap + 63) / 64, p.B), dim3(64), 0, s, p);
        hipLaunchKernelGGL(k_cut_vtab, dim3(p.B), dim3(256), 0, s, p);
        hipLaunchKernelGGL(k_cut_search<true>, gsearch, dim3(64), 0, s, p);
    }
    hipLaunchKernelGGL(k_cut_finish, dim3(p.B), dim3(64), 0, s, p);
    return hipGetLastError();
}

}
```

Measured before the change: 801,900.

## Shrink per-line cut record by storing geometry and recomputing polynomial coefficients

The per-line cut record goes from 80 to 48 doubles. Instead of storing the 36 precomputed P polynomial coefficients, it stores the transformed endpoints and line Jacobian (8 doubles) and recomputes the coefficients on the fly in the search, verify and bounds kernels. Proof-mode error bounds move into a separate side buffer, and a debug kernel rebuilds the old 80-double layout for the debug API. This cuts memory traffic and LDS footprint per line, at the cost of extra arithmetic when the coefficients are rebuilt.

```diff
diff --git a/gf-pl-slam_amd/csrc/gfpl_abi.hip b/gf-pl-slam_amd/csrc/gfpl_abi.hip
--- a/gf-pl-slam_amd/csrc/gfpl_abi.hip
+++ b/gf-pl-slam_amd/csrc/gfpl_abi.hip
@@ -142,6 +142,7 @@
     sb->tr.kf_nsince = c.take<int32_t>(B);
     sb->tr.kf_flag = c.take<int32_t>(B);
     sb->scr.cut_rec = c.take<double>(B * sb->mls_cap * CUT_REC);
+    sb->scr.cut_prf = c.take<double>(B * sb->mls_cap * CUT_PRF);
     sb->scr.knn = c.take<int32_t>(B * 2 * (size_t)sb->kp_cap * 3);
     sb->scr.proj = reinterpret_cast<double*>(sb->scr.knn);
     sb->scr.bytes = c.take<int64_t>(B * STEP_REC);
@@ -1465,9 +1466,18 @@
     if (!sb || !out || b < 0 || b >= sb->B || n_lines < 0 || n_lines > sb->mls_cap) return GFPL_E_INVALID;
     if (hipSetDevice(sb->ctx->device) != hipSuccess) return GFPL_E_HIP;
     if (hipStreamSynchronize(sb->ctx->stream) != hipSuccess) return GFPL_E_HIP;
-    const size_t n = (size_t)n_lines * CUT_REC;
-    return hipMemcpy(out, sb->scr.cut_rec + (size_t)b * sb->mls_cap * CUT_REC, n * sizeof(double),
-                     hipMemcpyDeviceToHost) == hipSuccess ? GFPL_OK : GFPL_E_HIP;
+    if (n_lines == 0) return GFPL_OK;
+    const size_t bytes = (size_t)n_lines * CUT_DBG_REC * sizeof(double);
+    int32_t flagged = 0;
+    if (sb->last_cut_mode == 1 || sb->last_cut_mode == 3)
+        if (hipMemcpy(&flagged, sb->scr.cut_flag + b, sizeof flagged, hipMemcpyDeviceToHost) != hipSuccess) return GFPL_E_HIP;
+    double* view = nullptr;
+    if (hipMalloc(&view, bytes) != hipSuccess) return GFPL_E_HIP;
+    bool ok = launch_cut_debug_view(params(sb, nullptr), b, sb->last_cut_mode, flagged, n_lines, view, sb->ctx->stream) == hipSuccess;
+    ok = ok && hipStreamSynchronize(sb->ctx->stream) == hipSuccess;
+    ok = ok && hipMemcpy(out, view, bytes, hipMemcpyDeviceToHost) == hipSuccess;
+    (void)hipFree(view);
+    return ok ? GFPL_OK : GFPL_E_HIP;
 }
 
 int gfpl_debug_step_records(gfpl_seqbatch* sb, int64_t* out) {
diff --git a/gf-pl-slam_amd/csrc/gfpl_kernels.hpp b/gf-pl-slam_amd/csrc/gfpl_kernels.hpp
--- a/gf-pl-slam_amd/csrc/gfpl_kernels.hpp
+++ b/gf-pl-slam_amd/csrc/gfpl_kernels.hpp
@@ -46,6 +46,7 @@
 hipError_t launch_cross_points(const KParams& p, hipStream_t s);
 hipError_t launch_cross_lines(const KParams& p, hipStream_t s);
 hipError_t launch_line_cut(const KParams& p, hipStream_t s, const hipEvent_t* marks );
+hipError_t launch_cut_debug_view(const KParams& p, int b, int mode, int flagged, int n, double* out, hipStream_t s);
 hipError_t launch_pose(const KParams& p, hipStream_t s, hipEvent_t mark );
 hipError_t launch_step_bytes(const KParams& p, hipStream_t s);
 hipError_t launch_need_kf(const KParams& p, hipStream_t s);
diff --git a/gf-pl-slam_amd/csrc/gfpl_records.hpp b/gf-pl-slam_amd/csrc/gfpl_records.hpp
--- a/gf-pl-slam_amd/csrc/gfpl_records.hpp
+++ b/gf-pl-slam_amd/csrc/gfpl_records.hpp
@@ -34,11 +34,30 @@
 #define CUT_P_EXACT 16
 #define CUT_KS 22
 
+#define CUT_REC 48
+constexpr int CUT_INFO = 21;
+#define CR_G0 0
+#define CR_G1 3
+#define CR_JL 6
+#define CR_VS 8
+#define CR_VE 13
+#define CR_OK 18
+#define CR_NEXT 19
+#define CR_INFO 20
+constexpr int CUT_GEO = 8;
+constexpr int CUT_HEAD = CR_INFO;
+constexpr int CUT_NX = CR_INFO + CUT_INFO;
+static_assert(CR_G1 == CR_G0 + 3 && CR_JL == CR_G0 + 6 && CR_VS == CR_G0 + CUT_GEO, "cut_rec_coeff reads g0 | g1 | Jl as one run");
+static_assert(CR_VE == CR_VS + 5 && CR_OK == CR_VS + 10 && CR_NEXT == CR_OK + 1 && CR_INFO == CR_NEXT + 1, "record layout");
+static_assert(CUT_REC * 8 == 384 && CUT_NX <= CUT_REC, "a record is 3 x 128 B: three 16-B loads per lane");
+
+constexpr int CUT_PRF = 10;
+#define PRF_ERR 0
+#define PRF_EB 7
+constexpr int CUT_NX_EB = 3;
+static_assert(PRF_ERR + 7 <= PRF_EB && PRF_EB + CUT_NX_EB <= CUT_PRF, "proven-mode side record");
+
 #define CUT_FAST 56
-#define CUT_REC 80
-constexpr int CUT_INFO = 21;
-constexpr int CUT_NX = CUT_FAST + CUT_INFO;
-constexpr int CUT_NX_EB = 3;
 #define PD_PS 0
 #define PD_PE 18
 #define PD_VS 36
@@ -46,8 +65,15 @@
 #define PD_OK 46
 #define PD_NEXT 47
 #define PD_ERR 48
+#define PD_GEO 56
+constexpr int CUT_VIEW = CUT_FAST + CUT_GEO;
+constexpr int CUT_DBG_REC = 80;
+constexpr int CUT_DBG_EB = CUT_FAST + CUT_INFO;
 static_assert(PD_ERR + 7 <= CUT_FAST && CUT_FAST == 56, "per-line comparison data layout");
-static_assert(CUT_REC * 8 == 640 && CUT_NX + CUT_NX_EB <= CUT_REC, "a record is 5 x 128 B: five 16-B loads per lane");
+static_assert(PD_PE == PD_PS + 18 && PD_VE == PD_VS + 5, "cut_ours_P / cut_ours_V: both sides as one run");
+static_assert(PD_VS - CR_VS == PD_NEXT - CR_NEXT && PD_VE - CR_VE == PD_OK - CR_OK, "record -> view: one shift past the geometry");
+static_assert(CUT_DBG_EB + CUT_NX_EB <= CUT_DBG_REC, "debug view");
+constexpr int cut_view_slot(int e) { return e < CUT_GEO ? PD_GEO + e : e + (PD_VS - CR_VS); }
 
 constexpr int CUT_SUM_REC = 24;
 
diff --git a/gf-pl-slam_amd/csrc/gfpl_state.hpp b/gf-pl-slam_amd/csrc/gfpl_state.hpp
--- a/gf-pl-slam_amd/csrc/gfpl_state.hpp
+++ b/gf-pl-slam_amd/csrc/gfpl_state.hpp
@@ -67,6 +67,7 @@
 
 struct DevScratch {
     double* cut_rec;
+    double* cut_prf;
     int32_t* knn;
     double* proj;
     int64_t* bytes;
diff --git a/gf-pl-slam_amd/csrc/k_cut.hip b/gf-pl-slam_amd/csrc/k_cut.hip
--- a/gf-pl-slam_amd/csrc/k_cut.hip
+++ b/gf-pl-slam_amd/csrc/k_cut.hip
@@ -142,7 +142,8 @@
 __device__ __forceinline__ void cut_poly_coeff_t(const T* g0, const T* g1, T lx, T ly, int k, T* Pk) {
     const T dx = g1[0] - g0[0], dy = g1[1] - g0[1], dz = g1[2] - g0[2];
     auto prod = [&](T a0, T a1, T b0, T b1) -> T {
-        return k == 0 ? a0 * b0 : (k == 1 ? a0 * b1 + a1 * b0 : a1 * b1);
+        const T c0 = a0 * b0, c1 = a0 * b1 + a1 * b0, c2 = a1 * b1;
+        return k == 0 ? c0 : (k == 1 ? c1 : c2);
     };
     auto lin = [&](T a0, T a1) -> T { return k == 0 ? a0 : (k == 1 ? a1 : T(0.0)); };
     const T x0 = g0[0], y0 = g0[1], z0 = g0[2];
@@ -155,11 +156,11 @@
 }
 
 template <typename T>
-__device__ __forceinline__ void cut_poly_coef_t(const double* Dl, const T* sP, const T* eP, const T* covS,
-                                                const T* covE, const T* Jl, T* P, T* V, T* g) {
+__device__ __forceinline__ void cut_poly_geo_t(const double* Dl, const T* sP, const T* eP, const T* covS,
+                                               const T* covE, T* g, T* Af) {
     se3_apply_t<T, double>(Dl, sP, g);
     se3_apply_t<T, double>(Dl, eP, g + 3);
-    T A[2][6];
+    T (*A)[6] = reinterpret_cast<T (*)[6]>(Af);
     const T* Cs[2] = {covS, covE};
 #pragma unroll
     for (int w = 0; w < 2; ++w) {
@@ -176,33 +177,65 @@
             A[w][e] = (Tm[ii[e] * 3 + 0] * T(Dl[jj[e] * 4 + 0]) + Tm[ii[e] * 3 + 1] * T(Dl[jj[e] * 4 + 1])) +
                       Tm[ii[e] * 3 + 2] * T(Dl[jj[e] * 4 + 2]);
     }
+}
+template <typename T>
+__device__ __forceinline__ void cut_poly_var_t(const T* Aa, const T* Ab, const T* p0, const T* p1, T* v) {
+    const T a0 = sym3_t<T>(Aa, p0, p0), a1 = sym3_t<T>(Aa, p0, p1), a2 = sym3_t<T>(Aa, p1, p1);
+    const T b0 = sym3_t<T>(Ab, p0, p0), b1 = sym3_t<T>(Ab, p0, p1), b2 = sym3_t<T>(Ab, p1, p1);
+    v[0] = a0;
+    v[1] = T(2.0) * (a1 - a0);
+    v[2] = ((a2 - T(4.0) * a1) + a0) + b0;
+    v[3] = T(2.0) * ((a1 - a2) + b1);
+    v[4] = a2 + b2;
+}
+template <typename T>
+__device__ __forceinline__ void cut_poly_coef_t(const double* Dl, const T* sP, const T* eP, const T* covS,
+                                                const T* covE, const T* Jl, T* P, T* V, T* g) {
+    T A[2][6];
+    cut_poly_geo_t<T>(Dl, sP, eP, covS, covE, g, &A[0][0]);
 #pragma unroll
     for (int side = 0; side < 2; ++side) {
         T* Ps = P + 18 * side;
 #pragma unroll
         for (int k = 0; k < 3; ++k) cut_poly_coeff_t<T>(g + 3 * side, g + 3 * (1 - side), Jl[0], Jl[1], k, Ps + 6 * k);
-        const T* p0 = Ps;
-        const T* p1 = Ps + 6;
-        const T a0 = sym3_t<T>(A[side], p0, p0), a1 = sym3_t<T>(A[side], p0, p1), a2 = sym3_t<T>(A[side], p1, p1);
-        const T b0 = sym3_t<T>(A[1 - side], p0, p0), b1 = sym3_t<T>(A[1 - side], p0, p1), b2 = sym3_t<T>(A[1 - side], p1, p1);
-        T* v = V + 5 * side;
-        v[0] = a0;
-        v[1] = T(2.0) * (a1 - a0);
-        v[2] = ((a2 - T(4.0) * a1) + a0) + b0;
-        v[3] = T(2.0) * ((a1 - a2) + b1);
-        v[4] = a2 + b2;
-    }
-}
-
-__device__ __forceinline__ void cut_poly_data(const double* Dl, const LineCutData& d, double homog, double* fd) {
-    double P[36], V[10], g[6];
-    cut_poly_coef_t<double>(Dl, d.sP, d.eP, d.covS, d.covE, d.Jl, P, V, g);
-#pragma unroll
-    for (int i = 0; i < 18; ++i) { fd[PD_PS + i] = P[i]; fd[PD_PE + i] = P[18 + i]; }
-#pragma unroll
-    for (int i = 0; i < 5; ++i) { fd[PD_VS + i] = V[i]; fd[PD_VE + i] = V[5 + i]; }
+        cut_poly_var_t<T>(A[side], A[1 - side], Ps, Ps + 6, V + 5 * side);
+    }
+}
+
+__device__ __forceinline__ void cut_rec_coeff(const double* geo, int side, int k, double* Pk) {
+    double a[3], b[3];
+#pragma unroll
+    for (int i = 0; i < 3; ++i) {
+        const double u = geo[i], v = geo[3 + i];
+        a[i] = side ? v : u;
+        b[i] = side ? u : v;
+    }
+    cut_poly_coeff_t<double>(a, b, geo[6], geo[7], k, Pk);
+}
+__device__ __forceinline__ void cut_rec_coeffs(const double* geo, double* P) {
+#pragma unroll
+    for (int side = 0; side < 2; ++side)
+#pragma unroll
+        for (int k = 0; k < 3; ++k) cut_rec_coeff(geo, side, k, P + 18 * side + 6 * k);
+}
+
+__device__ __forceinline__ void cut_rec_head(const double* Dl, const LineCutData& d, double homog, double* hd) {
+    double V[10], A[2][6];
+    double* g = hd + CR_G0;
+    cut_poly_geo_t<double>(Dl, d.sP, d.eP, d.covS, d.covE, g, &A[0][0]);
+    hd[CR_JL] = d.Jl[0];
+    hd[CR_JL + 1] = d.Jl[1];
+#pragma unroll
+    for (int side = 0; side < 2; ++side) {
+        double p0[6], p1[6];
+        cut_rec_coeff(g, side, 0, p0);
+        cut_rec_coeff(g, side, 1, p1);
+        cut_poly_var_t<double>(A[side], A[1 - side], p0, p1, V + 5 * side);
+    }
+#pragma unroll
+    for (int i = 0; i < 10; ++i) hd[CR_VS + i] = V[i];
     const double z0 = g[2], z1 = g[5];
-    fd[PD_OK] = (((z0 > 0.0 && z1 > 0.0) || (z0 < 0.0 && z1 < 0.0)) && z0 * z0 > 2.0 * homog && z1 * z1 > 2.0 * homog)
+    hd[CR_OK] = (((z0 > 0.0 && z1 > 0.0) || (z0 < 0.0 && z1 < 0.0)) && z0 * z0 > 2.0 * homog && z1 * z1 > 2.0 * homog)
                     ? 1.0 : 0.0;
 }
 
@@ -245,16 +278,14 @@
             const int m = ((lines ? c : c - nl_ch) << 6) + lane;
             const int cnt = chunk_cnt(c);
             double info[21];
-            double fd[CUT_FAST];
+            double hd[CUT_HEAD];
             if (lane < cnt) {
                 if (lines) {
                     LineCutData d;
                     load_line(L, lb + mls[m], d);
                     poseInfoOnLine<false>(cam, homog, Dl, d, 0.0, 0.0, info);
-#pragma unroll
-                    for (int i = PD_ERR; i < CUT_FAST; ++i) fd[i] = 0.0;
-                    cut_poly_data(Dl, d, homog, fd);
-                    fd[PD_NEXT] = (double)mls[min(m + 1, nls - 1)];
+                    cut_rec_head(Dl, d, homog, hd);
+                    hd[CR_NEXT] = (double)mls[min(m + 1, nls - 1)];
                 } else {
                     const size_t q = pbase + mpt[m];
                     double Pp[3] = {P.P[3 * q], P.P[3 * q + 1], P.P[3 * q + 2]};
@@ -280,7 +311,7 @@
 #pragma unroll
                         for (int k = 0; k < 16; ++k) {
                             const int x = 16 * sl + k;
-                            stg[lane * 17 + k] = x < CUT_FAST ? fd[x] : (x < CUT_FAST + 21 ? info[x - CUT_FAST] : 0.0);
+                            stg[lane * 17 + k] = x < CUT_HEAD ? hd[x] : (x < CUT_NX ? info[x - CR_INFO] : 0.0);
                         }
                     }
                     wave_lds_sync();
@@ -487,13 +518,13 @@
     const int nls = p.tr.n_matched_ls[b];
     if (m >= nls || (p.cfg.cut_proof != 2 && p.scr.cut_flag[b] == 0)) return;
     const size_t q = (size_t)b * p.kl_cap + p.tr.matched_ls[LINE_SLOT(p, b, m)];
-    double* rec = p.scr.cut_rec + LINE_SLOT(p, b, m) * CUT_REC;
+    const double* rec = p.scr.cut_rec + LINE_SLOT(p, b, m) * CUT_REC;
     double Dl[16];
 #pragma unroll
     for (int i = 0; i < 16; ++i) Dl[i] = p.scr.cut_dtinv[16 * b + i];
     float eb[14];
-    cut_line_bounds(p, q, rec[PD_OK] != 0.0, Dl, eb);
-    float* out = reinterpret_cast<float*>(rec + PD_ERR);
+    cut_line_bounds(p, q, rec[CR_OK] != 0.0, Dl, eb);
+    float* out = reinterpret_cast<float*>(p.scr.cut_prf + LINE_SLOT(p, b, m) * CUT_PRF + PRF_ERR);
 #pragma unroll
     for (int i = 0; i < 14; ++i) out[i] = eb[i];
 }
@@ -578,14 +609,14 @@
     return __builtin_fma(t, __builtin_fma(t, c2, c1), c0);
 }
 
-__device__ __forceinline__ double cut_ours_P(const double* fd, int side, int i, double t) {
-    const int o = side ? PD_PE : PD_PS;
-    return h2(fd[o + i], fd[o + 6 + i], fd[o + 12 + i], t);
-}
-__device__ __forceinline__ double cut_ours_V(const double* fd, int side, double t) {
-    const int o = side ? PD_VE : PD_VS;
-    return __builtin_fma(t, __builtin_fma(t, __builtin_fma(t, __builtin_fma(t, fd[o + 4], fd[o + 3]), fd[o + 2]),
-                                          fd[o + 1]), fd[o]);
+__device__ __forceinline__ double cut_ours_P(const double* P, int side, int i, double t) {
+    const int o = 18 * side;
+    return h2(P[o + i], P[o + 6 + i], P[o + 12 + i], t);
+}
+__device__ __forceinline__ double cut_ours_V(const double* V, int side, double t) {
+    const int o = 5 * side;
+    return __builtin_fma(t, __builtin_fma(t, __builtin_fma(t, __builtin_fma(t, V[o + 4], V[o + 3]), V[o + 2]),
+                                          V[o + 1]), V[o]);
 }
 __device__ __forceinline__ double cut_ours_info(const double* xs, double is, double ie, int ra, int cb) {
     return __builtin_fma(xs[1 + ra] * is, xs[1 + cb], (xs[8 + ra] * ie) * xs[8 + cb]);
@@ -748,7 +779,7 @@
                             const int e = 4 * c + i;
                             if (e < 21) {
                                 tmpw[4 * lane + i] = info[e];
-                                tmpw[256 + 4 * lane + i] = recG[(size_t)(s0 + lane) * CUT_REC + CUT_FAST + e];
+                                tmpw[256 + 4 * lane + i] = recG[(size_t)(s0 + lane) * CUT_REC + CR_INFO + e];
                             }
                         }
                     }
@@ -778,7 +809,7 @@
             for (int i = 0; i < 7; ++i) epf[CUT_SL * j + i] = o7[i];
         }
 #pragma unroll
-        for (int e = 0; e < 21; ++e) xs[e] = sumE[e] - rec_l[(size_t)m * CUT_REC + CUT_FAST + e];
+        for (int e = 0; e < 21; ++e) xs[e] = sumE[e] - rec_l[(size_t)m * CUT_REC + CR_INFO + e];
     }
     wave_lds_sync();
     if (exact) {
@@ -879,9 +910,9 @@
 __global__ void __launch_bounds__(64) __attribute__((amdgpu_waves_per_eu(GFPL_CUT_WPE, GFPL_CUT_WPE))) k_cut_search(KParams p) {
     __shared__ double sumA[CUT_G][CUT_SSTR];
     __shared__ double sumE[CUT_G][CUT_SSTR];
-    __shared__ double fst[CUT_G][CUT_FAST + 1];
+    __shared__ double fst[CUT_G][CUT_VIEW + 1];
     constexpr bool PF = !PROOF && !GFPL_CUT_NOPF;
-    __shared__ __attribute__((aligned(16))) double nxl[PF ? 5 : 1][PF ? 128 : 2];
+    __shared__ __attribute__((aligned(16))) double nxl[PF ? CUT_REC / 16 : 1][PF ? 128 : 2];
     __shared__ double tmp[CUT_G][CUT_EP + 25 + 1];
     static_assert(CUT_G * (CUT_EP + 25 + 1) >= 512, "the exact-sum flush stages 64 x (4 + 4) doubles in tmp");
     __shared__ CutCmp cmpl[CUT_G];
@@ -910,6 +941,7 @@
     const size_t lb = (size_t)(live ? b : 0) * p.kl_cap;
     const int32_t* mls = p.tr.matched_ls + (size_t)(live ? b : 0) * p.mls_cap;
     const double* rec_l = p.scr.cut_rec + LINE_SLOT(p, live ? b : 0, 0) * CUT_REC;
+    double* const prf_l = p.scr.cut_prf + LINE_SLOT(p, live ? b : 0, 0) * CUT_PRF;
     const double* Dl = p.scr.cut_dtinv + 16 * (size_t)(live ? b : 0);
     const double st = p.cfg.cut_step;
     const double rlo = p.cfg.cut_rng[0], rhi = p.cfg.cut_rng[1];
@@ -946,6 +978,8 @@
             n0s = n1s = cnxt[0];
             p0s = p1s = cprv[0];
         }
+        double Pj[6];
+        cut_rec_coeff(&fst[g][PD_GEO], j >= 3 ? 1 : 0, j >= 3 ? j - 3 : j, Pj);
         double o[28];
         {
             double S[21];
@@ -958,13 +992,13 @@
             double w[6];
 #pragma unroll
             for (int i = 0; i < 6; ++i) {
-                double u = fst[g][6 * j + i];
+                double u = Pj[i];
 #pragma unroll
                 for (int k = 0; k < i; ++k) u = __builtin_fma(-o[tri(i, k)], w[k], u);
                 w[i] = u * o[21 + i];
             }
 #pragma unroll
-            for (int i = 0; i < 6; ++i) wg[6 * j + i] = w[i];
+            for (int i = 0; i < 6; ++i) { wg[6 * j + i] = w[i]; fst[g][PD_PS + 6 * j + i] = Pj[i]; }
             double x[6], sg = 0.0;
             if (PROOF) {
 #pragma unroll
@@ -1033,7 +1067,7 @@
 #pragma unroll
             for (int i = 1; i < 6; ++i) usable = usable && e6[i] < __builtin_inff();
             n_unb += usable ? 0 : 1;
-            if (j < 6 && live) reinterpret_cast<float*>(const_cast<double*>(rec_l) + (size_t)m * CUT_REC + CUT_NX)[j] = e6[j];
+            if (j < 6 && live) reinterpret_cast<float*>(prf_l + (size_t)m * CUT_PRF + PRF_EB)[j] = e6[j];
         }
         const double vs0 = PROOF ? vtab[g][0] : cl[CC_VS], ve0 = PROOF ? vtab[g][CUT_KS] : cl[CC_VE];
         dc = cut_dcore_p1<PROOF>(cl[CC_NS], vs0, cl[CC_NE], ve0, cl[CC_CC], cl[CC_BND], cl[CC_BND + 1], cl[CC_BND + 2],
@@ -1043,20 +1077,29 @@
         if (!PF) return;
         const char* src = reinterpret_cast<const char*>(rec_l + (size_t)mm * CUT_REC) + 16 * j;
 #pragma unroll
-        for (int k = 0; k < (PF ? 5 : 0); ++k) {
+        for (int k = 0; k < (PF ? CUT_REC / 16 : 0); ++k) {
             const uint32_t dst = (uint32_t)(uintptr_t)&nxl[k][0];
             asm volatile("s_mov_b32 m0, %1\n\tglobal_load_lds_dwordx4 %0, off" ::"v"(src + 128 * k), "s"(dst)
                          : "memory", "m0");
         }
+    };
+    auto view_from_hbm = [&](int mm) {
+        const double* r = rec_l + (size_t)mm * CUT_REC;
+#pragma unroll
+        for (int k = 0; k < (CUT_HEAD + 7) / 8; ++k) {
+            const int e = j + 8 * k;
+            if (e < CUT_HEAD) fst[g][cut_view_slot(e)] = r[e];
+        }
+        if (PROOF && j < 7) fst[g][PD_ERR + j] = prf_l[(size_t)mm * CUT_PRF + PRF_ERR + j];
     };
     if (m < nls) {
         q_cur = lb + mls[0];
         if (nls > 1) q_nx = lb + mls[1];
-        for (int e = j; e < CUT_FAST; e += 8) fst[g][e] = rec_l[e];
+        view_from_hbm(0);
 #pragma unroll
         for (int e = j; e < 21; e += 8) {
             const double s0 = p.scr.cut_sum[CUT_SUM_REC * b + e];
-            sumA[g][e] = s0 - rec_l[CUT_FAST + e];
+            sumA[g][e] = s0 - rec_l[CR_INFO + e];
             sumE[g][e] = s0;
         }
         wave_lds_sync();
@@ -1172,10 +1215,10 @@
             if (pend) {
                 if (!PROOF && fst[g][PD_OK] != 0.0) {
                     if (j < 6) {
-                        xs[1 + j] = cut_ours_P(fst[g], 0, j, r0);
-                        xs[8 + j] = cut_ours_P(fst[g], 1, j, r1);
+                        xs[1 + j] = cut_ours_P(fst[g] + PD_PS, 0, j, r0);
+                        xs[8 + j] = cut_ours_P(fst[g] + PD_PS, 1, j, r1);
                     } else {
-                        xs[7 * (j - 6)] = cut_ours_V(fst[g], j - 6, j == 6 ? r0 : r1);
+                        xs[7 * (j - 6)] = cut_ours_V(fst[g] + PD_VS, j - 6, j == 6 ? r0 : r1);
                     }
                 } else if (j < 2) {
                     double o7[7];
@@ -1200,10 +1243,7 @@
                         info[kk] = cut_ours_info(xs, is, ie, ra, cb);
                     }
                 }
-                if (!PF) {
-#pragma unroll
-                    for (int k = 0; k < CUT_FAST / 8; ++k) fst[g][j + 8 * k] = rec_l[(size_t)m * CUT_REC + j + 8 * k];
-                }
+                if (!PF) view_from_hbm(m);
                 if (!PROOF) {
                     if (PF) asm volatile("s_waitcnt vmcnt(0)" ::: "memory");
                     if (j == 0) {
@@ -1214,9 +1254,9 @@
                         *reinterpret_cast<unsigned long long*>(path + (size_t)(m - 1) * CUT_PATH + 8 * j) =
                             *reinterpret_cast<const unsigned long long*>(&pth[g][8 * j]);
 #pragma unroll
-                    for (int k = 0; k < (PF ? CUT_FAST / 8 : 0); ++k) {
+                    for (int k = 0; k < (PF ? (CUT_HEAD + 7) / 8 : 0); ++k) {
                         const int e = j + 8 * k;
-                        fst[g][e] = nxl[e >> 4][16 * g + (e & 15)];
+                        if (e < CUT_HEAD) fst[g][cut_view_slot(e)] = nxl[e >> 4][16 * g + (e & 15)];
                     }
                 }
             }
@@ -1232,7 +1272,7 @@
 #pragma unroll
                 for (int kk = 0; kk < 3; ++kk) {
                     const int e = j + 8 * kk;
-                    const int x = CUT_FAST + e;
+                    const int x = CR_INFO + e;
                     if (e < 21) {
                         const double mid = sumA[g][e] + info[kk];
                         const double nw = mid - (PF ? nxl[x >> 4][16 * g + (x & 15)] : rec_l[(size_t)m * CUT_REC + x]);
@@ -1298,7 +1338,7 @@
 __global__ void __launch_bounds__(64) __attribute__((amdgpu_waves_per_eu(2, 2))) k_cut_search_w(KParams p) {
     __shared__ double sumA[25];
     __shared__ double sumE[25];
-    __shared__ double fst[CUT_FAST + 1];
+    __shared__ double fst[CUT_VIEW + 1];
     __shared__ double tmp[CUT_G][CUT_EP + 25 + 1];
     __shared__ double wgs[64];
     __shared__ double xsl[16];
@@ -1330,6 +1370,11 @@
     PhaseClock<TCLOCK, 7> tk;
     tk.reset();
     auto open_line = [&]() {
+        double Pj[6];
+        {
+            const int k6 = min(lane, 5);
+            cut_rec_coeff(&fst[PD_GEO], k6 >= 3 ? 1 : 0, k6 >= 3 ? k6 - 3 : k6, Pj);
+        }
         double o[28];
         {
             double S[21];
@@ -1343,13 +1388,13 @@
             double w[6];
 #pragma unroll
             for (int i = 0; i < 6; ++i) {
-                double u = fst[6 * lane + i];
+                double u = Pj[i];
 #pragma unroll
                 for (int k = 0; k < i; ++k) u = __builtin_fma(-o[tri(i, k)], w[k], u);
                 w[i] = u * o[21 + i];
             }
 #pragma unroll
-            for (int i = 0; i < 6; ++i) wgs[6 * lane + i] = w[i];
+            for (int i = 0; i < 6; ++i) { wgs[6 * lane + i] = w[i]; fst[PD_PS + 6 * lane + i] = Pj[i]; }
         }
         wave_lds_sync();
         PHASE_TICK(tk, 3);
@@ -1408,10 +1453,10 @@
     };
     if (nls > 0) {
         q_cur = lb + mls[0];
-        for (int e = lane; e < CUT_FAST; e += 64) fst[e] = rec_l[e];
+        if (lane < CUT_HEAD) fst[cut_view_slot(lane)] = rec_l[lane];
         if (lane < 21) {
             const double s0 = p.scr.cut_sum[CUT_SUM_REC * b + lane];
-            sumA[lane] = s0 - rec_l[CUT_FAST + lane];
+            sumA[lane] = s0 - rec_l[CR_INFO + lane];
             sumE[lane] = s0;
         }
         wave_lds_sync();
@@ -1424,8 +1469,8 @@
             int iv = mn;
             asm volatile("" : "+v"(iv));
             const double* rn = rec_l + (size_t)iv * CUT_REC;
-            pf_i0 = lane < 21 ? rn[CUT_FAST + lane] : 0.0;
-            pf_f0 = rn[lane < CUT_FAST ? lane : 0];
+            pf_i0 = lane < 21 ? rn[CR_INFO + lane] : 0.0;
+            pf_f0 = rn[lane < CUT_HEAD ? lane : 0];
             pf_q = mls[iv];
         }
     };
@@ -1656,9 +1701,9 @@
                 const int ra = (int)((TRI_ROW >> (3 * lane)) & 7), cb = (int)((TRI_COL >> (3 * lane)) & 7);
                 if (fst[PD_OK] != 0.0) {
                     if (lane < 21) {
-                        const double is = rcp_fast(cut_ours_V(fst, 0, r0)), ie = rcp_fast(cut_ours_V(fst, 1, r1));
-                        const double psr = cut_ours_P(fst, 0, ra, r0), psc = cut_ours_P(fst, 0, cb, r0);
-                        const double per = cut_ours_P(fst, 1, ra, r1), pec = cut_ours_P(fst, 1, cb, r1);
+                        const double is = rcp_fast(cut_ours_V(fst + PD_VS, 0, r0)), ie = rcp_fast(cut_ours_V(fst + PD_VS, 1, r1));
+                        const double psr = cut_ours_P(fst + PD_PS, 0, ra, r0), psc = cut_ours_P(fst + PD_PS, 0, cb, r0);
+                        const double per = cut_ours_P(fst + PD_PS, 1, ra, r1), pec = cut_ours_P(fst + PD_PS, 1, cb, r1);
                         info = __builtin_fma(psr * is, psc, (per * ie) * pec);
                     }
                 } else {
@@ -1676,7 +1721,7 @@
             PHASE_TICK(tk, 0);
             if (m < nls) {
                 wave_lds_sync();
-                if (lane < CUT_FAST) fst[lane] = pf_f0;
+                if (lane < CUT_HEAD) fst[cut_view_slot(lane)] = pf_f0;
                 if (lane < 21) sumA[lane] = (sumA[lane] + info) - pf_i0;
                 q_cur = lb + __builtin_amdgcn_readfirstlane(pf_q);
                 first = 1;
@@ -1748,7 +1793,7 @@
         for (int kk = 0; kk < 3; ++kk) {
             const int e = j + 8 * kk;
             if (e < 21) {
-                ci[kk] = rec_l[(size_t)m * CUT_REC + CUT_FAST + e];
+                ci[kk] = rec_l[(size_t)m * CUT_REC + CR_INFO + e];
                 ss[kk] = se[kk] - ci[kk];
                 smat[g][e] = se[kk];
             }
@@ -1932,7 +1977,7 @@
     Jl[0] = L.le_obs[3 * q];
     Jl[1] = L.le_obs[3 * q + 1];
 #pragma unroll
-    for (int k = 0; k < 5; ++k) { qs[k] = fd[PD_VS + k]; qe[k] = fd[PD_VE + k]; }
+    for (int k = 0; k < 5; ++k) { qs[k] = fd[CR_VS + k]; qe[k] = fd[CR_VE + k]; }
     double r0 = 0.0, r1 = 0.0;
     bool done = false;
     long long ct0[4] = {-1, -1, -1, -1}, ct1[4] = {-1, -1, -1, -1};
@@ -2122,7 +2167,7 @@
             Jl[0] = L.le_obs[3 * q];
             Jl[1] = L.le_obs[3 * q + 1];
 #pragma unroll
-            for (int k = 0; k < 5; ++k) qc[k] = fd[(side ? PD_VE : PD_VS) + k];
+            for (int k = 0; k < 5; ++k) qc[k] = fd[(side ? CR_VE : CR_VS) + k];
             const double t = keys[kk];
             const double vr = ref_vprime_at<true>(p.cam, p.cfg.homog_th, Dl, P0, P1, C0, C1, Jl, t);
             const double vo = __builtin_fma(t, __builtin_fma(t, __builtin_fma(t, __builtin_fma(t, qc[4], qc[3]), qc[2]),
@@ -2165,7 +2210,7 @@
     const int m = blockIdx.x * 64 + threadIdx.x;
     if (m >= p.tr.n_matched_ls[b]) return;
     const double* fd = p.scr.cut_rec + LINE_SLOT(p, b, m) * CUT_REC;
-    if (fd[PD_OK] == 0.0) return;
+    if (fd[CR_OK] == 0.0) return;
     const size_t q = (size_t)b * p.kl_cap + p.tr.matched_ls[LINE_SLOT(p, b, m)];
     double Dl[16];
 #pragma unroll
@@ -2220,7 +2265,7 @@
                                                             double ce, double R0, double rts, double rte, bool line_ok,
                                                             const double* Scol, int sstride, int& n_xchk) {
     const double st = p.cfg.cut_step, rlo = p.cfg.cut_rng[0], rhi = p.cfg.cut_rng[1];
-    const bool pdok = fd[PD_OK] != 0.0;
+    const bool pdok = fd[CR_OK] != 0.0;
     int bad = 0;
     {
             double r0 = 0.0, r1 = 0.0;
@@ -2248,7 +2293,7 @@
                             ct[side][z] = t;
                             cv[side][z] = vr;
                         }
-                        const double vo = cut_ours_V(fd, side, t);
+                        const double vo = cut_ours_V(fd + CR_VS, side, t);
                         const double lo = fmin(vr, vo);
                         const double rv = fabs(vo - vr) / vr;
                         if (!(lo > 0.0 && rv < 0.01)) { vok = false; continue; }
@@ -2260,7 +2305,7 @@
                     if (!(vok && line_ok && E * 1.0001 <= R0)) {
                         double Sref[21], Sfull[21];
 #pragma unroll
-                        for (int e = 0; e < 21; ++e) { Sfull[e] = Scol[sstride * e]; Sref[e] = Sfull[e] - fd[CUT_FAST + e]; }
+                        for (int e = 0; e < 21; ++e) { Sfull[e] = Scol[sstride * e]; Sref[e] = Sfull[e] - fd[CR_INFO + e]; }
                         ++n_xchk;
                         if (!verify_exact_step(p, Dl, q, r0, r1, first, Sref, Sfull, (by & CUT_P_STAY) ? CUT_P_STAY : (by & 7)))
                             bad |= 512;
@@ -2323,6 +2368,8 @@
             }
             sg[j] = 1.002 * a;
         }
+        double Pc[36];
+        cut_rec_coeffs(fd + CR_G0, Pc);
         double Bn[2] = {0.0, 0.0};
 #pragma unroll
         for (int side = 0; side < 2; ++side) {
@@ -2332,7 +2379,7 @@
                 double w[6], a = 0.0;
 #pragma unroll
                 for (int i = 0; i < 6; ++i) {
-                    double uu = fd[(side ? PD_PE : PD_PS) + 6 * kk + i];
+                    double uu = Pc[18 * side + 6 * kk + i];
 #pragma unroll
                     for (int k = 0; k < i; ++k) uu = uu - o28[tri(i, k)] * w[k];
                     w[i] = uu * o28[21 + i];
@@ -2347,8 +2394,8 @@
         for (int i = 0; i < 6; ++i) {
             const double Sii = So[65 * tri(i, i)];
             const double es = eb[i], ee = eb[7 + i];
-            const double ps = fabs(fd[PD_PS + i]) + T * (fabs(fd[PD_PS + 6 + i]) + T * fabs(fd[PD_PS + 12 + i])) + es;
-            const double pe = fabs(fd[PD_PE + i]) + T * (fabs(fd[PD_PE + 6 + i]) + T * fabs(fd[PD_PE + 12 + i])) + ee;
+            const double ps = fabs(Pc[i]) + T * (fabs(Pc[6 + i]) + T * fabs(Pc[12 + i])) + es;
+            const double pe = fabs(Pc[18 + i]) + T * (fabs(Pc[24 + i]) + T * fabs(Pc[30 + i])) + ee;
             const double kc = Sii * sg[i];
             Kc = Kc + kc;
             xi = xi + sqrt(kc);
@@ -2361,7 +2408,7 @@
 #pragma unroll
             for (int k = 0; k < 6; ++k) {
                 const int e = tri(i > k ? i : k, i > k ? k : i);
-                const double sref = Sf[65 * e] - fd[CUT_FAST + e];
+                const double sref = Sf[65 * e] - fd[CR_INFO + e];
                 const double dd = 1.0000000000000004 * fabs(So[65 * e] - sref);
                 dSn = dSn + dd * sqrt(sg[i] * sg[k]);
             }
@@ -2410,7 +2457,7 @@
     double sA = 0.0, sE = 0.0;
     if (nls > 0 && lane < 21) {
         const double s0 = p.scr.cut_sum[CUT_SUM_REC * b + lane];
-        sA = s0 - rec_l[CUT_FAST + lane];
+        sA = s0 - rec_l[CR_INFO + lane];
         sE = s0;
     }
     constexpr bool VCLOCK = GFPL_DIAG(GFPL_VERIFY_CLOCK);
@@ -2438,14 +2485,16 @@
             }
         }
         PHASE_TICK(vk, 0);
-        const bool pdok = fd[PD_OK] != 0.0;
+        const bool pdok = fd[CR_OK] != 0.0;
         {
             double xs[14];
             if (pdok) {
-                xs[0] = cut_ours_V(fd, 0, r0f);
-                xs[7] = cut_ours_V(fd, 1, r1f);
-#pragma unroll
-                for (int i = 0; i < 6; ++i) { xs[1 + i] = cut_ours_P(fd, 0, i, r0f); xs[8 + i] = cut_ours_P(fd, 1, i, r1f); }
+                double Pc[36];
+                cut_rec_coeffs(fd + CR_G0, Pc);
+                xs[0] = cut_ours_V(fd + CR_VS, 0, r0f);
+                xs[7] = cut_ours_V(fd + CR_VS, 1, r1f);
+#pragma unroll
+                for (int i = 0; i < 6; ++i) { xs[1 + i] = cut_ours_P(Pc, 0, i, r0f); xs[8 + i] = cut_ours_P(Pc, 1, i, r1f); }
             } else {
                 exact_endpoint(cam, homog, Dl, L, q, 0, r0f, xs);
                 exact_endpoint(cam, homog, Dl, L, q, 1, r1f, xs + 7);
@@ -2466,7 +2515,7 @@
 #pragma unroll
                 for (int k = 0; k < 17; ++k) {
                     const int mm = c0 + l0 + k;
-                    v[k] = (l0 + k <= cnt && mm < nls) ? rec_l[(size_t)mm * CUT_REC + CUT_FAST + lane] : 0.0;
+                    v[k] = (l0 + k <= cnt && mm < nls) ? rec_l[(size_t)mm * CUT_REC + CR_INFO + lane] : 0.0;
                 }
             };
             double iv[17];
@@ -2652,4 +2701,29 @@
     return hipGetLastError();
 }
 
-}
+__global__ void __launch_bounds__(64) k_cut_debug_view(const double* rec, const double* prf, int n, double* out) {
+    const int m = blockIdx.x * 64 + threadIdx.x;
+    if (m >= n) return;
+    const double* r = rec + (size_t)m * CUT_REC;
+    double* o = out + (size_t)m * CUT_DBG_REC;
+    double P[36];
+    cut_rec_coeffs(r + CR_G0, P);
+#pragma unroll
+    for (int i = 0; i < 36; ++i) o[PD_PS + i] = P[i];
+#pragma unroll
+    for (int e = CUT_GEO; e < CUT_HEAD; ++e) o[cut_view_slot(e)] = r[e];
+    for (int i = PD_ERR; i < CUT_FAST; ++i) o[i] = (prf && i < PD_ERR + 7) ? prf[(size_t)m * CUT_PRF + PRF_ERR + i - PD_ERR] : 0.0;
+    for (int e = 0; e < CUT_INFO; ++e) o[CUT_FAST + e] = r[CR_INFO + e];
+    for (int i = 0; i < CUT_DBG_REC - CUT_DBG_EB; ++i)
+        o[CUT_DBG_EB + i] = (prf && i < CUT_NX_EB) ? prf[(size_t)m * CUT_PRF + PRF_EB + i] : 0.0;
+}
+
+hipError_t launch_cut_debug_view(const KParams& p, int b, int mode, int flagged, int n, double* out, hipStream_t s) {
+    if (n <= 0) return hipSuccess;
+    const bool has = mode == 2 || ((mode == 1 || mode == 3) && flagged);
+    hipLaunchKernelGGL(k_cut_debug_view, dim3((n + 63) / 64), dim3(64), 0, s, p.scr.cut_rec + LINE_SLOT(p, b, 0) * CUT_REC,
+                       has ? p.scr.cut_prf + LINE_SLOT(p, b, 0) * CUT_PRF : nullptr, n, out);
+    return hipGetLastError();
+}
+
+}
```

New measurement: 798,000. Within noise of the previous version (-0.5%).
